# uga-ssrl/SSRLCV

Measured on AMD Instinct MI355X. Metric: Mpix/s SIFT extract (+ Mmatches/s 128-D brute-force, see `matcher`), higher is better.
Workload: dtype f32; 1 GPU; 2-view 4096x4096 pair per GPU (tools/scene.py pinhole views (PCG32 terrain + texture through Image::Camera)): SIFT_FeatureFactory::generateFeatures (sparse DoG path) on each image, pixels resident in HBM; images_per_gpu=2, parallelism=image-pair shard, library=release build (libssrlcv_hip_release.so)

## Files before the change

ssrlcv_amd/csrc/dev_switch.h:

```cpp
#pragma once
#include <stdlib.h>

#if (defined(SSRLCV_STAMPS) || defined(SSRLCV_MATCH_STATS) || defined(SSRLCV_TIMING_VARIANT)) && !defined(SSRLCV_INSTRUMENTED_BUILD)
#error "SSRLCV_STAMPS / SSRLCV_MATCH_STATS only build through `make instrumented` or the tools/ lab programs (-DSSRLCV_INSTRUMENTED_BUILD)"
#endif
#if defined(SSRLCV_LAB) || defined(SSRLCV_MATCH_LAB) || defined(SSRLCV_LAB_LOCAL_GATHER) || defined(SSRLCV_LAB_UPS_LOADS)
#error "the timing-lab variants (results invalid) were removed in round 6; see git history before 2026-10-05"
#endif

namespace svdev {
inline const char* env(const char* name) {
#ifdef SSRLCV_RELEASE
  (void)name;
  return nullptr;
#else
  return getenv(name);
#endif
}
}
```

ssrlcv_amd/csrc/keypoints.hip:

```cpp
#include <hip/hip_runtime.h>
#include <float.h>
#include <math.h>
#include <stdlib.h>
#include "compact.h"
#include "dev_switch.h"
#include "scan_lookback.h"
#include "device_math.h"
#include "sift_plan.h"
#include "ssrlcv_hip.h"

using svp::OctaveState;

namespace {

struct LevelSet {
  const float* lvl[svp::kGauss];
  const float* lvlMinMax;
  const float* minmax;
  const float2* polar;
  int w, h;
};

struct DogView {
  const float* lo;
// ... 104 lines not shown
  st->n = total;
  if (total == 0) st->hasExtrema = 0;
}
__global__ void k_book_featbase(OctaveState* st, uint32_t* featBase, uint32_t* numFeatures, uint32_t maxFeatures) {
  uint32_t tot = 0;
  for (int o = 0; o < svp::kOctaves; ++o) {
    featBase[o] = tot;
    tot += st[o].hasExtrema ? (uint32_t)st[o].n : 0u;
  }
  if (tot > maxFeatures) tot = maxFeatures;
  *numFeatures = tot;
}

__device__ __forceinline__ int segment_of(const OctaveState* st, int i) {
  int s = 0;
#pragma unroll
  for (int k = 1; k < svp::kDog; ++k)
    if (st->idx[k] <= i) s = k;
  return s;
}

__global__ __launch_bounds__(256) void k_flag_noise(const OctaveState* st, ssrlcv_sskeypoint* kps, float thr) {
  int n = st->hasExtrema ? st->n : 0;
  for (int i = blockIdx.x * 256 + threadIdx.x; i < n; i += gridDim.x * 256)
    kps[i].discard = (uint8_t)(fabsf(kps[i].intensity) < thr);
}

__global__ __launch_bounds__(256) void k_flag_edges(const OctaveState* st, ssrlcv_sskeypoint* kps, LevelSet L, float thr) {
  int n = st->hasExtrema ? st->n : 0;
  for (int i = blockIdx.x * 256 + threadIdx.x; i < n; i += gridDim.x * 256) {
    const DogView D = dog_view(L, segment_of(st, i));
    kps[i].discard = (uint8_t)edge_response_above(D, kps[i], L.w, thr);
  }
}

__global__ __launch_bounds__(256) void k_flag_noise_edges_window(const OctaveState* st, ssrlcv_sskeypoint* kps, LevelSet L,
                                                                 float noiseThr, float edgeThr, float pixelWidth,
                                                                 float lambda) {
  int n = st->hasExtrema ? st->n : 0;
  for (int i = blockIdx.x * 256 + threadIdx.x; i < n; i += gridDim.x * 256) {
    ssrlcv_sskeypoint kp = kps[i];
    bool drop = fabsf(kp.intensity) < noiseThr;
    drop = drop || edge_response_above(dog_view(L, segment_of(st, i)), kp, L.w, edgeThr);
    float ww = kp.sigma * lambda / pixelWidth;
    drop = drop || (kp.loc.x - ww) < 0.0f || (kp.loc.y - ww) < 0.0f || (kp.loc.x + ww) >= (unsigned)(L.w - 1) ||
           (kp.loc.y + ww) >= (unsigned)(L.h - 1);
    kps[i].discard = (uint8_t)drop;
  }
}

__global__ __launch_bounds__(256) void k_flag_window(const OctaveState* st, ssrlcv_sskeypoint* kps, int w, int h, float pixelWidth,
                                                     float lambda) {
  int n = st->hasExtrema ? st->n : 0;
  for (int i = blockIdx.x * 256 + threadIdx.x; i < n; i += gridDim.x * 256) {
    const ssrlcv_sskeypoint kp = kps[i];
    const float ww = kp.sigma * lambda / pixelWidth;
    kps[i].discard = (uint8_t)((kp.loc.x - ww) < 0.0f || (kp.loc.y - ww) < 0.0f || (kp.loc.x + ww) >= (unsigned)(w - 1) ||
                               (kp.loc.y + ww) >= (unsigned)(h - 1));
  }
}

template <typename Src>
__device__ __forceinline__ void refine_one(ssrlcv_sskeypoint& kp, int W, int H, int numBlurs, float sigmaMin, float mult, const Src& src) {
  int lx = (int)roundf(kp.loc.x), ly = (int)roundf(kp.loc.y);
  float hess[3][3], hinv[3][3] = {{0.0f, 0.0f, 0.0f}, {0.0f, 0.0f, 0.0f}, {0.0f, 0.0f, 0.0f}};
  float grad[3], temp[3], offset[3] = {0.0f, 0.0f, 0.0f};
  int bl = kp.blur;
  for (int attempt = 0; attempt < 5; ++attempt) {
    const auto Dl = src.view(bl - 1), Dm = src.view(bl), Du = src.view(bl + 1);
#define PM(yy, xx) Dm.norm((size_t)(yy) * W + (xx))
#define PL(yy, xx) Dl.norm((size_t)(yy) * W + (xx))
#define PU(yy, xx) Du.norm((size_t)(yy) * W + (xx))
    grad[0] = PM(ly, lx + 1) - PM(ly, lx - 1);
    grad[1] = PM(ly + 1, lx) - PM(ly - 1, lx);
    grad[2] = PU(ly, lx) - PL(ly, lx);
    float centre = PM(ly, lx);
    hess[0][0] = grad[0] - 2 * centre;
    hess[0][1] = (PM(ly + 1, lx + 1) - PM(ly - 1, lx + 1) - PM(ly + 1, lx - 1) + PM(ly - 1, lx - 1)) / 4.0f;
    hess[0][2] = (PU(ly, lx + 1) - PL(ly, lx + 1) - PU(ly, lx - 1) + PL(ly, lx - 1)) / 4.0f;
    hess[1][0] = hess[0][1];
    hess[1][1] = grad[1] - 2 * centre;
    hess[1][2] = (PU(ly + 1, lx) - PL(ly + 1, lx) - PU(ly - 1, lx) + PL(ly - 1, lx)) / 4.0f;
    hess[2][0] = hess[0][2];
    hess[2][1] = hess[1][2];
    hess[2][2] = grad[2] - 2 * centre;
#pragma unroll
    for (int r = 0; r < 3; ++r)
#pragma unroll
      for (int c = 0; c < 3; ++c) hess[r][c] *= -1.0f;
    sv::inverse3(hess, hinv);
#pragma unroll
    for (int r = 0; r < 3; ++r) {
      float val = 0;
#pragma unroll
      for (int c = 0; c < 3; ++c) val = __builtin_fmaf(hinv[r][c], grad[c], val);
      offset[r] = val;
    }
#pragma unroll
    for (int c = 0; c < 3; ++c) {
      float val = 0;
#pragma unroll
      for (int r = 0; r < 3; ++r) val = __builtin_fmaf(hess[r][c], grad[r], val);
      temp[c] = val;
    }
    if (fabsf(offset[0]) <= 0.5f && fabsf(offset[1]) <= 0.5f && fabsf(offset[2]) <= 0.5f) {
      kp.loc.x = (float)lx + offset[0];
      kp.loc.y = (float)ly + offset[1];
      lx = (int)roundf(kp.loc.x);
      ly = (int)roundf(kp.loc.y);
      kp.discard = (uint8_t)(lx <= 0 || ly <= 0 || lx >= W - 1 || ly >= H - 1);
      if (kp.discard) break;
      kp.intensity = PM(ly, lx) - (0.5f * ((temp[0] * grad[0]) + (temp[1] * grad[1]) + (temp[2] * grad[2])));
      kp.sigma = sigmaMin * sv_powf(mult, ((float)bl + offset[2]));
      if (fabsf(offset[2]) > 0.5) bl += (offset[2] > 0) ? 1 : -1;
      break;
    } else if (attempt == 4) {
      kp.discard = 1;
      break;
    } else {
      if (fabsf(offset[0]) > 0.5) lx += (offset[0] > 0) ? 1 : -1;
      if (fabsf(offset[1]) > 0.5) ly += (offset[1] > 0) ? 1 : -1;
      kp.loc.x = (float)lx;
      kp.loc.y = (float)ly;
      if (fabsf(offset[2]) > 0.5) bl += (offset[2] > 0) ? 1 : -1;
      if (bl >= numBlurs - 1 || bl <= 0 || lx <= 0 || ly <= 0 || lx >= W - 1 || ly >= H - 1) {
        kp.discard = 1;
        break;
      }
    }
#undef PM
#undef PL
#undef PU
  }
  kp.blur = bl;
}

__global__ __launch_bounds__(256) void k_refine(const OctaveState* st, ssrlcv_sskeypoint* kps, LevelSet L, float sigmaMin,
                                                float mult) {
  int n = st->hasExtrema ? st->n : 0;
  const PlanSource src{L};
  for (int gi = blockIdx.x * 256 + threadIdx.x; gi < n; gi += gridDim.x * 256) {
    ssrlcv_sskeypoint kp = kps[gi];
    refine_one(kp, L.w, L.h, svp::kDog, sigmaMin, mult, src);
    kps[gi] = kp;
  }
}

constexpr int kPolRows = 16;
struct PolarJobs {
  LevelSet L[svp::kOctaves];
  float2* out[svp::kOctaves];
  uint32_t start[svp::kOctaves + 1];
  uint32_t tilesX[svp::kOctaves];
};
#ifndef SSRLCV_NT_STORES
#define SSRLCV_NT_STORES 1
#endif
typedef float f32x2p __attribute__((ext_vector_type(2)));
__device__ __forceinline__ float polar_ld(const float* p) {
#if SSRLCV_NT_STORES
  return __builtin_nontemporal_load(p);
#else
  return *p;
#endif
}
__global__ __launch_bounds__(256) void k_polar(PolarJobs jobs) {
  __shared__ float s_n[kPolRows][256 + 2];
  int o = 0;
#pragma unroll
  for (int k = 1; k < svp::kOctaves; ++k)
    if (blockIdx.x >= jobs.start[k]) o = k;
  const LevelSet& L = jobs.L[o];
  float2* __restrict__ out = jobs.out[o];
  const uint32_t tile = blockIdx.x - jobs.start[o];
  const int tileX = (int)(tile % jobs.tilesX[o]), tileY = (int)(tile / jobs.tilesX[o]);
  const int W = L.w, H = L.h;
  const int x0 = tileX * 256, y0 = tileY * kPolRows;
  const int t = threadIdx.x, x = x0 + t;
  const int xc = x < W ? x : W - 1;
  const bool haloRole = t < 2 * kPolRows;
  const int hside = t & 1;
  int hx = hside ? x0 + 256 : x0 - 1;
  hx = hx < 0 ? 0 : (hx > W - 1 ? W - 1 : hx);
  int hy = y0 + (t >> 1);
  hy = hy > H - 1 ? H - 1 : hy;
  size_t rowOff[kPolRows + 2];
#pragma unroll
  for (int j = 0; j < kPolRows + 2; ++j) {
    int yy = y0 - 1 + j;
    yy = yy < 0 ? 0 : (yy > H - 1 ? H - 1 : yy);
    rowOff[j] = (size_t)yy * W + xc;
  }
  const size_t haloOff = (size_t)hy * W + hx;
  float nlo[kPolRows + 2], nloH = 0.0f;
  {
    const float mn = L.lvlMinMax[2];
    const sv::Divisor rg = sv::make_divisor(L.lvlMinMax[3] - mn);
    const float* __restrict__ g = L.lvl[1];
#pragma unroll
    for (int j = 0; j < kPolRows + 2; ++j) nlo[j] = sv::div_by(polar_ld(g + rowOff[j]) - mn, rg);
    if (haloRole) nloH = sv::div_by(g[haloOff] - mn, rg);
  }
  const int cl = x == 0 ? 1 : (x == W - 1 ? t - 1 : t);
  const int cr = x == 0 ? 3 : (x == W - 1 ? t + 1 : t + 2);
#pragma unroll 1
  for (int lvl = 1; lvl <= 3; ++lvl) {
    const float mn = L.lvlMinMax[2 * (lvl + 1)];
    const sv::Divisor rg = sv::make_divisor(L.lvlMinMax[2 * (lvl + 1) + 1] - mn);
    const float dmn = L.minmax[2 * lvl];
    const sv::Divisor drg = sv::make_divisor(L.minmax[2 * lvl + 1] - dmn);
    const float* __restrict__ g = L.lvl[lvl + 1];
    float v[kPolRows + 2];
#pragma unroll
    for (int j = 0; j < kPolRows + 2; ++j) {
      const float nhi = sv::div_by(polar_ld(g + rowOff[j]) - mn, rg);
      v[j] = sv::div_by((nhi - nlo[j]) - dmn, drg);
      nlo[j] = nhi;
    }
    if (lvl > 1) __syncthreads();
#pragma unroll
    for (int i = 0; i < kPolRows; ++i) s_n[i][t + 1] = v[i + 1];
    if (haloRole) {
      const float nhi = sv::div_by(g[haloOff] - mn, rg);
      s_n[t >> 1][hside ? 257 : 0] = sv::div_by((nhi - nloH) - dmn, drg);
      nloH = nhi;
    }
    __syncthreads();
    float2* __restrict__ lvlOut = out + (size_t)(lvl - 1) * svp::polar_level_stride(W, H);
    if (tile == 0) {
      if (t == 0) lvlOut[0] = make_float2(0.0f, 0.0f);
      for (int i = t; i < W + 1; i += 256) lvlOut[1 + (size_t)W * H + i] = make_float2(0.0f, 0.0f);
    }
    if (x < W) {
      float2* __restrict__ o = lvlOut + 1 + (size_t)y0 * W + x;
#pragma unroll
      for (int i = 0; i < kPolRows; ++i) {
        const int y = y0 + i;
        if (y >= H) break;
        float2 g2;
        g2.x = s_n[i][cr] - s_n[i][cl];
        const float up = y == 0 ? v[i + 3 < kPolRows + 2 ? i + 3 : kPolRows + 1] : (y == H - 1 ? v[i + 1] : v[i + 2]);
        const float dn = y == 0 ? v[i + 1] : (y == H - 1 ? v[i > 0 ? i - 1 : 0] : v[i]);
        g2.y = up - dn;
        float2 r;
        r.x = sqrtf((g2.x * g2.x) + (g2.y * g2.y));
        r.y = sv_atan2f(g2.y, g2.x);
#if SSRLCV_NT_STORES
        __builtin_nontemporal_store(f32x2p{r.x, r.y}, reinterpret_cast<f32x2p*>(o + (size_t)i * W));
#else
        o[(size_t)i * W] = r;
#endif
      }
    }
  }
}
typedef float f32x2 __attribute__((ext_vector_type(2)));
__device__ __forceinline__ int round_pos(float v) {
  int r;
  asm("v_cvt_rpi_i32_f32 %0, %1" : "=v"(r) : "v"(v));
  return r;
}

__device__ __forceinline__ float fmod_2pi_above(float v, float p) { return v >= p ? v - p : v; }
__device__ __forceinline__ float2 polar_px(const float2* __restrict__ pl, int W, int x, int y) {
  return pl[y * W + x];
}
__device__ __forceinline__ int round_coord(float v) {
  int r;
  asm("v_cvt_rpi_i32_f32 %0, %1" : "=v"(r) : "v"(v));
  return v == -0.5f ? -1 : r;
}

constexpr int kThetaChunk = 8;

struct RangeTable {
  uint32_t first[20], count[20], start[20];
  uint32_t total;
  uint32_t pad[3];
};
static_assert(sizeof(RangeTable) == 256, "tables sit at 256-byte strides in the plan's group block");
__device__ __constant__ const int kSegOrder[5] = {3, 2, 1, 4, 0};
__device__ __forceinline__ void build_ranges(const OctaveState* st, RangeTable* tab, int unitShift, uint32_t sel) {
  uint32_t pos = 0;
  for (int k = 0; k < 5; ++k) {
    const int seg = kSegOrder[k];
    for (int o = 0; o < svp::kOctaves; ++o) {
      const int r = k * 4 + o;
      uint32_t first = 0, count = 0;
      if (st[o].hasExtrema && ((sel >> (o * 5 + seg)) & 1u)) {
        const int lo = st[o].idx[seg], hi = seg < svp::kDog - 1 ? st[o].idx[seg + 1] : st[o].n;
        if (hi > lo) { first = (uint32_t)lo; count = (uint32_t)(hi - lo); }
      }
      tab->first[r] = first;
      tab->count[r] = count;
      tab->start[r] = pos;
      pos += (count + (1u << unitShift) - 1) >> unitShift;
    }
  }
  tab->total = pos;
}
__global__ void k_build_ranges(const OctaveState* st, RangeTable* tab, int unitShift, uint32_t sel) { build_ranges(st, tab, unitShift, sel); }
__global__ void k_book_and_desc_ranges(OctaveState* st, uint32_t* featBase, uint32_t* numFeatures, uint32_t maxFeatures, RangeTable* tab) {
  uint32_t tot = 0;
  for (int o = 0; o < svp::kOctaves; ++o) {
    featBase[o] = tot;
    tot += st[o].hasExtrema ? (uint32_t)st[o].n : 0u;
  }
  if (tot > maxFeatures) tot = maxFeatures;
  *numFeatures = tot;
  build_ranges(st, tab, 0, 0xFFFFFu);
}

constexpr int kOct0Groups = svp::kSampleGroups - 1;
struct GroupCtl {
  uint32_t segStart[svp::kDog];
  uint32_t totals[svp::kSampleGroups + 1];
  uint32_t groupSum[svp::kSampleGroups];
  uint32_t done[svp::kSampleGroups];
  uint32_t regular;
  uint32_t cut[2];
  uint32_t pad[32 - svp::kDog - 3 * svp::kSampleGroups - 4];
};
static_assert(sizeof(GroupCtl) == 128, "four of them + eight range tables fit the plan's 4 KB group block");
__device__ __forceinline__ bool blur_indices_regular(const OctaveState* st) {
  if (!st->hasExtrema) return true;
  bool ok = st->idx[0] == 0;
  for (int k = 1; k < svp::kDog; ++k) ok = ok && st->idx[k - 1] <= st->idx[k];
  return ok && st->idx[svp::kDog - 1] <= st->n;
}
__global__ void k_build_group_ranges(const OctaveState* st, RangeTable* tabs, GroupCtl* ctl, int unitShift, bool forceIrregular) {
  const bool reg = blur_indices_regular(st) && !forceIrregular;
  const uint32_t n0 = st[0].hasExtrema && st[0].n > 0 ? (uint32_t)st[0].n : 0u;
  ctl[0].regular = reg ? 1u : 0u;
  ctl[0].cut[0] = reg && n0 ? (uint32_t)st[0].idx[2] : n0;
  ctl[0].cut[1] = reg && n0 ? (uint32_t)st[0].idx[3] : n0;
  const uint32_t oct0 = 0x1Fu, rest = 0xFFFFFu & ~oct0;
  build_ranges(st, tabs + 0, unitShift, reg ? 0x03u : oct0);
  build_ranges(st, tabs + 1, unitShift, reg ? 0x04u : 0u);
  build_ranges(st, tabs + 2, unitShift, reg ? 0x18u : 0u);
  build_ranges(st, tabs + 3, unitShift, rest);
}
__global__ void k_build_desc_ranges_oct0(const OctaveState* st, RangeTable* tab, const GroupCtl* ctl, int g, uint32_t cap) {
  if (!ctl->regular) {
    build_ranges(st, tab, 0, g == kOct0Groups - 1 ? 0x1Fu : 0u);
    return;
  }
  const int segLo = g == 0 ? 0 : g + 1, segHi = g == 0 ? 2 : (g == 1 ? 3 : svp::kDog);
  const uint32_t end = ctl->totals[g + 1] < cap ? ctl->totals[g + 1] : cap;
  auto start_of = [&](int seg) {
    if (seg >= segHi) return end;
    const uint32_t enc = ctl->segStart[seg];
    const uint32_t v = enc ? enc - 1u : end;
    return v < end ? v : end;
  };
  uint32_t pos = 0;
  for (int k = 0; k < 5; ++k) {
    const int seg = kSegOrder[k];
    for (int o = 0; o < svp::kOctaves; ++o) {
      const int r = k * 4 + o;
      uint32_t first = 0, count = 0;
      if (o == 0 && seg >= segLo && seg < segHi) {
        const uint32_t lo = start_of(seg), hi = start_of(seg + 1);
        if (hi > lo) { first = lo; count = hi - lo; }
      }
      tab->first[r] = first;
      tab->count[r] = count;
      tab->start[r] = pos;
      pos += count;
    }
  }
  tab->total = pos;
}
__device__ __forceinline__ int range_of(const RangeTable* tab, uint32_t u) {
  int r = 0;
#pragma unroll
  for (int k = 1; k < 20; ++k)
    if (tab->start[k] <= u) r = k;
  return r;
}

struct OctaveSet {
  LevelSet L[svp::kOctaves];
  const ssrlcv_sskeypoint* kps[svp::kOctaves];
  float pixelWidth[svp::kOctaves];
  float* thetas[svp::kOctaves];
  uint32_t* thetaCnt[svp::kOctaves];
  const void* consts[svp::kOctaves];
};

template <int MAXO, int LPKS>
__global__ __launch_bounds__(64) void k_thetas(const OctaveState* states, const RangeTable* tab, OctaveSet set, float lambda,
                                               float orientationThreshold) {
  constexpr int LANES = 1 << LPKS, PER_BLOCK = 64 >> LPKS, CW = kThetaChunk * LANES;
  __shared__ float s_hist[36][PER_BLOCK];
  if (blockIdx.x >= tab->total) return;
  const int range = __builtin_amdgcn_readfirstlane(range_of(tab, blockIdx.x));
  const int octave = range & 3, useg = kSegOrder[range >> 2];
  const LevelSet& L = set.L[octave];
  const float pixelWidth = set.pixelWidth[octave];
  const int t = threadIdx.x, sub = t & (LANES - 1), col = t >> LPKS;
  const float fsub2 = (float)(2 * sub);
  const uint32_t local = (blockIdx.x - tab->start[range]) * PER_BLOCK + (uint32_t)(t >> LPKS);
  const bool have = local < tab->count[range];
  const int gi = (int)(tab->first[range] + local);
  const float pi = SSRLCV_PI_F;
  const float rad10 = pi / 18.0f;
  const float inv10 = 1.0f / rad10;
  ssrlcv_sskeypoint kp;
  kp.loc.x = kp.loc.y = 0.0f;
  kp.sigma = 1.0f;
  if (have) kp = set.kps[octave][gi];
  const float kx = kp.loc.x, ky = kp.loc.y;
  const float windowWidth = ceilf(kp.sigma * 3.0f * lambda / pixelWidth);
  const float minx = kx - windowWidth, miny = ky - windowWidth, maxx = kx + windowWidth, maxy = ky + windowWidth;
  const bool inside = have && useg >= 1 && useg <= 3 &&
                      !(minx < 0.0f || miny < 0.0f || maxx >= (unsigned)(L.w - 1) || maxy >= (unsigned)(L.h - 1));
#pragma unroll
  for (int i = 0; i < 36 * PER_BLOCK / 64; ++i) (&s_hist[0][0])[i * 64 + t] = 0.0f;
  const float weight = 2.0f * lambda * lambda * kp.sigma * kp.sigma;
  const float rweight = 1.0f / weight;
  const int W = L.w;
  const size_t levelStride = svp::polar_level_stride(L.w, L.h);
  {
    const float2* base = L.polar + (size_t)(useg - 1) * levelStride;
    const __amdgpu_buffer_rsrc_t rsrc = __builtin_amdgcn_make_buffer_rsrc((void*)base, 0, (int)(uint32_t)(levelStride * 8), 0x00020000);
    typedef unsigned u32x4 __attribute__((ext_vector_type(4)));
    typedef unsigned u32x2 __attribute__((ext_vector_type(2)));
    struct Cursor { float x, y, ty2; unsigned rowoff; bool act; };
    Cursor cf;
    cf.x = minx;
    cf.y = miny;
    cf.ty2 = (miny - ky) * (miny - ky);
    cf.rowoff = (unsigned)round_pos(miny) * (unsigned)W + 1u;
    cf.act = inside;
    auto advance = [&](Cursor& c) {
      float xn = c.x + (float)CW;
      if (__any(c.act && !(c.x >= (float)CW))) {
        float ch = c.x;
#pragma unroll 8
        for (int i = 0; i < CW; ++i) ch += 1.0f;
        xn = c.x >= (float)CW ? xn : ch;
      }
      if (c.act) {
        if (xn <= maxx) {
          c.x = xn;
        } else {
          c.x = minx;
          c.y += 1.0f;
          if (!(c.y <= maxy)) c.act = false;
          const float ty = c.y - ky;
          c.ty2 = ty * ty;
          c.rowoff = (unsigned)round_pos(c.y) * (unsigned)W + 1u;
        }
      }
    };
    typedef u32x4 Chunk[kThetaChunk / 2];
    auto fetch = [&](const Cursor& c, Chunk& into) {
      if (!c.act) return;
      const unsigned off = (c.rowoff + (unsigned)round_pos(c.x)) * 8u + 16u * (unsigned)sub;
#pragma unroll
      for (int j = 0; j < kThetaChunk / 4; ++j) into[j] = __builtin_amdgcn_raw_buffer_load_b128(rsrc, (int)(off + 16u * LANES * j), 0, 0);
    };
    auto fetch_upper = [&](const Cursor& c, Chunk& into) {
      if (!c.act) return;
      const unsigned off = (c.rowoff + (unsigned)round_pos(c.x)) * 8u + 16u * (unsigned)sub;
#pragma unroll
      for (int j = kThetaChunk / 4; j < kThetaChunk / 2; ++j) into[j] = __builtin_amdgcn_raw_buffer_load_b128(rsrc, (int)(off + 16u * LANES * j), 0, 0);
    };
    auto wants_upper = [&](const Cursor& c) { return __any(c.act && c.x + (float)(CW / 2 - 1) <= maxx); };
    Chunk qa, qb;
    Cursor ca, cb;
#pragma unroll
    for (int j = 0; j < kThetaChunk / 2; ++j) qa[j] = qb[j] = u32x4{0u, 0u, 0u, 0u};
    ca = cf;
    fetch(cf, qa);
    if (wants_upper(cf)) fetch_upper(cf, qa);
    advance(cf);
    cb = cf;
    auto step = [&](Chunk& cur, const Cursor& cc, Chunk& nxt, Cursor& cn) __attribute__((always_inline)) {
      cn = cf;
      fetch(cf, nxt);
      if (wants_upper(cf)) fetch_upper(cf, nxt);
      advance(cf);
      float xs[kThetaChunk];
      float xlast = cc.x + (float)(CW - 1);
#pragma unroll
      for (int i = 0; i < kThetaChunk; ++i) xs[i] = cc.x + (fsub2 + (float)(((i >> 1) << (1 + LPKS)) | (i & 1)));
      if (__any(cc.act && !(cc.x >= (float)CW))) {
        float ch = cc.x;
        float xc[kThetaChunk];
#pragma unroll
        for (int sIdx = 0; sIdx < CW; ++sIdx) {
          const int q = (sIdx >> 1) & (LANES - 1), i = ((sIdx >> (1 + LPKS)) << 1) | (sIdx & 1);
          if (LANES == 1 || q == 0) xc[i] = ch;
          else xc[i] = sub == q ? ch : xc[i];
          if (sIdx + 1 < CW) ch += 1.0f;
        }
        const bool direct = cc.x >= (float)CW;
#pragma unroll
        for (int i = 0; i < kThetaChunk; ++i) xs[i] = direct ? xs[i] : xc[i];
        xlast = direct ? xlast : ch;
      }
      const float cty2 = cc.ty2;
      const unsigned crow = cc.rowoff;
      const bool cact = cc.act;
      const bool aligned = cc.x >= 4.0f && round_pos(xlast) == round_pos(cc.x) + (CW - 1);
      if (__any(cact && !aligned)) {
        if (cact && !aligned) {
#pragma unroll
          for (int i = 0; i < kThetaChunk; ++i) {
            u32x2 e = u32x2{0u, 0u};
            if (xs[i] <= maxx) e = __builtin_amdgcn_raw_buffer_load_b64(rsrc, (int)((crow + (unsigned)round_pos(xs[i])) * 8u), 0, 0);
            cur[i >> 1][(i & 1) * 2] = e[0];
            cur[i >> 1][(i & 1) * 2 + 1] = e[1];
          }
        }
      }
      auto weigh = [&](float ang, float xi, float& wgt, int& bin) {
        const float angle = fmod_2pi_above(ang + (2.0f * pi), 2.0f * pi);
        bin = (int)floorf(sv::exact_div3(angle, rad10, inv10));
        const float tx = xi - kx;
        wgt = sv::expf_nonpos(sv::exact_div5(-((tx * tx) + cty2), weight, rweight));
      };
      const bool upperHalf = __any(cact && xs[kThetaChunk / 2] <= maxx);
      float wg[kThetaChunk], mg[kThetaChunk];
      float* slot[kThetaChunk];
      auto weigh_half = [&](auto hc) __attribute__((always_inline)) {
        constexpr int i0 = decltype(hc)::value * (kThetaChunk / 2);
#pragma unroll
        for (int i = i0; i < i0 + kThetaChunk / 2; ++i) {
          const unsigned um = cur[i >> 1][(i & 1) * 2], ua = cur[i >> 1][(i & 1) * 2 + 1];
          int bin;
          weigh(__builtin_bit_cast(float, ua), xs[i], wg[i], bin);
          const bool counts = cact && xs[i] <= maxx && (unsigned)bin < 36u;
          slot[i] = &s_hist[counts ? bin : 0][col];
          mg[i] = counts ? __builtin_bit_cast(float, um) : 0.0f;
        }
      };
      auto vote_half = [&](auto hc) __attribute__((always_inline)) {
        constexpr int j0 = decltype(hc)::value * (kThetaChunk / 4);
#pragma unroll
        for (int j = j0; j < j0 + kThetaChunk / 4; ++j) {
#pragma unroll
          for (int q = 0; q < LANES; ++q) {
            if (LANES == 1 || sub == q) {
              const float h0 = *slot[2 * j], h1 = *slot[2 * j + 1];
              const float n0 = fmaf(mg[2 * j], wg[2 * j], h0);
              const float n1 = fmaf(mg[2 * j + 1], wg[2 * j + 1], slot[2 * j + 1] == slot[2 * j] ? n0 : h1);
              *slot[2 * j] = n0;
              *slot[2 * j + 1] = n1;
            }
            if (LANES > 1) __builtin_amdgcn_wave_barrier();
          }
        }
      };
      weigh_half(std::integral_constant<int, 0>{});
      if (upperHalf) weigh_half(std::integral_constant<int, 1>{});
      vote_half(std::integral_constant<int, 0>{});
      if (upperHalf) vote_half(std::integral_constant<int, 1>{});
    };
    while (__any(ca.act)) {
      step(qa, ca, qb, cb);
      if (!__any(cb.act)) break;
      step(qb, cb, qa, ca);
    }
  }
  uint32_t cnt = 0;
  float outTheta[MAXO];
#pragma unroll
  for (int i = 0; i < MAXO; ++i) outTheta[i] = -FLT_MAX;
  if (inside && sub == 0) {
    float maxHist = 0.0f;
    for (int i = 0; i < 36; ++i) {
      const float h = s_hist[i][col];
      if (h > maxHist) maxHist = h;
    }
    maxHist *= orientationThreshold;
    float bestMag[MAXO], bestTh[MAXO];
#pragma unroll
    for (int i = 0; i < MAXO; ++i) { bestMag[i] = 0.0f; bestTh[i] = 0.0f; }
    float hprev = s_hist[35][col], hb = s_hist[0][col];
    for (int b = 0; b < 36; ++b) {
      const float hnext = s_hist[b == 35 ? 0 : b + 1][col];
      if (!(hb < maxHist || hb < hprev || hb < hnext || hb < bestMag[MAXO - 1])) {
        float tmag = hb;
        float tt = (hprev - hnext) / (hprev - (2.0f * hb) + hnext);
        tt *= (pi / 36.0f);
        tt += (b * rad10);
        tt = fmodf(tt + (2.0f * pi), 2.0f * pi);
#pragma unroll
        for (int i = 0; i < MAXO; ++i) {
          if (tmag > bestMag[i]) {
#pragma unroll
            for (int ii = i; ii < MAXO; ++ii) {
              float m2 = bestMag[ii], t2 = bestTh[ii];
              bestMag[ii] = tmag;
              bestTh[ii] = tt;
              tmag = m2;
              tt = t2;
            }
          }
        }
      }
      hprev = hb;
      hb = hnext;
    }
#pragma unroll
    for (int i = 0; i < MAXO; ++i) {
      if (bestMag[i] != 0.0f) { outTheta[i] = bestTh[i]; cnt = i + 1; }
    }
  }
  if (have && sub == 0) {
#pragma unroll
    for (int i = 0; i < MAXO; ++i) set.thetas[octave][(size_t)gi * svp::kMaxOrient + i] = outTheta[i];
    set.thetaCnt[octave][gi] = cnt;
  }
}

__device__ __forceinline__ float uniform_f(float v) {
  return __builtin_bit_cast(float, __builtin_amdgcn_readfirstlane(__builtin_bit_cast(int, v)));
}
struct DescConst {
  float c, s;
  float windowWidth;
  float invExpDen;
  float voteScale;
  float invBin;
  uint32_t magic;
  int32_t segment;
};
static_assert(sizeof(DescConst) == 32, "one s_load_dwordx8");
__global__ __launch_bounds__(256) void k_desc_consts(const RangeTable* tab, OctaveSet set, float lambda, const OctaveState* states,
                                                     const GroupCtl* regularCtl) {
  const uint32_t total = tab->total;
  const bool fromTable = regularCtl != nullptr && regularCtl->regular != 0u;
  for (uint32_t u = blockIdx.x * 256 + threadIdx.x; u < total; u += gridDim.x * 256) {
    const int range = range_of(tab, u);
    const int octave = range & 3;
    const int i = (int)(tab->first[range] + (u - tab->start[range]));
    const ssrlcv_sskeypoint* kps = set.kps[octave];
    const float pixelWidth = set.pixelWidth[octave];
    DescConst* __restrict__ out = (DescConst*)const_cast<void*>(set.consts[octave]);
    DescConst d;
    const float theta = kps[i].theta;
    d.c = sv_cosf(-theta);
    d.s = sv_sinf(-theta);
    d.windowWidth = ceilf(kps[i].sigma * lambda / pixelWidth);
    d.invExpDen = 1.0f / (2.0f * d.windowWidth * d.windowWidth);
    int boundExp;
    (void)frexpf(1.4143f * ((d.windowWidth + 2.0f) * (d.windowWidth + 2.0f)), &boundExp);
    d.voteScale = ldexpf(1.0f, 31 - boundExp);
    d.invBin = 1.0f / (d.windowWidth / 2.0f);
    const unsigned wi = (unsigned)(int)d.windowWidth;
    d.magic = wi > 1u ? 0xFFFFFFFFu / wi + 1u : 0u;
    d.segment = fromTable ? kSegOrder[range >> 2] : segment_of(states + octave, i);
    out[i] = d;
  }
}

__device__ __forceinline__ unsigned vote_u32(float v) {
  int r;
  asm("v_cvt_rpi_i32_f32 %0, %1" : "=v"(r) : "v"(v));
  return (unsigned)r;
}

#ifndef SSRLCV_DESC_COPIES
#define SSRLCV_DESC_COPIES 8
#endif
constexpr int kDescCopies = SSRLCV_DESC_COPIES;
#ifndef SSRLCV_DESC_VGPRS
#define SSRLCV_DESC_VGPRS 64
#endif
__global__ __launch_bounds__(256) __attribute__((amdgpu_waves_per_eu(4, 8), amdgpu_num_vgpr(SSRLCV_DESC_VGPRS), amdgpu_num_sgpr(102))) void k_descriptors(const RangeTable* tab, OctaveSet set, const uint32_t* featBase,
                                                     ssrlcv_sift_feature* __restrict__ features, uint32_t maxFeatures) {
  __shared__ unsigned s_bins[4][(1 + 128 + 2) * kDescCopies];
  __shared__ __attribute__((aligned(8))) uint8_t s_bytes[4][128];
  const int lane = threadIdx.x & 63, wave = __builtin_amdgcn_readfirstlane(threadIdx.x >> 6);
  unsigned* bins = s_bins[wave] + kDescCopies;
  const int copy = lane & (kDescCopies - 1);
  const float pi = SSRLCV_PI_F;
  const float rad45 = pi / 4.0f;
  const float inv45 = 1.0f / rad45;
  const uint32_t totalUnits = tab->total;
  for (uint32_t unit = blockIdx.x * 4 + wave; unit < totalUnits; unit += gridDim.x * 4) {
    const int range = range_of(tab, unit);
    const int octave = range & 3;
    const int gi = (int)(tab->first[range] + (unit - tab->start[range]));
    const LevelSet& L = set.L[octave];
    const float pixelWidth = set.pixelWidth[octave];
    const float2* __restrict__ polar = L.polar;
    const DescConst dc = reinterpret_cast<const DescConst*>(set.consts[octave])[gi];
    const ssrlcv_sskeypoint kp = set.kps[octave][gi];
    const int seg = dc.segment;
    const float kx = kp.loc.x, ky = kp.loc.y;
    const float theta = kp.theta;
    const float windowWidth = dc.windowWidth;
    const float binWidth = windowWidth / 2.0f;
    const float c = dc.c, s = dc.s;
    const float2* __restrict__ pl = polar + (size_t)(seg - 1) * svp::polar_level_stride(L.w, L.h) + 1;
#pragma unroll
    for (int i = 0; i < 2 * kDescCopies; ++i) bins[i * 64 + lane] = 0u;
    f32x2 rc[16];
    {
      const int ci = lane & 15;
      const float hx = ((float)(ci >> 2) * 0.5f - 0.75f) * windowWidth, hy = ((float)(ci & 3) * 0.5f - 0.75f) * windowWidth;
      const float rx = (hx * c) + (hy * s), ry = (-hx * s) + (hy * c);
#pragma unroll
      for (int cell = 0; cell < 16; ++cell) {
        if ((cell >> 2) == 0 || (cell & 3) == 0) continue;
        rc[cell].x = __builtin_bit_cast(float, __builtin_amdgcn_readlane(__builtin_bit_cast(int, rx), cell));
        rc[cell].y = __builtin_bit_cast(float, __builtin_amdgcn_readlane(__builtin_bit_cast(int, ry), cell));
      }
    }
    const float expDen = 2.0f * windowWidth * windowWidth, invExpDen = dc.invExpDen, invBin = dc.invBin;
    const float voteScale = dc.voteScale;
    const int Wi = (int)windowWidth;
    const unsigned centreIdx = (unsigned)(Wi * (Wi + 1));
    const unsigned magic = dc.magic;
    auto sample = [&](unsigned idx, float& cx, float& cy, bool& ok) {
      const unsigned yq = Wi == 1 ? idx : __umulhi(idx, magic);
      const unsigned xq = idx - yq * (unsigned)Wi + 1u;
      const bool centre = idx >= centreIdx;
      const float x = centre ? 0.0f : (float)(int)xq;
      const float y = centre ? 0.0f : (float)(int)yq;
      cx = (x * c) + (y * s);
      cy = (-x * s) + (y * c);
      ok = idx <= centreIdx && fmaxf(fabsf(cx), fabsf(cy)) <= windowWidth;
    };
    auto gather = [&](float px, float py) { return polar_px(pl, L.w, round_coord(px), round_coord(py)); };
    auto split = [&](float2 pg, bool live, float& w0, float& w1, unsigned*& pa, float& ang, bool& odd) {
      ang = fmod_2pi_above(pg.y - theta + (2.0f * pi), 2.0f * pi);
      const float t45 = ang * inv45;
      const float fk = floorf(t45);
      const float u = t45 - fk;
      odd = live && !(u > 1.0e-4f && u < 0.9999f);
      int k0 = (int)fk;
      const float a0 = fabsf(ang - (fk * rad45)), a1 = fabsf(ang - ((fk + 1.0f) * rad45));
      w0 = (live && !odd && (unsigned)k0 < 8u) ? 1.0f - sv::exact_div3(a0, rad45, inv45) : 0.0f;
      w1 = (live && !odd && (unsigned)(k0 + 1) < 8u) ? 1.0f - sv::exact_div3(a1, rad45, inv45) : 0.0f;
      k0 = k0 < -1 ? -1 : k0;
      pa = bins + k0 * kDescCopies + copy;
    };
    float ncx, ncy;
    bool nok;
    sample((unsigned)lane, ncx, ncy, nok);
    float2 npg[4] = {make_float2(0.0f, 0.0f), make_float2(0.0f, 0.0f), make_float2(0.0f, 0.0f), make_float2(0.0f, 0.0f)};
    auto gather4 = [&]() {
      npg[0] = gather(ncx + kx, ncy + ky);
      npg[1] = gather(kx - ncy, ncx + ky);
      npg[2] = gather(kx - ncx, ky - ncy);
      npg[3] = gather(ncy + kx, ky - ncx);
    };
    if (nok) gather4();
    for (unsigned base = 0; base <= centreIdx; base += 64) {
      const float cx = ncx, cy = ncy;
      const bool ok = nok;
      const float2 pg0 = npg[0], pg1 = npg[1], pg2 = npg[2], pg3 = npg[3];
      const bool turned = ok && base + (unsigned)lane < centreIdx;
      sample(base + 64 + (unsigned)lane, ncx, ncy, nok);
      if (nok) gather4();
      const float r2n = -((cx * cx) + (cy * cy));
      const float g = sv::expf_nonpos(sv::exact_div3(r2n, expDen, invExpDen)) * voteScale;
      float a0, a1, b0, b1, c0, c1, d0, d1, angA, angB, angC, angD;
      bool oddA, oddB, oddC, oddD;
      unsigned *pa, *pb, *pc, *pd;
      split(pg0, ok, a0, a1, pa, angA, oddA);
      split(pg1, turned, b0, b1, pb, angB, oddB);
      split(pg2, turned, c0, c1, pc, angC, oddC);
      split(pg3, turned, d0, d1, pd, angD, oddD);
      const float magA = pg0.x * g, magB = pg1.x * g, magC = pg2.x * g, magD = pg3.x * g;
      const float bwl = ok ? binWidth : -1.0f;
#pragma unroll
      for (int cell = 0; cell < 16; ++cell) {
        const int nx = cell >> 2, ny = cell & 3;
        if (nx == 0 || ny == 0) continue;
        const int cellB = (3 - ny) * 4 + nx, cellC = 15 - cell, cellD = ny * 4 + (3 - nx);
        const float tx = fabsf(rc[cell].x - cx), ty = fabsf(rc[cell].y - cy);
        if (fmaxf(tx, ty) <= bwl) {
          const float wxy = (1.0f - sv::exact_div3(tx, binWidth, invBin)) * (1.0f - sv::exact_div3(ty, binWidth, invBin));
          atomicAdd(pa + cell * 8 * kDescCopies, vote_u32((wxy * a0) * magA));
          atomicAdd(pa + cell * 8 * kDescCopies + kDescCopies, vote_u32((wxy * a1) * magA));
          atomicAdd(pb + cellB * 8 * kDescCopies, vote_u32((wxy * b0) * magB));
          atomicAdd(pb + cellB * 8 * kDescCopies + kDescCopies, vote_u32((wxy * b1) * magB));
          atomicAdd(pc + cellC * 8 * kDescCopies, vote_u32((wxy * c0) * magC));
          atomicAdd(pc + cellC * 8 * kDescCopies + kDescCopies, vote_u32((wxy * c1) * magC));
          atomicAdd(pd + cellD * 8 * kDescCopies, vote_u32((wxy * d0) * magD));
          atomicAdd(pd + cellD * 8 * kDescCopies + kDescCopies, vote_u32((wxy * d1) * magD));
        }
      }
      if (__ballot(oddA || oddB || oddC || oddD) != 0ull) {
#pragma unroll 1
        for (int m = 0; m < 4; ++m) {
          const bool odd = m == 0 ? oddA : m == 1 ? oddB : m == 2 ? oddC : oddD;
          if (!odd) continue;
          const float mcx = m == 0 ? cx : m == 1 ? -cy : m == 2 ? -cx : cy;
          const float mcy = m == 0 ? cy : m == 1 ? cx : m == 2 ? -cy : -cx;
          const float mang = m == 0 ? angA : m == 1 ? angB : m == 2 ? angC : angD;
          const float mmag = m == 0 ? magA : m == 1 ? magB : m == 2 ? magC : magD;
#pragma unroll 1
          for (int cell = 0; cell < 16; ++cell) {
            const int ci = lane & 15;
            (void)ci;
            const float hx0 = ((float)(cell >> 2) * 0.5f - 0.75f) * windowWidth, hy0 = ((float)(cell & 3) * 0.5f - 0.75f) * windowWidth;
            const float rx = (hx0 * c) + (hy0 * s), ry = (-hx0 * s) + (hy0 * c);
            float hx = fabsf(rx - mcx), hy = fabsf(ry - mcy);
            if (hx <= binWidth && hy <= binWidth) {
              hx = hx / binWidth;
              hy = hy / binWidth;
              for (int k = 0; k < 8; ++k) {
                float angle = fabsf(mang - ((float)k * rad45));
                if (angle < rad45) {
                  angle /= rad45;
                  const float temp = (1.0f - hx) * (1.0f - hy) * (1.0f - angle) * mmag;
                  atomicAdd(bins + (cell * 8 + k) * kDescCopies + copy, vote_u32(temp));
                }
              }
            }
          }
        }
      }
    }
    __builtin_amdgcn_wave_barrier();
    unsigned t0 = 0u, t1 = 0u;
#pragma unroll
    for (int cpy = 0; cpy < kDescCopies; ++cpy) {
      t0 += bins[lane * kDescCopies + cpy];
      t1 += bins[(lane + 64) * kDescCopies + cpy];
    }
    float v0 = (float)t0, v1 = (float)t1;
    float sq = sqrtf(sv::wave_sum((v0 * v0) + (v1 * v1)));
    v0 = v0 / sq;
    v1 = v1 / sq;
    if (v0 > 0.2f) v0 = 0.2f;
    if (v1 > 0.2f) v1 = 0.2f;
    sq = sqrtf(sv::wave_sum((v0 * v0) + (v1 * v1)));
    {
      int b0 = lane, b1 = lane + 64;
      int o0 = (((b0 >> 3) & 3) * 4 + (b0 >> 5)) * 8 + (b0 & 7);
      int o1 = (((b1 >> 3) & 3) * 4 + (b1 >> 5)) * 8 + (b1 & 7);
      s_bytes[wave][o0] = (uint8_t)roundf(255.0f * v0 / sq);
      s_bytes[wave][o1] = (uint8_t)roundf(255.0f * v1 / sq);
    }
    __builtin_amdgcn_wave_barrier();
    const uint32_t fi = featBase[octave] + (uint32_t)gi;
    if (fi < maxFeatures) {
      ssrlcv_sift_feature* f = features + fi;
      if (lane < 16) *reinterpret_cast<uint2*>(&f->values[lane * 8]) = *reinterpret_cast<const uint2*>(&s_bytes[wave][lane * 8]);
      if (lane == 16) {
        f->parent = -1;
        reinterpret_cast<int*>(f)[1] = 0;
        f->theta = kp.theta;
        f->sigma = kp.sigma;
        f->loc.x = kp.loc.x * pixelWidth;
        f->loc.y = kp.loc.y * pixelWidth;
      }
    }
    __builtin_amdgcn_wave_barrier();
  }
}

LevelSet make_levels(const ssrlcv_sift_plan* plan, char* ws, int o) {
  LevelSet L;
  const svp::OctavePlan& oc = plan->oct[o];
  for (int b = 0; b < svp::kGauss; ++b) L.lvl[b] = (const float*)(ws + plan->off_gauss[o][b]);
  L.lvlMinMax = (const float*)(ws + plan->off_minmax) + (size_t)o * 2 * (svp::kGauss + svp::kDog);
  L.minmax = L.lvlMinMax + 2 * svp::kGauss;
  L.polar = (const float2*)(ws + oc.off_polar);
  L.w = (int)oc.w;
  L.h = (int)oc.h;
  return L;
}

void launch_polar(const ssrlcv_sift_plan* plan, char* ws, hipStream_t st, int oFirst = 0, int oLast = svp::kOctaves - 1) {
  PolarJobs jobs;
  uint32_t pos = 0;
  for (int o = 0; o < svp::kOctaves; ++o) {
    const svp::OctavePlan& oc = plan->oct[o];
    jobs.L[o] = make_levels(plan, ws, o);
    jobs.out[o] = (float2*)(ws + oc.off_polar);
    jobs.start[o] = pos;
    jobs.tilesX[o] = (oc.w + 255) / 256;
    if (o >= oFirst && o <= oLast) pos += jobs.tilesX[o] * ((oc.h + kPolRows - 1) / kPolRows);
  }
  jobs.start[svp::kOctaves] = pos;
  hipLaunchKernelGGL(k_polar, dim3(pos), dim3(256), 0, st, jobs);
}

}
namespace svp {
void launch_polar_octave(const ssrlcv_sift_plan* plan, char* ws, int octave, hipStream_t st) {
  PolarJobs jobs;
  const svp::OctavePlan& oc = plan->oct[octave];
  const uint32_t tilesX = (oc.w + 255) / 256, tiles = tilesX * ((oc.h + kPolRows - 1) / kPolRows);
  for (int o = 0; o < svp::kOctaves; ++o) {
    jobs.L[o] = make_levels(plan, ws, octave);
    jobs.out[o] = (float2*)(ws + oc.off_polar);
    jobs.tilesX[o] = tilesX;
    jobs.start[o] = o <= octave ? 0u : tiles;
  }
  jobs.start[svp::kOctaves] = tiles;
  hipLaunchKernelGGL(k_polar, dim3(tiles), dim3(256), 0, st, jobs);
}
}
namespace {
hipError_t run_discard(OctaveState* st, const ssrlcv_sskeypoint* src, ssrlcv_sskeypoint* dst, uint32_t cap,
                       uint32_t* words, hipStream_t stream) {
  const OctaveState* cst = st;
  auto keyfn = [=] __device__(uint32_t i) -> uint32_t {
    if (!cst->hasExtrema || (int)i >= cst->n) return 0u;
    if (src[i].discard) return 0u;
    return 1u << segment_of(cst, (int)i);
  };
  auto emit = [=] __device__(uint32_t i, int, uint32_t d) { dst[d] = src[i]; };
  uint32_t* totals = nullptr;
  auto post = [=] __device__(const uint32_t* tot) { book_discard(st, tot); };
  return svc::partition<svp::kDog, 8>(cap, keyfn, emit, words, &totals, stream, &st->n, 1u, post);
}

constexpr unsigned kWaveKernelOversubscription = 16;
inline unsigned list_blocks(uint32_t cap) {
  unsigned b = (cap + 255) / 256;
  return b > 1024 ? 1024 : b;
}

}

extern "C" {

int ssrlcv_sift_plan_keypoints(const ssrlcv_sift_plan* plan, void* workspace, int octave, ssrlcv_sskeypoint** list,
                               int** blurIndices_dev) {
  if (!plan || !workspace || octave < 0 || octave >= svp::kOctaves) return SSRLCV_ERR_INVALID_ARG;
  char* ws = (char*)workspace;
  if (list) *list = (ssrlcv_sskeypoint*)(ws + (plan->listInB[octave] ? plan->oct[octave].off_kpB : plan->oct[octave].off_kpA));
  if (blurIndices_dev) *blurIndices_dev = (int*)(ws + plan->off_state + sizeof(OctaveState) * octave);
  return SSRLCV_OK;
}

int ssrlcv_sift_plan_overflow(const ssrlcv_sift_plan* plan, const void* workspace, uint32_t* octaveMask,
                              ssrlcv_stream_t stream) {
  if (!plan || !workspace || !octaveMask) return SSRLCV_ERR_INVALID_ARG;
  OctaveState st[svp::kOctaves];
  SSRLCV_HIP_TRY(hipMemcpyAsync(st, (const char*)workspace + plan->off_state, sizeof st, hipMemcpyDeviceToHost,
                                (hipStream_t)stream));
  SSRLCV_HIP_TRY(hipStreamSynchronize((hipStream_t)stream));
  uint32_t m = 0;
  for (int o = 0; o < svp::kOctaves; ++o)
    if (st[o].overflow) m |= 1u << o;
  *octaveMask = m;
  return m ? SSRLCV_ERR_CAPACITY : SSRLCV_OK;
}

}
namespace {

struct ListCtx {
  const ssrlcv_sift_plan* plan;
  const svp::OctavePlan* oc;
  int o;
  hipStream_t s;
  OctaveState* st;
  LevelSet L;
  ssrlcv_sskeypoint *A, *B;
  uint8_t* flags;
  uint32_t* words;
  uint32_t cap;
  ssrlcv_sskeypoint* cur() const { return plan->listInB[o] ? B : A; }
  ssrlcv_sskeypoint* oth() const { return plan->listInB[o] ? A : B; }
  void flip() const { plan->listInB[o] ^= 1; }
};
ListCtx make_ctx(const ssrlcv_sift_plan* plan, char* ws, int o, hipStream_t s) {
  ListCtx c;
  c.plan = plan;
  c.oc = &plan->oct[o];
  c.o = o;
  c.s = s;
  c.st = (OctaveState*)(ws + plan->off_state) + o;
  c.L = make_levels(plan, ws, o);
  c.A = (ssrlcv_sskeypoint*)(ws + c.oc->off_kpA);
  c.B = (ssrlcv_sskeypoint*)(ws + c.oc->off_kpB);
  c.flags = (uint8_t*)(ws + c.oc->off_flags);
  c.words = (uint32_t*)(ws + c.oc->off_part);
  c.cap = c.oc->cap;
  return c;
}

int stage_extrema(const ListCtx& c, bool afterFirstNoise) {
  hipLaunchKernelGGL(k_state_reset, dim3(1), dim3(1), 0, c.s, c.st);
  c.plan->listInB[c.o] = 0;
  const uint32_t P = c.oc->w * c.oc->h, cap = c.cap;
  const int W = (int)c.oc->w;
  const int octaveId = c.o;
  const float s1 = c.oc->sigma[1], s2 = c.oc->sigma[2], s3 = c.oc->sigma[3];
  const LevelSet Lc = c.L;
  ssrlcv_sskeypoint* first = c.A;
  auto emit = [=] __device__(uint32_t p, int b, uint32_t d) {
    if (d >= cap) return;
    ssrlcv_sskeypoint kp;
    kp.octave = octaveId;
    kp.blur = (int)b + 1;
    kp.loc.x = (float)(p % W);
    kp.loc.y = (float)(p / W);
    kp.intensity = dog_view(Lc, b + 1).raw(p);
    kp.sigma = b == 0 ? s1 : b == 1 ? s2 : s3;
    kp.theta = -1.0f;
    kp.discard = 0;
    first[d] = kp;
  };
  uint32_t* totals = nullptr;
  hipError_t e = svc::partition_flags<3>(P, c.flags, afterFirstNoise ? svp::kNoiseFlagShift : 0, emit, c.words, &totals, c.s);
  if (e != hipSuccess) return (int)e;
  hipLaunchKernelGGL(k_book_extrema, dim3(1), dim3(1), 0, c.s, c.st, totals, cap);
  return SSRLCV_OK;
}
int discard_flagged(const ListCtx& c) {
  hipError_t e = run_discard(c.st, c.cur(), c.oth(), c.cap, c.words, c.s);
  if (e != hipSuccess) return (int)e;
  c.flip();
  return SSRLCV_OK;
}
int stage_noise(const ListCtx& c, float threshold) {
  hipLaunchKernelGGL(k_flag_noise, dim3(list_blocks(c.cap)), dim3(256), 0, c.s, c.st, c.cur(), threshold);
  return discard_flagged(c);
}
int stage_refine(const ListCtx& c) {
  hipLaunchKernelGGL(k_refine, dim3(list_blocks(c.cap)), dim3(256), 0, c.s, c.st, c.cur(), c.L, c.oc->sigma[0],
                     c.oc->sigma[1] / c.oc->sigma[0]);
  int rc = discard_flagged(c);
  if (rc) return rc;
  OctaveState* st = c.st;
  const OctaveState* cst = c.st;
  const ssrlcv_sskeypoint* src = c.cur();
  ssrlcv_sskeypoint* dst = c.oth();
  auto keyfn = [=] __device__(uint32_t i) -> uint32_t {
    if (!cst->hasExtrema || (int)i >= cst->n) return 0u;
    int b = src[i].blur;
    return (b < 0 || b >= svp::kDog) ? 0u : (1u << b);
  };
  auto emit = [=] __device__(uint32_t i, int, uint32_t d) { dst[d] = src[i]; };
  uint32_t* totals = nullptr;
  auto post = [=] __device__(const uint32_t* tot) { book_rescan(st, tot); };
  hipError_t e = svc::partition<svp::kDog, 8>(c.cap, keyfn, emit, c.words, &totals, c.s, &st->n, 1u, post);
  if (e != hipSuccess) return (int)e;
  c.flip();
  return SSRLCV_OK;
}
int stage_edges(const ListCtx& c) {
  hipLaunchKernelGGL(k_flag_edges, dim3(list_blocks(c.cap)), dim3(256), 0, c.s, c.st, c.cur(), c.L, svp::kEdgeThreshold);
  return discard_flagged(c);
}
int stage_window(const ListCtx& c) {
  hipLaunchKernelGGL(k_flag_window, dim3(list_blocks(c.cap)), dim3(256), 0, c.s, c.st, c.cur(), c.L.w, c.L.h, c.oc->pixelWidth,
                     c.plan->params.descriptorContribWidth);
  return discard_flagged(c);
}
int stage_noise_edges_window(const ListCtx& c) {
  hipLaunchKernelGGL(k_flag_noise_edges_window, dim3(list_blocks(c.cap)), dim3(256), 0, c.s, c.st, c.cur(), c.L, svp::kNoiseThreshold,
                     svp::kEdgeThreshold, c.oc->pixelWidth, c.plan->params.descriptorContribWidth);
  return discard_flagged(c);
}

OctaveSet make_set(const ssrlcv_sift_plan* plan, char* ws) {
  OctaveSet set;
  for (int o = 0; o < svp::kOctaves; ++o) {
    const svp::OctavePlan& oc = plan->oct[o];
    set.L[o] = make_levels(plan, ws, o);
    set.kps[o] = (const ssrlcv_sskeypoint*)(ws + (plan->listInB[o] ? oc.off_kpB : oc.off_kpA));
    set.pixelWidth[o] = oc.pixelWidth;
    set.thetas[o] = (float*)(ws + oc.off_theta);
    set.thetaCnt[o] = (uint32_t*)(ws + oc.off_thetaCnt);
    set.consts[o] = ws + oc.off_descConst;
  }
  return set;
}

constexpr int kExpandItems = 16;
__global__ __launch_bounds__(svs::kThreads) void k_expand_orient(OctaveState* st, const ssrlcv_sskeypoint* __restrict__ src,
                                                                 ssrlcv_sskeypoint* __restrict__ dst, const float* __restrict__ thetas,
                                                                 const uint32_t* __restrict__ thetaCnt, uint32_t maxO, uint32_t cap,
                                                                 svs::TileScan<1> ts, GroupCtl* ctl, int g, int pieces) {
  constexpr int ITEMS = kExpandItems;
  constexpr uint32_t kTile = svs::kThreads * ITEMS;
  const uint32_t n = st->hasExtrema && st->n > 0 ? (uint32_t)st->n : 0u;
  uint32_t lo = 0, hi = n;
  if (pieces > 1) {
    if (g > 0) lo = ctl->cut[g - 1] < n ? ctl->cut[g - 1] : n;
    if (g + 1 < pieces) hi = ctl->cut[g] < n ? ctl->cut[g] : n;
    if (hi < lo) hi = lo;
  }
  const uint32_t e0 = lo * maxO, e1 = hi * maxO;
  const uint32_t tiles = (e1 - e0 + kTile - 1) / kTile;
  const uint32_t before = ctl->totals[g];
  uint32_t segFirst[svp::kDog];
#pragma unroll
  for (int k = 0; k < svp::kDog; ++k) segFirst[k] = (uint32_t)st->idx[k] * maxO;
  for (uint32_t tile = svs::next_tile(ts.counter); tile < tiles; tile = svs::next_tile(ts.counter)) {
    const uint32_t base = e0 + tile * kTile + threadIdx.x * ITEMS;
    bool keep[ITEMS];
    uint32_t mine[1] = {0};
#pragma unroll
    for (int j = 0; j < ITEMS; ++j) {
      const uint32_t e = base + j, i = e / maxO;
      keep[j] = e < e1 && (e - i * maxO) < thetaCnt[i];
      mine[0] += keep[j] ? 1u : 0u;
    }
    uint32_t excl[1], total[1], prefix[1];
    svs::block_exclusive<1>(mine, excl, total);
    svs::tile_prefix<1>(ts, tile, total, prefix);
    uint32_t at = before + prefix[0] + excl[0];
#pragma unroll
    for (int j = 0; j < ITEMS; ++j) {
      const uint32_t e = base + j;
      if (e < e1) {
#pragma unroll
        for (int k = 0; k < svp::kDog; ++k)
          if (segFirst[k] == e) ctl->segStart[k] = at + 1u;
      }
      if (keep[j]) {
        if (at < cap) {
          const uint32_t i = e / maxO;
          ssrlcv_sskeypoint kp = src[i];
          kp.theta = thetas[(size_t)i * svp::kMaxOrient + (e - i * maxO)];
          dst[at] = kp;
        }
        ++at;
      }
    }
    if (tile == tiles - 1 && threadIdx.x == 0) ctl->groupSum[g] = prefix[0] + total[0];
  }
  __shared__ bool s_last;
  __syncthreads();
  if (threadIdx.x == 0) {
    __threadfence();
    s_last = atomicAdd(&ctl->done[g], 1u) == gridDim.x - 1;
  }
  __syncthreads();
  if (s_last && threadIdx.x == 0) {
    __threadfence();
    const uint32_t total = before + __hip_atomic_load(&ctl->groupSum[g], __ATOMIC_RELAXED, __HIP_MEMORY_SCOPE_AGENT);
    ctl->totals[g + 1] = total;
    if (g + 1 == pieces && st->hasExtrema) {
      for (int b = 0; b < svp::kDog; ++b) {
        const uint32_t enc = __hip_atomic_load(&ctl->segStart[b], __ATOMIC_RELAXED, __HIP_MEMORY_SCOPE_AGENT);
        const uint32_t start = enc ? enc - 1u : total;
        st->idx[b] = (int)(start < cap ? start : cap);
      }
      uint32_t kept = total;
      if (kept > cap) { st->overflow = 1; kept = cap; }
      st->n = (int)kept;
      if (kept == 0) st->hasExtrema = 0;
    }
  }
}

struct GroupBlock {
  RangeTable thetaTab[svp::kSampleGroups];
  RangeTable descTab[svp::kSampleGroups];
  GroupCtl ctl[svp::kOctaves];
};
static_assert(sizeof(RangeTable) <= 256 && 8 * 256 + svp::kOctaves * sizeof(GroupCtl) <= 4096, "fits the plan's group block");
inline RangeTable* theta_tab(const ssrlcv_sift_plan* plan, char* ws, int g) { return (RangeTable*)(ws + plan->off_groups + 256 * g); }
inline RangeTable* desc_tab(const ssrlcv_sift_plan* plan, char* ws, int g) { return (RangeTable*)(ws + plan->off_groups + 256 * (svp::kSampleGroups + g)); }
inline GroupCtl* group_ctl(const ssrlcv_sift_plan* plan, char* ws, int o) { return (GroupCtl*)(ws + plan->off_groups + 2048) + o; }

#ifndef SSRLCV_THETAS_LANES_SHIFT
#define SSRLCV_THETAS_LANES_SHIFT 2
#endif
inline int thetas_lanes_shift() {
  static const int shift = [] {
    const char* e = svdev::env("SSRLCV_THETAS_LANES");
    if (!e) return SSRLCV_THETAS_LANES_SHIFT;
    const int lanes = atoi(e);
    return lanes >= 4 ? 2 : (lanes >= 2 ? 1 : 0);
  }();
  return shift;
}
inline unsigned thetas_grid(const ssrlcv_sift_plan* plan, int oFirst, int oLast, int shift) {
  unsigned blocks = 20;
  const uint32_t per = 64u >> shift;
  for (int o = oFirst; o <= oLast; ++o) blocks += (plan->oct[o].cap + per - 1) / per;
  return blocks;
}
template <int LPKS, typename... Args>
void launch_thetas_l(uint32_t maxO, unsigned blocks, hipStream_t st, Args... args) {
  switch (maxO) {
    case 1: hipLaunchKernelGGL((k_thetas<1, LPKS>), dim3(blocks), dim3(64), 0, st, args...); break;
    case 2: hipLaunchKernelGGL((k_thetas<2, LPKS>), dim3(blocks), dim3(64), 0, st, args...); break;
    case 3: hipLaunchKernelGGL((k_thetas<3, LPKS>), dim3(blocks), dim3(64), 0, st, args...); break;
    default: hipLaunchKernelGGL((k_thetas<4, LPKS>), dim3(blocks), dim3(64), 0, st, args...); break;
  }
}
template <typename... Args>
void launch_thetas(uint32_t maxO, int shift, unsigned blocks, hipStream_t st, Args... args) {
  switch (shift) {
    case 0: launch_thetas_l<0>(maxO, blocks, st, args...); break;
    case 1: launch_thetas_l<1>(maxO, blocks, st, args...); break;
    default: launch_thetas_l<2>(maxO, blocks, st, args...); break;
  }
}

int expand_prepare(const ssrlcv_sift_plan* plan, char* ws, int o, int g, hipStream_t st) {
  const svp::OctavePlan& oc = plan->oct[o];
  const uint32_t capTiles = (oc.cap * plan->params.maxOrientations + svs::kThreads * kExpandItems - 1) / (svs::kThreads * kExpandItems);
  const size_t scanBytes = svs::workspace_bytes<1>(capTiles);
  SSRLCV_HIP_TRY(hipMemsetAsync(ws + oc.off_part + (size_t)g * scanBytes, 0, scanBytes, st));
  return SSRLCV_OK;
}
int launch_expand(const ssrlcv_sift_plan* plan, char* ws, int o, int g, int pieces, hipStream_t es, bool scratchZeroed = false) {
  const svp::OctavePlan& oc = plan->oct[o];
  const uint32_t maxO = plan->params.maxOrientations, cap = oc.cap;
  OctaveState* states = (OctaveState*)(ws + plan->off_state);
  const ssrlcv_sskeypoint* src = (const ssrlcv_sskeypoint*)(ws + (plan->listInB[o] ? oc.off_kpB : oc.off_kpA));
  ssrlcv_sskeypoint* dst = (ssrlcv_sskeypoint*)(ws + (plan->listInB[o] ? oc.off_kpA : oc.off_kpB));
  const uint32_t capTiles = (cap * maxO + svs::kThreads * kExpandItems - 1) / (svs::kThreads * kExpandItems);
  const size_t scanBytes = svs::workspace_bytes<1>(capTiles);
  char* part = ws + oc.off_part + (size_t)g * scanBytes;
  if (!scratchZeroed) SSRLCV_HIP_TRY(hipMemsetAsync(part, 0, scanBytes, es));
  unsigned blocks = capTiles / 8 + 1;
  blocks = blocks > 1024u ? 1024u : blocks;
  hipLaunchKernelGGL(k_expand_orient, dim3(blocks), dim3(svs::kThreads), 0, es, states + o, src, dst, (const float*)(ws + oc.off_theta),
                     (const uint32_t*)(ws + oc.off_thetaCnt), maxO, cap, svs::make_tile_scan<1>(part, capTiles), group_ctl(plan, ws, o), g, pieces);
  return SSRLCV_OK;
}
bool expand_scratch_fits(const ssrlcv_sift_plan* plan, int o, int pieces) {
  const svp::OctavePlan& oc = plan->oct[o];
  const uint32_t capTiles = (oc.cap * plan->params.maxOrientations + svs::kThreads * kExpandItems - 1) / (svs::kThreads * kExpandItems);
  const size_t P = (size_t)oc.w * oc.h;
  const size_t words = (size_t)3 * 4 * ((P + 8191) / 8192) + 16 + (size_t)svp::kDog * 4 * (((size_t)oc.cap * svp::kMaxOrient + 2047) / 2048) + 16;
  return (size_t)pieces * svs::workspace_bytes<1>(capTiles) <= words * 4;
}

int queue_rest_orientations(const ssrlcv_sift_plan* plan, char* ws, hipStream_t st, svp::PlanAsync* as) {
  OctaveState* states = (OctaveState*)(ws + plan->off_state);
  const uint32_t maxO = plan->params.maxOrientations;
  OctaveSet set = make_set(plan, ws);
  uint32_t thetaSel = 0xFFFFFu;
#ifdef SSRLCV_INSTRUMENTED_BUILD
  if (const char* e = svdev::env("SSRLCV_TIMING_THETAS_SEL")) thetaSel = (uint32_t)strtoul(e, nullptr, 16);
#endif
  const int lanesShift = thetas_lanes_shift();
  RangeTable* restRanges = theta_tab(plan, ws, 1);
  hipLaunchKernelGGL(k_build_ranges, dim3(1), dim3(1), 0, st, states, restRanges, 6 - lanesShift, 0xFFFFFu & ~0x1Fu & thetaSel);
  launch_thetas(maxO, lanesShift, thetas_grid(plan, 1, svp::kOctaves - 1, lanesShift), st, (const OctaveState*)states, (const RangeTable*)restRanges,
                set, plan->params.orientationContribWidth, plan->params.orientationThreshold);
  for (int o = 1; o < svp::kOctaves; ++o) {
    int rc = launch_expand(plan, ws, o, 0, 1, st);
    if (rc) return rc;
    plan->listInB[o] ^= 1;
  }
  SSRLCV_HIP_TRY(hipEventRecord(as->expandJoin[1], st));
  return SSRLCV_OK;
}

inline hipStream_t expand_stream(svp::PlanAsync* as, hipStream_t caller, int o) {
  return !as || o == 0 ? caller : (o == 1 ? as->chain : (o == 2 ? as->table : as->chain2));
}
int orientations_prologue(const ssrlcv_sift_plan* plan, char* ws, hipStream_t caller, svp::PlanAsync* as) {
  OctaveState* states = (OctaveState*)(ws + plan->off_state);
  uint32_t thetaSel = 0xFFFFFu;
#ifdef SSRLCV_INSTRUMENTED_BUILD
  if (const char* e = svdev::env("SSRLCV_TIMING_THETAS_SEL")) thetaSel = (uint32_t)strtoul(e, nullptr, 16);
#endif
  SSRLCV_HIP_TRY(hipMemsetAsync(group_ctl(plan, ws, 0), 0, sizeof(GroupCtl) * svp::kOctaves, caller));
  hipLaunchKernelGGL(k_build_ranges, dim3(1), dim3(1), 0, caller, states, theta_tab(plan, ws, 0), 6 - thetas_lanes_shift(), thetaSel);
  if (as) {
    SSRLCV_HIP_TRY(hipEventRecord(as->expandFork, caller));
    for (int o = 1; o < svp::kOctaves; ++o) SSRLCV_HIP_TRY(hipStreamWaitEvent(expand_stream(as, caller, o), as->expandFork, 0));
  }
  for (int o = 0; o < svp::kOctaves; ++o) {
    const int rc = expand_prepare(plan, ws, o, 0, expand_stream(as, caller, o));
    if (rc) return rc;
  }
  return SSRLCV_OK;
}

int stage_orientations(const ssrlcv_sift_plan* plan, char* ws, hipStream_t caller, svp::PlanAsync* as, bool polarDone, bool restInFlight = false,
                       bool prologueDone = false) {
  OctaveState* states = (OctaveState*)(ws + plan->off_state);
  const uint32_t maxO = plan->params.maxOrientations;
  OctaveSet set = make_set(plan, ws);
  RangeTable* thetaRanges = theta_tab(plan, ws, 0);
  uint32_t thetaSel = 0xFFFFFu;
#ifdef SSRLCV_INSTRUMENTED_BUILD
  if (const char* e = svdev::env("SSRLCV_TIMING_THETAS_SEL")) thetaSel = (uint32_t)strtoul(e, nullptr, 16);
#endif
  const int lanesShift = thetas_lanes_shift();
  const float lambdaO = plan->params.orientationContribWidth, othr = plan->params.orientationThreshold;
  if (restInFlight) {
    hipLaunchKernelGGL(k_build_ranges, dim3(1), dim3(1), 0, caller, states, thetaRanges, 6 - lanesShift, 0x1Fu & thetaSel);
    launch_thetas(maxO, lanesShift, thetas_grid(plan, 0, 0, lanesShift), caller, (const OctaveState*)states, (const RangeTable*)thetaRanges, set,
                  lambdaO, othr);
    int rc = launch_expand(plan, ws, 0, 0, 1, caller);
    if (rc) return rc;
    plan->listInB[0] ^= 1;
    SSRLCV_HIP_TRY(hipStreamWaitEvent(caller, as->expandJoin[1], 0));
    return SSRLCV_OK;
  }
  if (!prologueDone) orientations_prologue(plan, ws, caller, as);
  if (!polarDone) launch_polar(plan, ws, caller);
  launch_thetas(maxO, lanesShift, thetas_grid(plan, 0, svp::kOctaves - 1, lanesShift), caller, (const OctaveState*)states, (const RangeTable*)thetaRanges, set, lambdaO, othr);
  if (as) {
    SSRLCV_HIP_TRY(hipEventRecord(as->groupFork, caller));
    for (int o = 1; o < svp::kOctaves; ++o) SSRLCV_HIP_TRY(hipStreamWaitEvent(expand_stream(as, caller, o), as->groupFork, 0));
  }
  for (int o = 0; o < svp::kOctaves; ++o) {
    int rc = launch_expand(plan, ws, o, 0, 1, expand_stream(as, caller, o), true);
    if (rc) return rc;
    plan->listInB[o] ^= 1;
  }
  if (as) {
    for (int o = 1; o < svp::kOctaves; ++o) {
      SSRLCV_HIP_TRY(hipEventRecord(as->groupExpanded[o - 1], expand_stream(as, caller, o)));
      SSRLCV_HIP_TRY(hipStreamWaitEvent(caller, as->groupExpanded[o - 1], 0));
    }
  }
  return SSRLCV_OK;
}

void book_features(const ssrlcv_sift_plan* plan, char* ws, uint32_t* numFeatures, hipStream_t caller, bool withDescRanges = false) {
  if (withDescRanges)
    hipLaunchKernelGGL(k_book_and_desc_ranges, dim3(1), dim3(1), 0, caller, (OctaveState*)(ws + plan->off_state),
                       (uint32_t*)(ws + plan->oct[0].off_featBase), numFeatures, plan->maxFeatures, desc_tab(plan, ws, 0));
  else
    hipLaunchKernelGGL(k_book_featbase, dim3(1), dim3(1), 0, caller, (OctaveState*)(ws + plan->off_state),
                       (uint32_t*)(ws + plan->oct[0].off_featBase), numFeatures, plan->maxFeatures);
}

unsigned desc_blocks(const ssrlcv_sift_plan* plan, int oFirst, int oLast, unsigned* maxBlocks) {
  unsigned blocks = 0, mx = 1;
  for (int o = oFirst; o <= oLast; ++o) {
    blocks += list_blocks(plan->oct[o].cap);
    mx = list_blocks(plan->oct[o].cap) > mx ? list_blocks(plan->oct[o].cap) : mx;
  }
  if (maxBlocks) *maxBlocks = mx;
  return blocks;
}

int stage_descriptors(const ssrlcv_sift_plan* plan, char* ws, ssrlcv_sift_feature* features, hipStream_t caller, bool rangesBuilt = false) {
  OctaveState* states = (OctaveState*)(ws + plan->off_state);
  OctaveSet set = make_set(plan, ws);
  RangeTable* descRanges = desc_tab(plan, ws, 0);
  uint32_t* featBase = (uint32_t*)(ws + plan->oct[0].off_featBase);
  unsigned maxBlocks = 1;
  const unsigned descBlocks = desc_blocks(plan, 0, svp::kOctaves - 1, &maxBlocks);
  if (!rangesBuilt) hipLaunchKernelGGL(k_build_ranges, dim3(1), dim3(1), 0, caller, states, descRanges, 0, 0xFFFFFu);
  hipLaunchKernelGGL(k_desc_consts, dim3(maxBlocks * svp::kOctaves), dim3(256), 0, caller, (const RangeTable*)descRanges, set,
                     plan->params.descriptorContribWidth, (const OctaveState*)states, (const GroupCtl*)nullptr);
  hipLaunchKernelGGL(k_descriptors, dim3(descBlocks * kWaveKernelOversubscription), dim3(256), 0, caller, (const RangeTable*)descRanges, set,
                     (const uint32_t*)featBase, features, plan->maxFeatures);
  return SSRLCV_OK;
}

int stage_sampling_pipelined(const ssrlcv_sift_plan* plan, char* ws, ssrlcv_sift_feature* features, uint32_t* numFeatures,
                             hipStream_t caller, svp::PlanAsync* as) {
  OctaveState* states = (OctaveState*)(ws + plan->off_state);
  const uint32_t maxO = plan->params.maxOrientations;
  const float lambdaO = plan->params.orientationContribWidth, othr = plan->params.orientationThreshold;
  const float lambdaD = plan->params.descriptorContribWidth;
  uint32_t* featBase = (uint32_t*)(ws + plan->oct[0].off_featBase);
  OctaveSet setT = make_set(plan, ws);
  for (int o = 0; o < svp::kOctaves; ++o) plan->listInB[o] ^= 1;
  OctaveSet setD = make_set(plan, ws);
  for (int o = 0; o < svp::kOctaves; ++o) plan->listInB[o] ^= 1;
  const hipStream_t gs[svp::kSampleGroups] = {caller, as->chain, as->chain2, as->table};
  const int lanesShift = thetas_lanes_shift();
  unsigned thetaBlocks[svp::kSampleGroups], descBlocks[svp::kSampleGroups], constBlocks[svp::kSampleGroups];
  for (int g = 0; g < svp::kSampleGroups; ++g) {
    const int oFirst = g < kOct0Groups ? 0 : 1, oLast = g < kOct0Groups ? 0 : svp::kOctaves - 1;
    thetaBlocks[g] = thetas_grid(plan, oFirst, oLast, lanesShift);
    unsigned mx = 1;
    descBlocks[g] = desc_blocks(plan, oFirst, oLast, &mx) * kWaveKernelOversubscription;
    constBlocks[g] = mx * (unsigned)(oLast - oFirst + 1);
  }
  SSRLCV_HIP_TRY(hipMemsetAsync(group_ctl(plan, ws, 0), 0, sizeof(GroupCtl) * svp::kOctaves, caller));
  SSRLCV_HIP_TRY(hipMemsetAsync(featBase, 0, 4 * svp::kOctaves, caller));
  static const bool forceIrregular = svdev::env("SSRLCV_SAMPLING_IRREGULAR") != nullptr;
  hipLaunchKernelGGL(k_build_group_ranges, dim3(1), dim3(1), 0, caller, (const OctaveState*)states, theta_tab(plan, ws, 0), group_ctl(plan, ws, 0), 6 - lanesShift,
                     forceIrregular);
  SSRLCV_HIP_TRY(hipEventRecord(as->groupFork, caller));
  for (int g = 1; g < svp::kSampleGroups; ++g) SSRLCV_HIP_TRY(hipStreamWaitEvent(gs[g], as->groupFork, 0));
  for (int g = 0; g < svp::kSampleGroups; ++g)
    launch_thetas(maxO, lanesShift, thetaBlocks[g], gs[g], (const OctaveState*)states, (const RangeTable*)theta_tab(plan, ws, g), setT, lambdaO, othr);
  for (int g = 0; g < kOct0Groups; ++g) {
    if (g > 0) SSRLCV_HIP_TRY(hipStreamWaitEvent(gs[g], as->groupExpanded[g - 1], 0));
    int rc = launch_expand(plan, ws, 0, g, kOct0Groups, gs[g]);
    if (rc) return rc;
    SSRLCV_HIP_TRY(hipEventRecord(as->groupExpanded[g], gs[g]));
    hipLaunchKernelGGL(k_build_desc_ranges_oct0, dim3(1), dim3(1), 0, gs[g], (const OctaveState*)states, desc_tab(plan, ws, g),
                       (const GroupCtl*)group_ctl(plan, ws, 0), g, plan->oct[0].cap);
    hipLaunchKernelGGL(k_desc_consts, dim3(constBlocks[g]), dim3(256), 0, gs[g], (const RangeTable*)desc_tab(plan, ws, g), setD, lambdaD,
                       (const OctaveState*)states, (const GroupCtl*)group_ctl(plan, ws, 0));
    if (g > 0) SSRLCV_HIP_TRY(hipEventRecord(as->groupReady[g], gs[g]));
  }
  {
    const int g = svp::kSampleGroups - 1;
    for (int o = 1; o < svp::kOctaves; ++o) {
      int rc = launch_expand(plan, ws, o, 0, 1, gs[g]);
      if (rc) return rc;
    }
    SSRLCV_HIP_TRY(hipStreamWaitEvent(gs[g], as->groupExpanded[kOct0Groups - 1], 0));
    book_features(plan, ws, numFeatures, gs[g]);
    hipLaunchKernelGGL(k_build_ranges, dim3(1), dim3(1), 0, gs[g], (const OctaveState*)states, desc_tab(plan, ws, g), 0, 0xFFFFFu & ~0x1Fu);
    hipLaunchKernelGGL(k_desc_consts, dim3(constBlocks[g]), dim3(256), 0, gs[g], (const RangeTable*)desc_tab(plan, ws, g), setD, lambdaD,
                       (const OctaveState*)states, (const GroupCtl*)nullptr);
    SSRLCV_HIP_TRY(hipEventRecord(as->groupReady[g], gs[g]));
  }
  for (int o = 0; o < svp::kOctaves; ++o) plan->listInB[o] ^= 1;
  for (int g = 0; g < svp::kSampleGroups; ++g) {
    if (g > 0) SSRLCV_HIP_TRY(hipStreamWaitEvent(caller, as->groupReady[g], 0));
    hipLaunchKernelGGL(k_descriptors, dim3(descBlocks[g]), dim3(256), 0, caller, (const RangeTable*)desc_tab(plan, ws, g), setD,
                       (const uint32_t*)featBase, features, plan->maxFeatures);
  }
  return SSRLCV_OK;
}

int run_list_chain(const ssrlcv_sift_plan* plan, char* ws, int o, hipStream_t s) {
  const int stop = plan->stopStage;
  const ListCtx c = make_ctx(plan, ws, o, s);
  int rc = stage_extrema(c, stop >= 1);
  if (!rc && stop >= 2) rc = stage_refine(c);
  if (!rc && stop >= 5) rc = stage_noise_edges_window(c);
  else {
    if (!rc && stop >= 3) rc = stage_noise(c, svp::kNoiseThreshold);
    if (!rc && stop >= 4) rc = stage_edges(c);
  }
  return rc;
}

}
namespace svp {
int launch_chain_octave(const ssrlcv_sift_plan* plan, char* ws, int octave, hipStream_t st) { return run_list_chain(plan, ws, octave, st); }
}
extern "C" {

static void drain_side_streams(const ssrlcv_sift_plan* plan, hipStream_t st) {
  svp::PlanAsync* as = plan->asyncState == 1 ? plan->async : nullptr;
  if (as) {
    for (hipStream_t side : {as->chain, as->table, as->chain2, as->polar}) {
      if (hipEventRecord(as->fork, side) == hipSuccess) (void)hipStreamWaitEvent(st, as->fork, 0);
    }
    (void)hipGetLastError();
  }
  plan->chain0InFlight = 0;
  plan->polarInFlight = 0;
}
static int describe_impl(const ssrlcv_sift_plan* plan, void* workspace, ssrlcv_sift_feature* features, uint32_t* numFeatures, ssrlcv_stream_t stream);
int ssrlcv_hip_sift_describe(const ssrlcv_sift_plan* plan, void* workspace, ssrlcv_sift_feature* features, uint32_t* numFeatures,
                             ssrlcv_stream_t stream) {
  const int rc = describe_impl(plan, workspace, features, numFeatures, stream);
  if (rc && plan) drain_side_streams(plan, (hipStream_t)stream);
  return rc;
}
static int describe_impl(const ssrlcv_sift_plan* plan, void* workspace, ssrlcv_sift_feature* features,
                             uint32_t* numFeatures, ssrlcv_stream_t stream) {
  if (!plan || !workspace || !numFeatures) return SSRLCV_ERR_INVALID_ARG;
  char* ws = (char*)workspace;
  const int stop = plan->stopStage;
  if (stop >= 7 && !features) return SSRLCV_ERR_INVALID_ARG;
  svp::PlanAsync* as = svp::plan_async(plan);
  const hipStream_t caller = (hipStream_t)stream;
  static const bool splitWanted = svdev::env("SSRLCV_THETAS_SPLIT") != nullptr;
  static const bool pipelinedSampling = svdev::env("SSRLCV_SAMPLING_PIPELINED") != nullptr;
  const bool splitRest = as && stop >= 6 && !plan->polarInFlight && splitWanted && !pipelinedSampling;
  if (splitRest) SSRLCV_HIP_TRY(hipMemsetAsync(group_ctl(plan, ws, 0), 0, sizeof(GroupCtl) * svp::kOctaves, caller));
  if (as) {
    SSRLCV_HIP_TRY(hipEventRecord(as->fork, caller));
    SSRLCV_HIP_TRY(hipStreamWaitEvent(as->chain, as->fork, 0));
    SSRLCV_HIP_TRY(hipStreamWaitEvent(as->chain2, as->fork, 0));
    SSRLCV_HIP_TRY(hipStreamWaitEvent(as->table, as->fork, 0));
    if ((svp::stream_priority_mode() & 1)) SSRLCV_HIP_TRY(hipStreamWaitEvent(as->polar, as->fork, 0));
    if (stop >= 6 && !plan->polarInFlight) {
      const hipStream_t ps = (svp::stream_priority_mode() & 1) ? as->polar : as->table;
      if (splitRest) {
        launch_polar(plan, ws, ps, 1, svp::kOctaves - 1);
        SSRLCV_HIP_TRY(hipEventRecord(as->polarDone[1], ps));
        launch_polar(plan, ws, ps, 0, 0);
      } else {
        launch_polar(plan, ws, ps);
      }
    }
  }
  for (int o = 0; o < svp::kOctaves; ++o) {
    const hipStream_t cs = !as || o == 0 ? caller : (o == 1 ? as->chain : as->chain2);
    if (!((plan->chain0InFlight >> o) & 1)) {
      const int rc = run_list_chain(plan, ws, o, cs);
      if (rc) return rc;
    }
    if (as && (o == 1 || o == svp::kOctaves - 1)) {
      SSRLCV_HIP_TRY(hipEventRecord(as->join[o], cs));
      SSRLCV_HIP_TRY(hipStreamWaitEvent(caller, as->join[o], 0));
    }
  }
  plan->chain0InFlight = 0;
  if (splitRest) {
    SSRLCV_HIP_TRY(hipStreamWaitEvent(as->chain2, as->join[1], 0));
    SSRLCV_HIP_TRY(hipStreamWaitEvent(as->chain2, as->polarDone[1], 0));
    const int rc = queue_rest_orientations(plan, ws, as->chain2, as);
    if (rc) return rc;
  }
  const bool earlyPrologue = as && stop >= 6 && !splitRest && !(stop >= 7 && pipelinedSampling && expand_scratch_fits(plan, 0, kOct0Groups));
  if (earlyPrologue) {
    const int rc = orientations_prologue(plan, ws, caller, as);
    if (rc) return rc;
  }
  if (as) {
    SSRLCV_HIP_TRY(hipEventRecord(as->join[svp::kOctaves], (svp::stream_priority_mode() & 1) ? as->polar : as->table));
    SSRLCV_HIP_TRY(hipStreamWaitEvent(caller, as->join[svp::kOctaves], 0));
    if (plan->polarInFlight) {
      for (int o = 0; o < svp::kOctaves; ++o) SSRLCV_HIP_TRY(hipStreamWaitEvent(caller, as->polarDone[o], 0));
      plan->polarInFlight = 0;
    }
  }
  if (stop >= 7 && as && pipelinedSampling && expand_scratch_fits(plan, 0, kOct0Groups)) {
    int rc = stage_sampling_pipelined(plan, ws, features, numFeatures, caller, as);
    if (rc) return rc;
    SSRLCV_LAUNCH_CHECK();
    return SSRLCV_OK;
  }
  if (stop >= 6) {
    int rc = stage_orientations(plan, ws, caller, as, as != nullptr, splitRest, earlyPrologue);
    if (rc) return rc;
  }
  book_features(plan, ws, numFeatures, caller, stop >= 7);
  if (stop >= 7) {
    int rc = stage_descriptors(plan, ws, features, caller, true);
    if (rc) return rc;
  }
  SSRLCV_LAUNCH_CHECK();
  return SSRLCV_OK;
}

int ssrlcv_hip_sift_stage(const ssrlcv_sift_plan* plan, void* workspace, int stage, ssrlcv_sift_feature* features,
                          uint32_t* numFeatures, ssrlcv_stream_t stream) {
  if (!plan || !workspace || !numFeatures || stage < 0 || stage > 7) return SSRLCV_ERR_INVALID_ARG;
  if (stage == 7 && !features) return SSRLCV_ERR_INVALID_ARG;
  char* ws = (char*)workspace;
  const hipStream_t caller = (hipStream_t)stream;
  int rc = SSRLCV_OK;
  if (stage <= 5) {
    for (int o = 0; o < svp::kOctaves && !rc; ++o) {
      const ListCtx c = make_ctx(plan, ws, o, caller);
      switch (stage) {
        case 0: rc = stage_extrema(c, false); break;
        case 1: rc = stage_noise(c, (float)(svp::kNoiseThreshold * 0.8)); break;
        case 2: rc = stage_refine(c); break;
        case 3: rc = stage_noise(c, svp::kNoiseThreshold); break;
        case 4: rc = stage_edges(c); break;
        default: rc = stage_window(c); break;
      }
    }
  } else if (stage == 6) {
    rc = stage_orientations(plan, ws, caller, nullptr, false);
  }
  if (rc) return rc;
  book_features(plan, ws, numFeatures, caller);
  if (stage == 7) rc = stage_descriptors(plan, ws, features, caller);
  if (rc) return rc;
  SSRLCV_LAUNCH_CHECK();
  return SSRLCV_OK;
}

}
namespace {
__global__ __launch_bounds__(256) void k_x_find_extrema(int W, int H, const float* __restrict__ up, const float* __restrict__ mid,
                                                        const float* __restrict__ low, int* __restrict__ extrema) {
  const size_t id = (size_t)blockIdx.x * 256 + threadIdx.x;
  if (id >= (size_t)W * H) return;
  const int x = (int)(id % W), y = (int)(id / W);
  if (!(x > 0 && y > 0 && x < W - 1 && y < H - 1)) return;
  const float v = mid[id];
  float mx = -FLT_MAX, mn = FLT_MAX;
#pragma unroll
  for (int dy = -1; dy <= 1; ++dy)
#pragma unroll
    for (int dx = -1; dx <= 1; ++dx) {
      const size_t a = (size_t)(y + dy) * W + (x + dx);
      mx = fmaxf(mx, fmaxf(low[a], fmaxf(mid[a], up[a])));
      mn = fminf(mn, fminf(low[a], fminf(mid[a], up[a])));
    }
  extrema[id] = (mx == v || mn == v) ? (int)id : -1;
}
__global__ __launch_bounds__(256) void k_x_fill_extrema(int n, int W, int octave, int blur, float sigma, const int* __restrict__ addr,
                                                        const float* __restrict__ pixels, ssrlcv_sskeypoint* __restrict__ out) {
  const int i = blockIdx.x * 256 + threadIdx.x;
  if (i >= n) return;
  const int index = addr[i];
  ssrlcv_sskeypoint kp;
  kp.octave = octave;
  kp.blur = blur;
  kp.loc.x = (float)(index % W);
  kp.loc.y = (float)(index / W);
  kp.intensity = pixels[index];
  kp.sigma = sigma;
  kp.theta = -1.0f;
  kp.discard = 0;
  out[i] = kp;
}
__global__ __launch_bounds__(256) void k_x_flag_noise(uint32_t n, ssrlcv_sskeypoint* kps, float thr) {
  const uint32_t i = blockIdx.x * 256 + threadIdx.x;
  if (i < n) kps[i].discard = (uint8_t)(fabsf(kps[i].intensity) < thr);
}
__global__ __launch_bounds__(256) void k_x_flag_edges(uint32_t n, uint32_t start, int W, ssrlcv_sskeypoint* kps, const float* pixels,
                                                      float thr) {
  const uint32_t i = blockIdx.x * 256 + threadIdx.x;
  if (i < n) kps[start + i].discard = (uint8_t)edge_response_above(MatView{pixels}, kps[start + i], W, thr);
}
__global__ __launch_bounds__(256) void k_x_check(uint32_t n, uint32_t start, int W, int H, float pixelWidth, float lambda,
                                                 ssrlcv_sskeypoint* kps) {
  const uint32_t i = blockIdx.x * 256 + threadIdx.x;
  if (i >= n) return;
  const ssrlcv_sskeypoint kp = kps[start + i];
  const float ww = kp.sigma * lambda / pixelWidth;
  if ((kp.loc.x - ww) < 0.0f || (kp.loc.y - ww) < 0.0f || (kp.loc.x + ww) >= (unsigned)(W - 1) || (kp.loc.y + ww) >= (unsigned)(H - 1))
    kps[start + i].discard = 1;
}
__global__ __launch_bounds__(256) void k_x_refine(uint32_t n, int W, int H, float sigmaMin, float mult, int numBlurs, MatSource src,
                                                  ssrlcv_sskeypoint* kps) {
  const uint32_t i = blockIdx.x * 256 + threadIdx.x;
  if (i >= n) return;
  ssrlcv_sskeypoint kp = kps[i];
  refine_one(kp, W, H, numBlurs, sigmaMin, mult, src);
  kps[i] = kp;
}
__device__ __forceinline__ float2 x_gradient(const float* __restrict__ px, int W, int H, int x, int y) {
  int xc0 = x + 1, xc1 = x - 1, yc0 = y + 1, yc1 = y - 1;
  if (xc1 == -1) { xc0 += 1; xc1 += 1; }
  else if (xc0 == W) { xc0 -= 1; xc1 -= 1; }
  if (yc1 == -1) { yc0 += 1; yc1 += 1; }
  else if (yc0 == H) { yc0 -= 1; yc1 -= 1; }
  float2 g;
  g.x = px[(size_t)y * W + xc0] - px[(size_t)y * W + xc1];
  g.y = px[(size_t)yc0 * W + x] - px[(size_t)yc1 * W + x];
  return g;
}
__global__ __launch_bounds__(256) void k_x_gradients(int W, int H, const float* __restrict__ px, float2* __restrict__ grad) {
  const size_t id = (size_t)blockIdx.x * 256 + threadIdx.x;
  if (id < (size_t)W * H) grad[id] = x_gradient(px, W, H, (int)(id % W), (int)(id / W));
}
__global__ __launch_bounds__(64) void k_x_thetas(uint32_t n, uint32_t start, int W, int H, float pixelWidth, float lambda,
                                                 const ssrlcv_sskeypoint* __restrict__ kps, const float2* __restrict__ grad,
                                                 int* __restrict__ thetaNumbers, uint32_t maxO, float orientationThreshold,
                                                 float* __restrict__ thetas) {
  const uint32_t gi = blockIdx.x * 64 + threadIdx.x;
  if (gi >= n) return;
  const float pi = 3.1415927f;
  const ssrlcv_sskeypoint kp = kps[start + gi];
  const int regNumOrient = (int)(maxO > 8u ? 8u : maxO);
  for (int i = 0; i < regNumOrient; ++i) { thetas[(size_t)gi * maxO + i] = -FLT_MAX; thetaNumbers[(size_t)gi * maxO + i] = -1; }
  const float kx = kp.loc.x, ky = kp.loc.y;
  const float windowWidth = ceilf(kp.sigma * 3.0f * lambda / pixelWidth);
  const float minx = kx - windowWidth, miny = ky - windowWidth, maxx = kx + windowWidth, maxy = ky + windowWidth;
  if (minx < 0.0f || miny < 0.0f || maxx >= (unsigned)(W - 1) || maxy >= (unsigned)(H - 1)) return;
  float hist[36];
  for (int i = 0; i < 36; ++i) hist[i] = 0.0f;
  const float weight = 2.0f * lambda * lambda * kp.sigma * kp.sigma;
  const float rad10 = pi / 18.0f;
  for (float y = miny; y <= maxy; y += 1.0f) {
    for (float x = minx; x <= maxx; x += 1.0f) {
      const float2 g = grad[(size_t)llroundf(y) * W + (size_t)llroundf(x)];
      const float tx = x - kx, ty = y - ky;
      const float angle = fmodf(sv_atan2f(g.y, g.x) + (2.0f * pi), 2.0f * pi);
      const int bin = (int)floorf(angle / rad10);
      const float mag = sqrtf((g.x * g.x) + (g.y * g.y));
      const float wgt = sv_expf(-((tx * tx) + (ty * ty)) / weight);
#pragma unroll
      for (int b = 0; b < 36; ++b)
        if (b == bin) hist[b] = __builtin_fmaf(mag, wgt, hist[b]);
    }
  }
  float maxHist = 0.0f;
  for (int i = 0; i < 36; ++i)
    if (hist[i] > maxHist) maxHist = hist[i];
  maxHist *= orientationThreshold;
  float bx[8], by[8];
  for (int i = 0; i < 8; ++i) { bx[i] = 0.0f; by[i] = 0.0f; }
  for (int b = 0; b < 36; ++b) {
// ... 273 lines not shown
```

ssrlcv_amd/csrc/pyramid.hip:

```cpp
#include <hip/hip_runtime.h>
#include <map>
#include <mutex>
#include <float.h>
#include <math.h>
#include <new>
#include <stdlib.h>
#include <string.h>
#include "dev_switch.h"
#include "device_math.h"
#include "sift_plan.h"
#include "ssrlcv_hip.h"

namespace {

__device__ __forceinline__ int sym_coord(int i, int l) {
  int ll = 2 * l;
  if (__builtin_expect(i < -ll || i >= ll, 0)) i = (i + ll) % ll;
  if (i < 0) i += ll;
  return (i > l - 1) ? ll - 1 - i : i;
}

__device__ __forceinline__ int mirror_into(int i, int l, int R) {
  if (l < 64) return sym_coord(i, l);
  i = i > l - 1 + R ? l - 1 + R : i;
// ... 876 lines not shown
        bin2x_from_tile(pend[t2], pairOk, a.binOut, (size_t)(gy >> 1) * (size_t)(W >> 1) + (size_t)(gxo >> 1));
      }
    }
#pragma unroll
    for (int t2 = 0; t2 < 2; ++t2) {
      const int gxo = x0 + (ct0 + t2) * 16 + lk * 4;
      float* o = a.out + ((size_t)gy * W + gxo);
      const f32x4 v = pend[t2];
      if (gy < H && vec4 && gxo + 3 < W) {
        *reinterpret_cast<f32x4*>(o) = v;
        mn = fminf(fminf(mn, v[0]), fminf(v[1], fminf(v[2], v[3])));
        mx = fmaxf(fmaxf(mx, v[0]), fmaxf(v[1], fmaxf(v[2], v[3])));
      } else if (gy < H) {
#pragma unroll
        for (int r = 0; r < 4; ++r)
          if (gxo + r < W) { o[r] = v[r]; mn = fminf(mn, v[r]); mx = fmaxf(mx, v[r]); }
      }
    }
  }
  if (a.minmax) block_minmax_commit(mn, mx, a.minmax, s_mem);
}

__global__ __launch_bounds__(256) void k_conv1d(const float* __restrict__ in, float* __restrict__ out, uint32_t w,
                                                uint32_t h, int taps, const float* __restrict__ wgt, int vertical,
                                                float* __restrict__ minmax) {
  uint32_t x = blockIdx.x * 256 + threadIdx.x;
  uint32_t y = blockIdx.y;
  float mn = FLT_MAX, mx = -FLT_MAX;
  if (x < w && y < h) {
    int r = taps / 2;
    float sum = 0.0f;
    for (int k = -r; k <= r; ++k) {
      int sx = vertical ? (int)x : sym_coord((int)x + k, (int)w);
      int sy = vertical ? sym_coord((int)y + k, (int)h) : (int)y;
      sum = __builtin_fmaf(in[(size_t)sy * w + sx], wgt[k + r], sum);
    }
    out[(size_t)y * w + x] = sum;
    mn = sum;
    mx = sum;
  }
  if (minmax) wave_minmax_commit(mn, mx, minmax);
}

__global__ __launch_bounds__(256) void k_minmax(const float* __restrict__ in, size_t n, float* __restrict__ minmax) {
  float mn = FLT_MAX, mx = -FLT_MAX;
  size_t stride = (size_t)gridDim.x * 256 * 4;
  for (size_t i = ((size_t)blockIdx.x * 256 + threadIdx.x) * 4; i < n; i += stride) {
    if (i + 3 < n) {
      float4 v = *reinterpret_cast<const float4*>(in + i);
      mn = fminf(fminf(mn, v.x), fminf(v.y, fminf(v.z, v.w)));
      mx = fmaxf(fmaxf(mx, v.x), fmaxf(v.y, fmaxf(v.z, v.w)));
    } else {
      for (size_t k = i; k < n; ++k) { mn = fminf(mn, in[k]); mx = fmaxf(mx, in[k]); }
    }
  }
  __shared__ float s_red[8];
  block_minmax_commit(mn, mx, minmax, s_red);
}
__global__ __launch_bounds__(256) void k_normalize(float* __restrict__ data, size_t n, const float* __restrict__ minmax) {
  const float mn = minmax[0], mx = minmax[1];
  const sv::Divisor range = sv::make_divisor(mx - mn);
  size_t i = (size_t)blockIdx.x * 256 + threadIdx.x;
  if (i < n) data[i] = sv::div_by(data[i] - mn, range);
}

struct DogArgs {
  const float* lvl[svp::kGauss];
  float* dog[svp::kDog];
  const float* lvlMinMax;
  float* dogMinMax;
  float* partial;
  size_t n;
};
template <bool PARTIAL>
__global__ __launch_bounds__(256) void k_dog(DogArgs a, int first, int last) {
  float lmn[svp::kGauss];
  sv::Divisor range[svp::kGauss];
#pragma unroll
  for (int b = 0; b < svp::kGauss; ++b) {
    lmn[b] = 0.0f;
    range[b] = sv::Divisor{1.0f, 1.0f};
    if (b >= first && b <= last) {
      lmn[b] = a.lvlMinMax[2 * b];
      range[b] = sv::make_divisor(a.lvlMinMax[2 * b + 1] - lmn[b]);
    }
  }
  float dmn[svp::kDog], dmx[svp::kDog];
#pragma unroll
  for (int b = 0; b < svp::kDog; ++b) { dmn[b] = FLT_MAX; dmx[b] = -FLT_MAX; }
  typedef float f32x4nt __attribute__((ext_vector_type(4)));
  auto normalised = [&](const float* lvl, size_t i, float mn, const sv::Divisor& rg) {
    const f32x4nt c0 = __builtin_nontemporal_load(reinterpret_cast<const f32x4nt*>(lvl + i));
    return make_float4(sv::div_by(c0.x - mn, rg), sv::div_by(c0.y - mn, rg), sv::div_by(c0.z - mn, rg), sv::div_by(c0.w - mn, rg));
  };
  size_t stride = (size_t)gridDim.x * 256 * 4;
  for (size_t i = ((size_t)blockIdx.x * 256 + threadIdx.x) * 4; i < a.n; i += stride) {
    float4 prev = make_float4(0.0f, 0.0f, 0.0f, 0.0f);
#pragma unroll
    for (int b = 0; b < svp::kDog; ++b) {
      if (b < first || b >= last) continue;
      if (b == first) prev = normalised(a.lvl[b], i, lmn[b], range[b]);
      const float4 cur = normalised(a.lvl[b + 1], i, lmn[b + 1], range[b + 1]);
      float4 d = make_float4(cur.x - prev.x, cur.y - prev.y, cur.z - prev.z, cur.w - prev.w);
      __builtin_nontemporal_store(f32x4nt{d.x, d.y, d.z, d.w}, reinterpret_cast<f32x4nt*>(a.dog[b] + i));
      dmn[b] = fminf(fminf(dmn[b], d.x), fminf(d.y, fminf(d.z, d.w)));
      dmx[b] = fmaxf(fmaxf(dmx[b], d.x), fmaxf(d.y, fmaxf(d.z, d.w)));
      prev = cur;
    }
  }
  if (PARTIAL) {
    const int lane = threadIdx.x & 63;
    const size_t slot = (size_t)blockIdx.x * 4 + (threadIdx.x >> 6);
#pragma unroll
    for (int b = 0; b < svp::kDog; ++b) {
      if (b < first || b >= last) continue;
#pragma unroll
      for (int o = 32; o > 0; o >>= 1) {
        dmn[b] = fminf(dmn[b], __shfl_xor(dmn[b], o, 64));
        dmx[b] = fmaxf(dmx[b], __shfl_xor(dmx[b], o, 64));
      }
      if (lane == 0) {
        a.partial[(size_t)(2 * b) * svp::kDogMaxWaves + slot] = dmn[b];
        a.partial[(size_t)(2 * b + 1) * svp::kDogMaxWaves + slot] = dmx[b];
      }
    }
    return;
  }
  if (a.dogMinMax) {
    __shared__ float s_red[4][2 * svp::kDog];
    const int lane = threadIdx.x & 63, wave = threadIdx.x >> 6;
#pragma unroll
    for (int b = 0; b < svp::kDog; ++b) {
      if (b < first || b >= last) continue;
#pragma unroll
      for (int o = 32; o > 0; o >>= 1) {
        dmn[b] = fminf(dmn[b], __shfl_xor(dmn[b], o, 64));
        dmx[b] = fmaxf(dmx[b], __shfl_xor(dmx[b], o, 64));
      }
      if (lane == 0) { s_red[wave][2 * b] = dmn[b]; s_red[wave][2 * b + 1] = dmx[b]; }
    }
    __syncthreads();
    const int t = threadIdx.x;
    if (t < 2 * svp::kDog && (t >> 1) >= first && (t >> 1) < last) {
      float v = s_red[0][t];
      for (int w = 1; w < 4; ++w) v = (t & 1) ? fmaxf(v, s_red[w][t]) : fminf(v, s_red[w][t]);
      if (t & 1) atomic_max_f(a.dogMinMax + t, v);
      else atomic_min_f(a.dogMinMax + t, v);
    }
  }
}

constexpr int kFinalizeThreads = 1024;
__global__ __launch_bounds__(kFinalizeThreads) void k_dog_finalize(const float* __restrict__ partial, unsigned waves, int first,
                                                                   float* __restrict__ dogMinMax) {
  const int b = first + (int)blockIdx.x;
  const float* pmn = partial + (size_t)(2 * b) * svp::kDogMaxWaves;
  const float* pmx = partial + (size_t)(2 * b + 1) * svp::kDogMaxWaves;
  float mn = FLT_MAX, mx = -FLT_MAX;
  for (unsigned i = threadIdx.x; i < waves; i += kFinalizeThreads) {
    mn = fminf(mn, pmn[i]);
    mx = fmaxf(mx, pmx[i]);
  }
#pragma unroll
  for (int o = 32; o > 0; o >>= 1) {
    mn = fminf(mn, __shfl_xor(mn, o, 64));
    mx = fmaxf(mx, __shfl_xor(mx, o, 64));
  }
  __shared__ float s_red[2 * kFinalizeThreads / 64];
  const int wave = threadIdx.x >> 6;
  if ((threadIdx.x & 63) == 0) { s_red[2 * wave] = mn; s_red[2 * wave + 1] = mx; }
  __syncthreads();
  if (threadIdx.x == 0) {
    for (int w = 1; w < kFinalizeThreads / 64; ++w) { mn = fminf(mn, s_red[2 * w]); mx = fmaxf(mx, s_red[2 * w + 1]); }
    dogMinMax[2 * b] = mn;
    dogMinMax[2 * b + 1] = mx;
  }
}

struct DogxArgs {
  const float* lvl[svp::kGauss];
  const float* lvlMinMax;
  uint8_t* flags;
  float* partial;
  int w, h;
  int strips;
  int rowsPerWave;
  float minAbs;
};

__device__ __forceinline__ float dpp_from_lane_below(float v) {
  return __builtin_bit_cast(float, __builtin_amdgcn_update_dpp(__builtin_bit_cast(int, v), __builtin_bit_cast(int, v), 0x138, 0xF, 0xF, false));
}
__device__ __forceinline__ float dpp_from_lane_above(float v) {
  return __builtin_bit_cast(float, __builtin_amdgcn_update_dpp(__builtin_bit_cast(int, v), __builtin_bit_cast(int, v), 0x130, 0xF, 0xF, false));
}
__device__ __forceinline__ float dmax3(float a, float b, float c) { return __builtin_fmaxf(__builtin_fmaxf(a, b), c); }
__device__ __forceinline__ float dmin3(float a, float b, float c) { return __builtin_fminf(__builtin_fminf(a, b), c); }

template <int NPX, int first, int last, int mmFirst, bool orFlags>
#ifndef SSRLCV_DOGX_MINWAVES
#define SSRLCV_DOGX_MINWAVES 1
#endif
#ifndef SSRLCV_DOGX_VGPR_MIN
#define SSRLCV_DOGX_VGPR_MIN 0
#endif
#ifndef SSRLCV_EARLY_CHAIN0
#define SSRLCV_EARLY_CHAIN0 1
#endif
#ifndef SSRLCV_DOGX_RING
#define SSRLCV_DOGX_RING 1
#endif
#ifndef SSRLCV_PAIR_F32_MINPX
#define SSRLCV_PAIR_F32_MINPX (~(size_t)0)
#endif
__global__ __launch_bounds__(256, SSRLCV_DOGX_MINWAVES) void k_dogx(DogxArgs a) {
  typedef float vec __attribute__((ext_vector_type(NPX)));
  const int lane = threadIdx.x & 63;
  const int gwave = blockIdx.x * 4 + (threadIdx.x >> 6);
  const int strip = gwave % a.strips, seg = gwave / a.strips;
  const int W = a.w, H = a.h;
  const int r0 = seg * a.rowsPerWave;
  if (r0 >= H) return;
  const int r1 = r0 + a.rowsPerWave < H ? r0 + a.rowsPerWave : H;
  const int x = (strip * 62 + lane - 1) * NPX;
  const bool mine = lane >= 1 && lane <= 62 && x < W;
  const int xl = x < 0 ? 0 : (x < W ? x : W - NPX);
  float lmn[svp::kGauss];
  sv::Divisor rg[svp::kGauss];
#pragma unroll
  for (int b = 0; b < svp::kGauss; ++b) {
    lmn[b] = 0.0f;
    rg[b] = sv::Divisor{1.0f, 1.0f};
    if (b >= first && b <= last) {
      lmn[b] = a.lvlMinMax[2 * b];
      rg[b] = sv::make_divisor(a.lvlMinMax[2 * b + 1] - lmn[b]);
#if SSRLCV_DOGX_VGPR_MIN
      asm volatile("" : "+v"(lmn[b]));
#endif
    }
  }
  float dmn[svp::kDog], dmx[svp::kDog];
#pragma unroll
  for (int b = 0; b < svp::kDog; ++b) { dmn[b] = FLT_MAX; dmx[b] = -FLT_MAX; }
  float gmxA[3][NPX], gmnA[3][NPX], gmxB[3][NPX], gmnB[3][NPX], gmxC[3][NPX], gmnC[3][NPX];
  float ctrX[3][NPX], ctrY[3][NPX], ctrZ[3][NPX];
#pragma unroll
  for (int k = 0; k < 3; ++k)
#pragma unroll
    for (int i = 0; i < NPX; ++i) {
      gmxA[k][i] = gmnA[k][i] = gmxB[k][i] = gmnB[k][i] = gmxC[k][i] = gmnC[k][i] = 0.0f;
      ctrX[k][i] = ctrY[k][i] = ctrZ[k][i] = 0.0f;
    }
  constexpr bool RING = SSRLCV_DOGX_RING && NPX == 4;
  constexpr int NL = last - first + 1;
  static_assert(!RING || (NL >= 4 && NL <= 6), "ring_take's wait counts are written out for 4..6 levels");
  __shared__ float4 s_ring[RING ? 4 * 2 * NL * 64 : 1];
  const int wave = __builtin_amdgcn_readfirstlane((int)(threadIdx.x >> 6));
  float4* const ring = s_ring + (RING ? wave * 2 * NL * 64 : 0);
  vec cur[svp::kGauss];
  auto fetch = [&](int y) {
    y = y < 0 ? 0 : (y > H - 1 ? H - 1 : y);
    const size_t row = (size_t)y * W + xl;
#pragma unroll
    for (int b = first; b <= last; ++b) cur[b] = __builtin_nontemporal_load(reinterpret_cast<const vec*>(a.lvl[b] + row));
  };
  auto ring_issue = [&](int y, int slot) {
    y = y < 0 ? 0 : (y > H - 1 ? H - 1 : y);
    const size_t row = (size_t)y * W + xl;
#pragma unroll
    for (int b = first; b <= last; ++b)
      __builtin_amdgcn_global_load_lds((const void __attribute__((address_space(1)))*)(a.lvl[b] + row),
                                       (void __attribute__((address_space(3)))*)(ring + (slot * NL + (b - first)) * 64), 16, 0, 2 );
  };
  auto ring_take = [&](int slot, bool followed) {
    if (followed) {
      if (NL == 6) asm volatile("s_waitcnt vmcnt(6)" ::: "memory");
      else if (NL == 5) asm volatile("s_waitcnt vmcnt(5)" ::: "memory");
      else asm volatile("s_waitcnt vmcnt(4)" ::: "memory");
    } else {
      asm volatile("s_waitcnt vmcnt(0)" ::: "memory");
    }
    const uint32_t addr = (uint32_t)(uintptr_t)(void __attribute__((address_space(3)))*)(ring + slot * NL * 64) + 16u * (uint32_t)lane;
#pragma unroll
    for (int b = first; b <= last; ++b)
      asm volatile("ds_read_b128 %0, %1 offset:%2" : "=v"(cur[b]) : "v"(addr), "n"((b - first) * 1024) : "memory");
    if (NL == 6) asm volatile("s_waitcnt lgkmcnt(0)" : "+v"(cur[first]), "+v"(cur[first + 1]), "+v"(cur[first + 2]), "+v"(cur[first + 3]), "+v"(cur[first + 4]), "+v"(cur[last]) : : "memory");
    else if (NL == 5) asm volatile("s_waitcnt lgkmcnt(0)" : "+v"(cur[first]), "+v"(cur[first + 1]), "+v"(cur[first + 2]), "+v"(cur[first + 3]), "+v"(cur[last]) : : "memory");
    else asm volatile("s_waitcnt lgkmcnt(0)" : "+v"(cur[first]), "+v"(cur[first + 1]), "+v"(cur[first + 2]), "+v"(cur[last]) : : "memory");
  };
  const int yEnd = r0 - 1 + (r1 - r0 + 2 + 2) / 3 * 3 - 1;
  unsigned pendPacked = 0;
  unsigned* pendPtr = nullptr;
  auto flush_flags = [&]() {
    if (pendPtr) *pendPtr = orFlags ? (*pendPtr | pendPacked) : pendPacked;
    pendPtr = nullptr;
  };
  auto row = [&](int y, const float (&oMx)[3][NPX], const float (&oMn)[3][NPX], const float (&pMx)[3][NPX],
                 const float (&pMn)[3][NPX], float (&nMx)[3][NPX], float (&nMn)[3][NPX], const float (&cPrev)[3][NPX],
                 float (&cNew)[3][NPX]) __attribute__((always_inline)) {
    float d[svp::kDog][NPX];
    {
      float prev[NPX];
#pragma unroll
      for (int b = first; b <= last; ++b) {
        float n[NPX];
#pragma unroll
        for (int i = 0; i < NPX; ++i) n[i] = sv::div_by(cur[b][i] - lmn[b], rg[b]);
        if (b > first) {
#pragma unroll
          for (int i = 0; i < NPX; ++i) d[b - 1][i] = n[i] - prev[i];
        }
#pragma unroll
        for (int i = 0; i < NPX; ++i) prev[i] = n[i];
      }
    }
#pragma unroll
    for (int b = first; b < last; ++b) {
#pragma unroll
      for (int i = 0; i < NPX; ++i) asm volatile("" : "+v"(d[b][i]) : : "memory");
    }
    if (RING) {
      if (y < yEnd) {
        const int slot = (y + 1 - (r0 - 1)) & 1;
        ring_take(slot, y + 2 <= yEnd);
        flush_flags();
        if (y + 3 <= yEnd) ring_issue(y + 3, slot);
      } else {
        flush_flags();
      }
    } else {
      fetch(y + 1);
    }
    float hmx[svp::kDog][NPX], hmn[svp::kDog][NPX];
#pragma unroll
    for (int b = first; b < last; ++b) {
      const float left = dpp_from_lane_below(d[b][NPX - 1]);
      const float right = dpp_from_lane_above(d[b][0]);
#pragma unroll
      for (int i = 0; i < NPX; ++i) {
        const float l = i == 0 ? left : d[b][i - 1], r = i == NPX - 1 ? right : d[b][i + 1];
        hmx[b][i] = dmax3(l, d[b][i], r);
        hmn[b][i] = dmin3(l, d[b][i], r);
      }
      if (b >= mmFirst) {
        if (NPX == 4) {
          dmx[b] = dmax3(dmx[b], hmx[b][1], d[b][3]);
          dmn[b] = dmin3(dmn[b], hmn[b][1], d[b][3]);
        } else if (NPX == 2) {
          dmx[b] = dmax3(dmx[b], d[b][0], d[b][1]);
          dmn[b] = dmin3(dmn[b], d[b][0], d[b][1]);
        } else {
          dmx[b] = __builtin_fmaxf(dmx[b], d[b][0]);
          dmn[b] = __builtin_fminf(dmn[b], d[b][0]);
        }
      }
    }
#pragma unroll
    for (int k = 0; k < 3; ++k) {
#pragma unroll
      for (int i = 0; i < NPX; ++i) nMx[k][i] = nMn[k][i] = 0.0f;
      if (k < first || k + 2 >= last) continue;
#pragma unroll
      for (int i = 0; i < NPX; ++i) {
        nMx[k][i] = dmax3(hmx[k][i], hmx[k + 1][i], hmx[k + 2][i]);
        nMn[k][i] = dmin3(hmn[k][i], hmn[k + 1][i], hmn[k + 2][i]);
      }
    }
    const int yo = y - 1;
    if (yo >= r0 && yo < r1 && mine) {
      const bool rowIn = yo > 0 && yo < H - 1;
      unsigned packed = 0;
#pragma unroll
      for (int i = 0; i < NPX; ++i) {
        const bool in = rowIn && (x + i) > 0 && (x + i) < W - 1;
#pragma unroll
        for (int k = 0; k < 3; ++k) {
          if (k < first || k + 2 >= last) continue;
          const float hi = dmax3(oMx[k][i], pMx[k][i], nMx[k][i]);
          const float lo = dmin3(oMn[k][i], pMn[k][i], nMn[k][i]);
          const float c = cPrev[k][i];
          const bool ext = in && (hi == c || lo == c);
          const bool loud = ext && !(__builtin_fabsf(c) < a.minAbs);
          packed |= (ext ? 1u << (8 * i + k) : 0u) | (loud ? 1u << (8 * i + svp::kNoiseFlagShift + k) : 0u);
        }
      }
      uint8_t* fp = a.flags + (size_t)yo * W + x;
      if (RING) {
        pendPacked = packed;
        pendPtr = reinterpret_cast<unsigned*>(fp);
      } else if (NPX == 4) {
        unsigned* p4 = reinterpret_cast<unsigned*>(fp);
        *p4 = orFlags ? (*p4 | packed) : packed;
      } else if (NPX == 2) {
        unsigned short* p2 = reinterpret_cast<unsigned short*>(fp);
        *p2 = (unsigned short)(orFlags ? (*p2 | packed) : packed);
      } else {
        *fp = (uint8_t)(orFlags ? (*fp | packed) : packed);
      }
    }
#pragma unroll
    for (int k = 0; k < 3; ++k) {
#pragma unroll
      for (int i = 0; i < NPX; ++i) cNew[k][i] = (k < first || k + 2 >= last) ? 0.0f : d[k + 1][i];
    }
  };
  if (RING) {
    ring_issue(r0 - 1, 0);
    ring_issue(r0, 1);
    ring_take(0, true);
    ring_issue(r0 + 1, 0);
  } else {
    fetch(r0 - 1);
  }
  for (int y = r0 - 1; y <= r1; y += 3) {
    row(y, gmxA, gmnA, gmxB, gmnB, gmxC, gmnC, ctrX, ctrY);
    row(y + 1, gmxB, gmnB, gmxC, gmnC, gmxA, gmnA, ctrY, ctrZ);
    row(y + 2, gmxC, gmnC, gmxA, gmnA, gmxB, gmnB, ctrZ, ctrX);
  }
  if (RING) flush_flags();
  if (RING) asm volatile("s_waitcnt vmcnt(0)" ::: "memory");
#pragma unroll
  for (int b = mmFirst; b < last; ++b) {
#pragma unroll
    for (int o = 32; o > 0; o >>= 1) {
      dmn[b] = fminf(dmn[b], __shfl_xor(dmn[b], o, 64));
      dmx[b] = fmaxf(dmx[b], __shfl_xor(dmx[b], o, 64));
    }
    if (lane == 0) {
      a.partial[(size_t)(2 * b) * svp::kDogMaxWaves + gwave] = dmn[b];
      a.partial[(size_t)(2 * b + 1) * svp::kDogMaxWaves + gwave] = dmx[b];
    }
  }
}

int launch_dogx(const float* const levels[svp::kGauss], const float* levelMinMax, uint32_t w, uint32_t h, uint8_t* flags,
                float* dogMinMax, float* partial, int first, int last, int mmFirst, bool orFlags, float minAbs,
                unsigned targetWaves, hipStream_t st) {
  if (first < 0 || last > svp::kDog || last - first < 1 || mmFirst < first || mmFirst >= last) return SSRLCV_ERR_INVALID_ARG;
  DogxArgs a;
  for (int b = 0; b < svp::kGauss; ++b) a.lvl[b] = levels[b];
  a.lvlMinMax = levelMinMax;
  a.flags = flags;
  a.partial = partial;
  a.w = (int)w;
  a.h = (int)h;
  a.minAbs = minAbs;
  static const int forceNpx = svdev::env("SSRLCV_DOGX_NPX") ? atoi(svdev::env("SSRLCV_DOGX_NPX")) : 0;
  bool aligned16 = (w & 3) == 0, aligned8 = (w & 1) == 0;
  for (int b = first; b <= last; ++b) {
    aligned16 = aligned16 && (reinterpret_cast<size_t>(levels[b]) & 15) == 0;
    aligned8 = aligned8 && (reinterpret_cast<size_t>(levels[b]) & 7) == 0;
  }
  aligned16 = aligned16 && (reinterpret_cast<size_t>(flags) & 3) == 0;
  aligned8 = aligned8 && (reinterpret_cast<size_t>(flags) & 1) == 0;
  int npx = aligned16 ? 4 : aligned8 ? 2 : 1;
  if (forceNpx == 2 && aligned8) npx = 2;
  if (forceNpx == 1) npx = 1;
  a.strips = (int)((w + 62 * npx - 1) / (62 * npx));
  if (targetWaves > svp::kDogMaxWaves) targetWaves = svp::kDogMaxWaves;
  unsigned segs = targetWaves / (unsigned)a.strips;
  if (segs < 1) segs = 1;
  unsigned rows = (h + segs - 1) / segs;
  if (rows < 16) rows = 16;
  rows += (3 - (rows + 2) % 3) % 3;
  a.rowsPerWave = (int)rows;
  segs = (h + rows - 1) / rows;
  const unsigned waves = segs * (unsigned)a.strips;
  if (waves > svp::kDogMaxWaves) return SSRLCV_ERR_UNSUPPORTED;
  const dim3 grid((waves + 3) / 4);
#define SSRLCV_LAUNCH_DOGX(F, L, M, O)                                                               \
  do {                                                                                              \
    if (npx == 4) hipLaunchKernelGGL((k_dogx<4, F, L, M, O>), grid, dim3(256), 0, st, a);           \
    else if (npx == 2) hipLaunchKernelGGL((k_dogx<2, F, L, M, O>), grid, dim3(256), 0, st, a);      \
    else hipLaunchKernelGGL((k_dogx<1, F, L, M, O>), grid, dim3(256), 0, st, a);                    \
  } while (0)
  if (first == 0 && last == 5 && mmFirst == 0 && !orFlags) SSRLCV_LAUNCH_DOGX(0, 5, 0, false);
  else if (first == 0 && last == 3 && mmFirst == 0 && !orFlags) SSRLCV_LAUNCH_DOGX(0, 3, 0, false);
  else if (first == 1 && last == 5 && mmFirst == 3 && orFlags) SSRLCV_LAUNCH_DOGX(1, 5, 3, true);
  else return SSRLCV_ERR_INVALID_ARG;
#undef SSRLCV_LAUNCH_DOGX
  hipLaunchKernelGGL(k_dog_finalize, dim3((unsigned)(last - mmFirst)), dim3(kFinalizeThreads), 0, st, partial, waves, mmFirst, dogMinMax);
  SSRLCV_LAUNCH_CHECK();
  return SSRLCV_OK;
}

bool upsample_fusable(uint32_t w, uint32_t h, int taps) {
  static const bool off = svdev::env("SSRLCV_NO_UPSAMPLE_FUSION") != nullptr || svdev::env("SSRLCV_GAUSS_MFMA") != nullptr;
  return !off && taps / 2 <= 8 && w % kTX == 0 && (w & 3) == 0 && (h & 1) == 0;
}

void launch_valu(ConvArgs a, int RT, uint32_t firstColumn, hipStream_t st) {
  const uint32_t w = a.w, h = a.h;
  const uint32_t bx = (w - firstColumn + kTX - 1) / kTX;
  uint32_t rows = h;
  while (rows > 64 && ((w + kTX - 1) / kTX) * ((h + rows - 1) / rows) < 1024) rows = (rows + 1) / 2;
  rows = (rows + kNR - 1) / kNR * kNR;
  a.rowsPerBlock = rows;
  const uint32_t by = (h + rows - 1) / rows;
  const bool aligned = firstColumn == 0 && (w & 3) == 0 && (a.u8 || (reinterpret_cast<size_t>(a.in) & 15) == 0);
  const uint32_t nFull = aligned ? w / kTX : 0;
#define SSRLCV_LAUNCH_VALU(RR)                                                                                 \
  do {                                                                                                          \
    if (nFull && a.u8) hipLaunchKernelGGL((k_gauss_strip<RR, true>), dim3(nFull, by), dim3(kTX), 0, st, a);     \
    else if (nFull) hipLaunchKernelGGL((k_gauss_strip<RR, false>), dim3(nFull, by), dim3(kTX), 0, st, a);       \
    if (nFull < bx) {                                                                                           \
      a.x0base = firstColumn + nFull * kTX;                                                                     \
      hipLaunchKernelGGL(k_gauss_fused<RR>, dim3(bx - nFull, by), dim3(kTX), 0, st, a);                         \
    }                                                                                                           \
  } while (0)
  switch (RT) {
    case 6: SSRLCV_LAUNCH_VALU(6); break;
    case 8: SSRLCV_LAUNCH_VALU(8); break;
    case 11: SSRLCV_LAUNCH_VALU(11); break;
    case 16: SSRLCV_LAUNCH_VALU(16); break;
    case 23: SSRLCV_LAUNCH_VALU(23); break;
    default: SSRLCV_LAUNCH_VALU(32); break;
  }
#undef SSRLCV_LAUNCH_VALU
}

int& rm_mask() {
  static int m = svdev::env("SSRLCV_GAUSS_RM") ? atoi(svdev::env("SSRLCV_GAUSS_RM")) : (4 | 8 | 16);
  return m;
}
size_t& rm_min_px() {
  static size_t v = svdev::env("SSRLCV_GAUSS_RM_MINPX") ? (size_t)atoll(svdev::env("SSRLCV_GAUSS_RM_MINPX")) : ((size_t)1 << 24);
  return v;
}
int& rm_oneb_mask() {
  static int m = svdev::env("SSRLCV_GAUSS_RM_ONEB") ? atoi(svdev::env("SSRLCV_GAUSS_RM_ONEB")) : 0;
  return m;
}
int& rm_rows() {
  static int r = svdev::env("SSRLCV_GAUSS_RM_ROWS") ? atoi(svdev::env("SSRLCV_GAUSS_RM_ROWS")) : 0;
  return r;
}

int launch_conv(const float* in, float* out, float* tmp, uint32_t w, uint32_t h, int taps, const float* weights_host,
                float* minmax, hipStream_t st, const uint8_t* u8src = nullptr, float* binOut = nullptr,
                bool* binned = nullptr) {
  if (taps < 1 || (taps & 1) == 0 || taps > svp::kMaxTaps) return SSRLCV_ERR_INVALID_ARG;
  int R = taps / 2;
  if (R > 32) return SSRLCV_ERR_UNSUPPORTED;
  ConvArgs a;
  a.in = in;
  a.out = out;
  a.minmax = minmax;
  a.w = w;
  a.h = h;
  a.x0base = 0;
  a.rowsPerBlock = h;
  a.binOut = nullptr;
  static const bool noXcdStrips = svdev::env("SSRLCV_NO_XCD_STRIPS") != nullptr;
  a.xcdStrips = noXcdStrips ? 0u : 1u;
  if (binned) *binned = false;
  static const bool noBinFold = svdev::env("SSRLCV_NO_BIN_FUSION") != nullptr;
  const bool canBin = binOut && !noBinFold && (w & 3) == 0 && (h & 1) == 0 && (reinterpret_cast<size_t>(binOut) & 7) == 0;
#ifdef SSRLCV_STAMPS
  a.stamps = g_lab_stamps;
#endif
  a.u8 = u8src;
  if (u8src && !upsample_fusable(w, h, taps)) return SSRLCV_ERR_INVALID_ARG;
  memset(a.wgt, 0, sizeof a.wgt);
  int RT = R <= 6 ? 6 : R <= 8 ? 8 : R <= 11 ? 11 : R <= 16 ? 16 : R <= 23 ? 23 : 32;
  for (int k = 0; k <= R; ++k) {
    if (weights_host[k] != weights_host[taps - 1 - k]) return SSRLCV_ERR_UNSUPPORTED;
    a.wgt[(RT - R) + k] = weights_host[k];
  }
  static const bool forceValu = svdev::env("SSRLCV_GAUSS_VALU") != nullptr, forceMfma = svdev::env("SSRLCV_GAUSS_MFMA") != nullptr;
  static const int mfmaMinR = svdev::env("SSRLCV_GAUSS_MFMA_MINR") ? atoi(svdev::env("SSRLCV_GAUSS_MFMA_MINR")) : 11;
  const bool useMfma = forceMfma || (!forceValu && !u8src && RT >= mfmaMinR);
  static const size_t tileMaxPx = svdev::env("SSRLCV_GAUSS_TILE_MAXPX") ? (size_t)atoll(svdev::env("SSRLCV_GAUSS_TILE_MAXPX")) : ((size_t)1 << 20);
  const bool tiny = w < 64 || h < 64;
  if (tiny || (!u8src && !forceValu && (size_t)w * h <= tileMaxPx)) {
    if (u8src) return SSRLCV_ERR_INVALID_ARG;
    if (canBin) { a.binOut = binOut; if (binned) *binned = true; }
#define SSRLCV_LAUNCH_TILE(RR)                                                                                     \
  do {                                                                                                              \
    static bool attr = false;                                                                                       \
    if (!attr) {                                                                                                    \
      SSRLCV_HIP_TRY(hipFuncSetAttribute((const void*)k_gauss_tile<RR>, hipFuncAttributeMaxDynamicSharedMemorySize, \
                                         (int)TileCfg<RR>::ldsBytes));                                              \
      attr = true;                                                                                                  \
    }                                                                                                               \
    hipLaunchKernelGGL(k_gauss_tile<RR>, dim3((w + 63) / 64, (h + 63) / 64), dim3(kTileThreads), TileCfg<RR>::ldsBytes, st, a); \
  } while (0)
    switch (RT) {
      case 6: SSRLCV_LAUNCH_TILE(6); break;
      case 8: SSRLCV_LAUNCH_TILE(8); break;
      case 11: SSRLCV_LAUNCH_TILE(11); break;
      case 16: SSRLCV_LAUNCH_TILE(16); break;
      case 23: SSRLCV_LAUNCH_TILE(23); break;
      default: SSRLCV_LAUNCH_TILE(32); break;
    }
#undef SSRLCV_LAUNCH_TILE
    SSRLCV_LAUNCH_CHECK();
    return SSRLCV_OK;
  }
  const int rmMask = rm_mask(), rmRows = rm_rows();
  const int R2 = R <= 6 ? 6 : R <= 8 ? 8 : R <= 12 ? 12 : R <= 16 ? 16 : R <= 24 ? 24 : 32;
  const int r2bit = R2 == 6 ? 1 : R2 == 8 ? 2 : R2 == 12 ? 4 : R2 == 16 ? 8 : R2 == 24 ? 16 : 32;
  if ((rmMask & r2bit) && !forceValu && !forceMfma && (size_t)w * h >= rm_min_px() && !u8src && w >= 256 && h >= 64 && (w & 3) == 0 && (h & 3) == 0 && (reinterpret_cast<size_t>(in) & 15) == 0 &&
      (reinterpret_cast<size_t>(out) & 15) == 0 && (uint64_t)w * h * 4 < ((uint64_t)1 << 32)) {
    const uint32_t nS = w / 256, cov = nS * 256;
    ConvArgs r = a;
    if (canBin && cov == w) { r.binOut = binOut; if (binned) *binned = true; }
    memset(r.wgt, 0, sizeof r.wgt);
    for (int k = 0; k <= R; ++k) r.wgt[(R2 - R) + k] = weights_host[k];
#define SSRLCV_LAUNCH_RM_V(RR, OB)                                                                                  \
  do {                                                                                                              \
    constexpr size_t ldsB = OB ? RmCfg<RR>::ldsBytesOneB : RmCfg<RR>::ldsBytes;                                    \
    static int blocksPerCu = 0, cus = 0;                                                                            \
    if (!blocksPerCu) {                                                                                             \
      SSRLCV_HIP_TRY(hipFuncSetAttribute((const void*)k_gauss_rm<RR, OB>, hipFuncAttributeMaxDynamicSharedMemorySize, \
                                         (int)ldsB));                                                               \
      int dev = 0, occ = 0;                                                                                         \
      SSRLCV_HIP_TRY(hipGetDevice(&dev));                                                                           \
      SSRLCV_HIP_TRY(hipDeviceGetAttribute(&cus, hipDeviceAttributeMultiprocessorCount, dev));                      \
      if (hipOccupancyMaxActiveBlocksPerMultiprocessor(&occ, (const void*)k_gauss_rm<RR, OB>, 256, ldsB) != hipSuccess || occ < 1) \
        occ = 1;                                                                                                    \
      blocksPerCu = occ;                                                                                            \
    }                                                                                                               \
    uint32_t by = ((uint32_t)(blocksPerCu * cus) + nS - 1) / nS;                                                    \
    uint32_t rows = (h + by - 1) / by;                                                                              \
    rows = rows < 128 ? 128 : rows;                                                                                 \
    if (rmRows > 0) rows = (uint32_t)rmRows;                                                                        \
    rows = (rows + 15) / 16 * 16;                                                                                   \
    r.rowsPerBlock = rows;                                                                                          \
    hipLaunchKernelGGL((k_gauss_rm<RR, OB>), dim3(nS, (h + rows - 1) / rows), dim3(256), ldsB, st, r);              \
  } while (0)
#define SSRLCV_LAUNCH_RM(RR)                                  \
  do {                                                        \
    if (rm_oneb_mask() & r2bit) SSRLCV_LAUNCH_RM_V(RR, true); \
    else SSRLCV_LAUNCH_RM_V(RR, false);                       \
// ... 83 lines not shown
      auto mk = [&](hipEvent_t& e) { ok = ok && hipEventCreateWithFlags(&e, hipEventDisableTiming) == hipSuccess; };
      if (ok) {
        struct Side { hipStream_t chain, table, chain2, polar; };
        static std::map<int, Side> pool;
        int dev = 0;
        ok = hipGetDevice(&dev) == hipSuccess;
        auto it = pool.find(dev);
        if (ok && it == pool.end()) {
          Side pr{nullptr, nullptr, nullptr, nullptr};
          int least = 0, greatest = 0;
          (void)hipDeviceGetStreamPriorityRange(&least, &greatest);
          const int tablePrio = svdev::env("SSRLCV_SIDE_LOW_PRIORITY") ? least : 0;
          const int prioMode = svp::stream_priority_mode();
          ok = hipStreamCreateWithPriority(&pr.chain, hipStreamNonBlocking, (prioMode & 2) ? greatest : 0) == hipSuccess &&
               hipStreamCreateWithPriority(&pr.table, hipStreamNonBlocking, tablePrio) == hipSuccess &&
               hipStreamCreateWithPriority(&pr.chain2, hipStreamNonBlocking, (prioMode & 2) ? greatest : 0) == hipSuccess &&
               hipStreamCreateWithPriority(&pr.polar, hipStreamNonBlocking, (prioMode & 1) ? least : 0) == hipSuccess;
          if (ok) it = pool.emplace(dev, pr).first;
        }
        if (ok) {
          a->chain = it->second.chain;
          a->table = it->second.table;
          a->chain2 = it->second.chain2;
          a->polar = it->second.polar;
        }
        mk(a->fork);
        for (hipEvent_t& e : a->join) mk(e);
        for (hipEvent_t& e : a->convDone) mk(e);
        for (hipEvent_t& e : a->dogDone) mk(e);
        for (hipEvent_t& e : a->polarDone) mk(e);
        for (hipEvent_t& e : a->binDone) mk(e);
        mk(a->groupFork);
        for (hipEvent_t& e : a->groupExpanded) mk(e);
        for (hipEvent_t& e : a->groupReady) mk(e);
        mk(a->expandFork);
        for (hipEvent_t& e : a->expandJoin) mk(e);
        for (auto& lv : a->levelDone)
          for (hipEvent_t& e : lv) mk(e);
      }
      if (ok) {
        plan->async = a;
        plan->asyncState = 1;
      } else {
        delete a;
        (void)hipGetLastError();
      }
    }
  }
  return plan->asyncState == 1 ? plan->async : nullptr;
}
}

extern "C" {

int ssrlcv_gauss_kernel_host(float sigma, float pixelWidth, float* weights) {
  int ksize = (int)ceilf((float)8 * sigma / pixelWidth);
  if (ksize % 2 == 0) ksize++;
  if (ksize > svp::kMaxTaps) return -ksize;
  int i = 0;
  for (int x = -ksize / 2; x <= ksize / 2; ++x, ++i) {
    weights[i] = expf(-((x * x) / 2.0f / sigma / sigma)) / sqrtf((float)(2.0f * SSRLCV_PI_D)) / sigma;
  }
  return ksize;
}

int ssrlcv_hip_convert_to_bw(const uint8_t* colorPixels, uint32_t colorDepth, uint8_t* bw, size_t numPixels,
                             ssrlcv_stream_t stream) {
  if (!colorPixels || !bw || colorDepth < 2 || colorDepth > 4) return SSRLCV_ERR_INVALID_ARG;
  if (numPixels == 0) return SSRLCV_OK;
  hipLaunchKernelGGL(k_to_bw, dim3((unsigned)((numPixels + 255) / 256)), dim3(256), 0, (hipStream_t)stream, colorPixels,
                     (int)colorDepth, bw, numPixels);
  SSRLCV_LAUNCH_CHECK();
  return SSRLCV_OK;
}

int ssrlcv_hip_u8_to_f32(const uint8_t* pixels, float* out, size_t n, ssrlcv_stream_t stream) {
  if (!pixels || !out) return SSRLCV_ERR_INVALID_ARG;
  if (n == 0) return SSRLCV_OK;
  hipLaunchKernelGGL(k_u8_to_f32, dim3((unsigned)((n + 1023) / 1024)), dim3(256), 0, (hipStream_t)stream, pixels, out, n);
  SSRLCV_LAUNCH_CHECK();
  return SSRLCV_OK;
}

int ssrlcv_hip_upsample2x(const float* in, uint32_t w, uint32_t h, float* out, ssrlcv_stream_t stream) {
  if (!in || !out || !w || !h) return SSRLCV_ERR_INVALID_ARG;
  hipLaunchKernelGGL(k_upsample2x<float>, dim3((2 * w + 255) / 256, 2 * h), dim3(256), 0, (hipStream_t)stream, in, w, h, out);
  SSRLCV_LAUNCH_CHECK();
  return SSRLCV_OK;
}

int ssrlcv_hip_upsample2x_u8(const uint8_t* in, uint32_t w, uint32_t h, float* out, ssrlcv_stream_t stream) {
  if (!in || !out || !w || !h) return SSRLCV_ERR_INVALID_ARG;
  if ((w & 1) == 0 && (reinterpret_cast<size_t>(out) & 15) == 0)
    hipLaunchKernelGGL(k_upsample2x_u8x4, dim3((2 * w / 4 + 255) / 256, 2 * h), dim3(256), 0, (hipStream_t)stream, in, w,
                       h, out);
  else
    hipLaunchKernelGGL(k_upsample2x<uint8_t>, dim3((2 * w + 255) / 256, 2 * h), dim3(256), 0, (hipStream_t)stream, in, w,
                       h, out);
  SSRLCV_LAUNCH_CHECK();
  return SSRLCV_OK;
}

int ssrlcv_hip_bin2x(const float* in, uint32_t w, uint32_t h, float* out, ssrlcv_stream_t stream) {
  if (!in || !out || w < 2 || h < 2 || (w & 1)) return SSRLCV_ERR_INVALID_ARG;
  hipLaunchKernelGGL(k_bin2x, dim3((w / 2 + 255) / 256, h / 2), dim3(256), 0, (hipStream_t)stream, in, w, h, out);
  SSRLCV_LAUNCH_CHECK();
  return SSRLCV_OK;
}

int ssrlcv_hip_gauss_sep_conv(const float* in, float* out, float* tmp, uint32_t w, uint32_t h, int taps,
                              const float* weights_host, float* minmax, ssrlcv_stream_t stream) {
  if (!in || !out || !weights_host || !w || !h || in == out) return SSRLCV_ERR_INVALID_ARG;
  return launch_conv(in, out, tmp, w, h, taps, weights_host, minmax, (hipStream_t)stream);
}

int ssrlcv_hip_minmax(const float* in, size_t n, float* minmax, ssrlcv_stream_t stream) {
  if (!in || !minmax || !n) return SSRLCV_ERR_INVALID_ARG;
  hipStream_t st = (hipStream_t)stream;
  hipLaunchKernelGGL(k_init_minmax, dim3(1), dim3(64), 0, st, minmax, 1);
  size_t blocks = (n + 1023) / 1024;
  if (blocks > 1024) blocks = 1024;
  hipLaunchKernelGGL(k_minmax, dim3((unsigned)blocks), dim3(256), 0, st, in, n, minmax);
  SSRLCV_LAUNCH_CHECK();
  return SSRLCV_OK;
}

int ssrlcv_hip_normalize(float* data, size_t n, const float* minmax, ssrlcv_stream_t stream) {
  if (!data || !minmax || !n) return SSRLCV_ERR_INVALID_ARG;
  hipLaunchKernelGGL(k_normalize, dim3((unsigned)((n + 255) / 256)), dim3(256), 0, (hipStream_t)stream, data, n, minmax);
  SSRLCV_LAUNCH_CHECK();
  return SSRLCV_OK;
}

static int launch_dog(const float* const levels_host[6], const float* levelMinMax, uint32_t w, uint32_t h,
                      float* const dog_host[5], float* dogMinMax, int firstDog, int lastDog, unsigned maxBlocks,
                      float* partial, ssrlcv_stream_t stream) {
  if (!levels_host || !levelMinMax || !dog_host || !w || !h) return SSRLCV_ERR_INVALID_ARG;
  if (firstDog < 0 || lastDog > svp::kDog || firstDog >= lastDog) return SSRLCV_ERR_INVALID_ARG;
  size_t n = (size_t)w * h;
  if (n % 4) return SSRLCV_ERR_INVALID_ARG;
  DogArgs a;
  for (int b = 0; b < svp::kGauss; ++b) a.lvl[b] = levels_host[b];
  for (int b = 0; b < svp::kDog; ++b) a.dog[b] = dog_host[b];
  a.lvlMinMax = levelMinMax;
  a.dogMinMax = dogMinMax;
  a.partial = partial;
  a.n = n;
  size_t blocks = (n / 4 + 255) / 256;
  if (partial && dogMinMax) {
    if (maxBlocks > svp::kDogMaxBlocks) maxBlocks = svp::kDogMaxBlocks;
    if (blocks > maxBlocks) blocks = maxBlocks;
    hipLaunchKernelGGL(k_dog<true>, dim3((unsigned)blocks), dim3(256), 0, (hipStream_t)stream, a, firstDog, lastDog);
    hipLaunchKernelGGL(k_dog_finalize, dim3((unsigned)(lastDog - firstDog)), dim3(kFinalizeThreads), 0, (hipStream_t)stream, partial,
                       (unsigned)blocks * 4, firstDog, dogMinMax);
  } else {
    if (blocks > 1024) blocks = 1024;
    hipLaunchKernelGGL(k_dog<false>, dim3((unsigned)blocks), dim3(256), 0, (hipStream_t)stream, a, firstDog, lastDog);
  }
  SSRLCV_LAUNCH_CHECK();
  return SSRLCV_OK;
}
int ssrlcv_hip_dog_normalised_sub(const float* const levels_host[6], const float* levelMinMax, uint32_t w, uint32_t h,
                                  float* const dog_host[5], float* dogMinMax, ssrlcv_stream_t stream) {
  return launch_dog(levels_host, levelMinMax, w, h, dog_host, dogMinMax, 0, svp::kDog, 1024, nullptr, stream);
}

int ssrlcv_sift_plan_create(uint32_t w, uint32_t h, const ssrlcv_sift_params* params, ssrlcv_sift_plan** out) {
  if (!out || !params || !w || !h) return SSRLCV_ERR_INVALID_ARG;
  if (params->maxOrientations == 0 || params->maxOrientations > (uint32_t)svp::kMaxOrient) return SSRLCV_ERR_UNSUPPORTED;
  if (!(params->descriptorContribWidth > 0.0f) || params->descriptorContribWidth > 30.0f ||
      !(params->orientationContribWidth > 0.0f) || params->orientationContribWidth > 5.0f)
    return SSRLCV_ERR_UNSUPPORTED;
  if (w / 8 == 0 || h / 8 == 0) return SSRLCV_ERR_INVALID_ARG;
  int padMode = 0;
  uint32_t padX = 0, padY = 0, ow = w * 2, oh = h * 2;
  if (w % 2 == 0 && h % 2 == 0) {
    if (w % 8 || h % 8) {
      padMode = 1;
      padX = w % 8 ? (8 - w % 8) / 2 : 0;
      padY = h % 8 ? (8 - h % 8) / 2 : 0;
      ow = (w + 2 * padX) * 2;
      oh = (h + 2 * padY) * 2;
    }
  } else if (ow % 32 || oh % 32) {
    padMode = 2;
    padX = ow % 32 ? (32 - ow % 32) / 2 : 0;
    padY = oh % 32 ? (32 - oh % 32) / 2 : 0;
    ow += 2 * padX;
    oh += 2 * padY;
  }
  if (ow < 128 || oh < 128) return SSRLCV_ERR_UNSUPPORTED;
  if (svp::polar_level_stride(ow, oh) * 8 >= ((size_t)1 << 32)) return SSRLCV_ERR_UNSUPPORTED;
  ssrlcv_sift_plan* p = new (std::nothrow) ssrlcv_sift_plan;
  if (!p) return SSRLCV_ERR_INVALID_ARG;
  memset(p, 0, sizeof *p);
  p->W = w;
  p->H = h;
  p->padMode = padMode;
  p->padX = padX;
  p->padY = padY;
  p->params = *params;
  p->stopStage = 7;
  p->fusedCall = 0;
  p->polarInFlight = 0;
  p->chain0InFlight = 0;
  p->stageEvent = nullptr;
  p->async = nullptr;
  p->asyncState = 0;
  float sigmas[svp::kGauss];
  float mulY = sqrtf(2.0f), mulX = 2;
  sigmas[0] = sqrtf(2.0f) / 2.0f;
  for (int i = 1; i < svp::kGauss; ++i) sigmas[i] = sigmas[i - 1] * mulY;
  float pixelWidth = 1.0f;
  pixelWidth /= 2.0f;
  size_t off = 0;
  auto take = [&](size_t bytes) { size_t r = off; off += align256(bytes); return r; };
  size_t P0 = (size_t)ow * oh;
  p->off_pad = take(padMode == 1 ? (size_t)(w + 2 * padX) * (h + 2 * padY) : padMode == 2 ? (size_t)w * h * 16 : 0);
  p->off_in0 = take(P0 * 4);
  p->off_in1 = take(P0 / 4 * 4);
  p->off_in2 = take(P0 / 16 * 4);
  for (int o = 0; o < svp::kOctaves; ++o)
    for (int b = 0; b < svp::kGauss; ++b) p->off_gauss[o][b] = take((P0 >> (2 * o)) * 4);
  p->off_minmax = take(sizeof(float) * 2 * (svp::kGauss + svp::kDog) * svp::kOctaves);
  p->off_state = take(sizeof(svp::OctaveState) * svp::kOctaves);
  uint32_t maxFeat = 0;
  for (int o = 0; o < svp::kOctaves; ++o) {
    svp::OctavePlan& oc = p->oct[o];
    oc.w = ow;
    oc.h = oh;
    oc.pixelWidth = pixelWidth;
    for (int b = 0; b < svp::kGauss; ++b) {
      oc.sigma[b] = sigmas[b];
      oc.taps[b] = ssrlcv_gauss_kernel_host(sigmas[b], pixelWidth, oc.weights[b]);
      if (oc.taps[b] <= 0 || oc.taps[b] > 65) { delete p; return SSRLCV_ERR_UNSUPPORTED; }
    }
    size_t P = (size_t)ow * oh;
    oc.off_flags = take(P);
    oc.off_polar = take(svp::polar_level_stride(oc.w, oc.h) * 3 * 8);
    uint32_t cap = params->maxKeyPointsPerOctave ? params->maxKeyPointsPerOctave : (uint32_t)(P / 16);
    if (cap < 4096) cap = 4096;
    oc.cap = cap;
    oc.off_kpA = take((size_t)cap * sizeof(ssrlcv_sskeypoint));
    oc.off_kpB = take((size_t)cap * sizeof(ssrlcv_sskeypoint));
    oc.off_theta = take((size_t)cap * svp::kMaxOrient * sizeof(float));
    oc.off_thetaCnt = take((size_t)cap * sizeof(uint32_t));
    size_t words = (size_t)3 * 4 * ((P + 8191) / 8192) + 16 +
                   (size_t)svp::kDog * 4 * (((size_t)cap * svp::kMaxOrient + 2047) / 2048) + 16;
    oc.off_part = take(words * 4);
    oc.off_featBase = take(256);
    oc.off_descConst = take((size_t)cap * 32);
    maxFeat += cap;
    if (o + 1 < svp::kOctaves) {
      ow /= 2;
      oh /= 2;
      pixelWidth *= 2.0f;
      for (int b = 0; b < svp::kGauss; ++b) sigmas[b] *= mulX;
    }
  }
  p->off_extremaCounts = take(256);
  p->off_dogPartial = take(sizeof(float) * 2 * svp::kDog * svp::kDogMaxWaves * svp::kOctaves);
  p->off_groups = take(4096);
  p->total = off;
  p->maxFeatures = maxFeat;
  *out = p;
  return SSRLCV_OK;
}

void ssrlcv_sift_plan_destroy(ssrlcv_sift_plan* plan) {
  if (!plan) return;
  if (plan->async) {
    svp::PlanAsync* a = plan->async;
    (void)hipEventDestroy(a->fork);
    for (hipEvent_t e : a->join) (void)hipEventDestroy(e);
    for (hipEvent_t e : a->convDone) (void)hipEventDestroy(e);
    for (hipEvent_t e : a->dogDone) (void)hipEventDestroy(e);
    for (hipEvent_t e : a->polarDone) (void)hipEventDestroy(e);
    for (hipEvent_t e : a->binDone) (void)hipEventDestroy(e);
    (void)hipEventDestroy(a->expandFork);
    (void)hipEventDestroy(a->groupFork);
    for (hipEvent_t e : a->groupExpanded) (void)hipEventDestroy(e);
    for (hipEvent_t e : a->groupReady) (void)hipEventDestroy(e);
    for (hipEvent_t e : a->expandJoin) (void)hipEventDestroy(e);
    for (auto& lv : a->levelDone)
      for (hipEvent_t e : lv) (void)hipEventDestroy(e);
    delete a;
  }
  delete plan;
}
size_t ssrlcv_sift_plan_workspace_bytes(const ssrlcv_sift_plan* plan) { return plan ? plan->total : 0; }
uint32_t ssrlcv_sift_plan_max_features(const ssrlcv_sift_plan* plan) { return plan ? plan->maxFeatures : 0; }
void ssrlcv_sift_plan_set_stop_stage(ssrlcv_sift_plan* plan, int stage) { if (plan) plan->stopStage = stage; }
int ssrlcv_sift_plan_set_stage_event(ssrlcv_sift_plan* plan, void* event) {
  if (!plan) return SSRLCV_ERR_INVALID_ARG;
  plan->stageEvent = (hipEvent_t)event;
  return SSRLCV_OK;
}

int ssrlcv_sift_plan_level(const ssrlcv_sift_plan* plan, void* workspace, int kind, int octave, int blur, float** data,
                           uint32_t* w, uint32_t* h, float** minmax_dev) {
  if (!plan || !workspace || octave < 0 || octave >= svp::kOctaves) return SSRLCV_ERR_INVALID_ARG;
  char* ws = (char*)workspace;
  const svp::OctavePlan& oc = plan->oct[octave];
  float* mm = (float*)(ws + plan->off_minmax) + (size_t)octave * 2 * (svp::kGauss + svp::kDog);
  if (kind == 0) {
    if (blur < 0 || blur >= svp::kDog) return SSRLCV_ERR_INVALID_ARG;
    if (((size_t)oc.w * oc.h) % 4) return SSRLCV_ERR_UNSUPPORTED;
    SSRLCV_HIP_TRY(hipDeviceSynchronize());
    const float* lv[svp::kGauss];
    float* dogs[svp::kDog];
    float* scratch = (float*)(ws + plan->off_in0);
    for (int b = 0; b < svp::kGauss; ++b) lv[b] = (const float*)(ws + plan->off_gauss[octave][b]);
    for (int b = 0; b < svp::kDog; ++b) dogs[b] = scratch;
    int rc = launch_dog(lv, mm, oc.w, oc.h, dogs, nullptr, blur, blur + 1, 1024, nullptr, nullptr);
    if (rc) return rc;
    SSRLCV_HIP_TRY(hipDeviceSynchronize());
    if (data) *data = scratch;
    if (minmax_dev) *minmax_dev = mm + 2 * (svp::kGauss + blur);
  } else if (kind == 1) {
    if (blur < 0 || blur >= svp::kGauss) return SSRLCV_ERR_INVALID_ARG;
    if (data) *data = (float*)(ws + plan->off_gauss[octave][blur]);
    if (minmax_dev) *minmax_dev = mm + 2 * blur;
  } else {
    return SSRLCV_ERR_INVALID_ARG;
  }
  if (w) *w = oc.w;
  if (h) *h = oc.h;
  return SSRLCV_OK;
}

namespace {
struct DogSchedule {
  int split;
  unsigned waves;
  DogSchedule() {
    split = 0;
    if (const char* e = svdev::env("SSRLCV_DOG_SPLIT")) split = atoi(e) != 0 ? 1 : 0;
    waves = 14336;
    if (const char* e = svdev::env("SSRLCV_DOGX_WAVES")) waves = (unsigned)atoi(e) > 0 ? (unsigned)atoi(e) : 14336;
  }
};
}

int ssrlcv_hip_sift_build_dog(const ssrlcv_sift_plan* plan, const uint8_t* pixels, void* workspace,
                              ssrlcv_stream_t stream) {
  if (!plan || !pixels || !workspace) return SSRLCV_ERR_INVALID_ARG;
  hipStream_t st = (hipStream_t)stream;
  char* ws = (char*)workspace;
  float* mmAll = (float*)(ws + plan->off_minmax);
  const int pairs = (svp::kGauss + svp::kDog) * svp::kOctaves;
  svp::PlanAsync* as = svp::plan_async(plan);
  hipStream_t sd = as ? as->table : st;
  static const DogSchedule sched;
  static const bool overlapOctaves = svdev::env("SSRLCV_NO_OCTAVE_OVERLAP") == nullptr;
  static const int overlapFrom = svdev::env("SSRLCV_OCTAVE_OVERLAP_FROM") ? atoi(svdev::env("SSRLCV_OCTAVE_OVERLAP_FROM")) : 1;
  static const int deferDog0 = [] {
    const int n = svdev::env("SSRLCV_DOGX0_AFTER") ? atoi(svdev::env("SSRLCV_DOGX0_AFTER")) : 0;
    return n == 1 || n == 2 ? n : 0;
  }();
  static const bool wantEarlyPolar = svdev::env("SSRLCV_EARLY_POLAR") != nullptr;
  const bool earlyPolar = as && plan->fusedCall && plan->stopStage >= 6 && wantEarlyPolar;
  plan->polarInFlight = 0;
  plan->chain0InFlight = 0;
  if (earlyPolar) {
    SSRLCV_HIP_TRY(hipEventRecord(as->fork, st));
    SSRLCV_HIP_TRY(hipStreamWaitEvent(as->polar, as->fork, 0));
  }
  hipLaunchKernelGGL(k_init_minmax, dim3(1), dim3(64), 0, st, mmAll, pairs);
  float* in = (float*)(ws + plan->off_in0);
  int rc;
  bool fuseUpsample = false;
  if (plan->padMode == 1) {
    const uint32_t pw = plan->W + 2 * plan->padX, ph = plan->H + 2 * plan->padY;
    uint8_t* padded = (uint8_t*)(ws + plan->off_pad);
    hipLaunchKernelGGL(k_add_border<uint8_t>, dim3((pw + 255) / 256, ph), dim3(256), 0, st, pixels, plan->W, plan->H, padded,
                       plan->padX, plan->padY);
    rc = ssrlcv_hip_upsample2x_u8(padded, pw, ph, in, stream);
  } else if (plan->padMode == 2) {
    float* up = (float*)(ws + plan->off_pad);
    rc = ssrlcv_hip_upsample2x_u8(pixels, plan->W, plan->H, up, stream);
    hipLaunchKernelGGL(k_add_border<float>, dim3((plan->oct[0].w + 255) / 256, plan->oct[0].h), dim3(256), 0, st, up,
                       2 * plan->W, 2 * plan->H, in, plan->padX, plan->padY);
  } else if (upsample_fusable(plan->oct[0].w, plan->oct[0].h, plan->oct[0].taps[0])) {
    rc = 0;
    fuseUpsample = true;
  } else {
    rc = ssrlcv_hip_upsample2x_u8(pixels, plan->W, plan->H, in, stream);
  }
  if (rc) return rc;
  float* nextIn[3] = {(float*)(ws + plan->off_in1), (float*)(ws + plan->off_in2), (float*)(ws + plan->off_in1)};
  const float firstNoise = (float)(svp::kNoiseThreshold * 0.8);
  static const int phased = svdev::env("SSRLCV_PHASED") ? atoi(svdev::env("SSRLCV_PHASED")) : 0;
  if (as && phased > 0) {
    const int ahead = phased - 1;
    const float* octIn = in;
    for (int o = 0; o < svp::kOctaves; ++o) {
      const svp::OctavePlan& oc = plan->oct[o];
      float* mm = mmAll + (size_t)o * 2 * (svp::kGauss + svp::kDog);
      const float* src = octIn;
      for (int b = 0; b < 4; ++b) {
        float* dst = (float*)(ws + plan->off_gauss[o][b]);
        bool binned = false;
        rc = launch_conv(src, dst, nullptr, oc.w, oc.h, oc.taps[b], oc.weights[b], mm + 2 * b, st,
                         (fuseUpsample && o == 0 && b == 0) ? pixels : nullptr, (b == 3 && o + 1 < svp::kOctaves) ? nextIn[o] : nullptr, &binned);
        if (rc) return rc;
        src = dst;
        if (b == 3 && o + 1 < svp::kOctaves) {
          if (!binned) {
            rc = ssrlcv_hip_bin2x(dst, oc.w, oc.h, nextIn[o], (ssrlcv_stream_t)st);
            if (rc) return rc;
          }
          octIn = nextIn[o];
        }
      }
      SSRLCV_HIP_TRY(hipEventRecord(as->binDone[o], st));
    }
    for (int o = 0; o < svp::kOctaves; ++o) {
      const svp::OctavePlan& oc = plan->oct[o];
      float* mm = mmAll + (size_t)o * 2 * (svp::kGauss + svp::kDog);
      const hipStream_t sb = o == 0 ? as->table : (o == 1 ? as->chain : st);
      const int gate = o + ahead < svp::kOctaves ? o + ahead : svp::kOctaves - 1;
      if (sb != st) SSRLCV_HIP_TRY(hipStreamWaitEvent(sb, as->binDone[gate], 0));
      const float* lv[svp::kGauss];
      for (int b = 0; b < svp::kGauss; ++b) lv[b] = (const float*)(ws + plan->off_gauss[o][b]);
      for (int b = 4; b < svp::kGauss; ++b) {
        rc = launch_conv(lv[b - 1], (float*)(ws + plan->off_gauss[o][b]), nullptr, oc.w, oc.h, oc.taps[b], oc.weights[b], mm + 2 * b, sb);
        if (rc) return rc;
      }
      float* dogPartial = (float*)(ws + plan->off_dogPartial) + (size_t)o * 2 * svp::kDog * svp::kDogMaxWaves;
      rc = launch_dogx(lv, mm, oc.w, oc.h, (uint8_t*)(ws + oc.off_flags), mm + 2 * svp::kGauss, dogPartial, 0, svp::kDog, 0, false, firstNoise,
                       sched.waves, sb);
      if (rc) return rc;
      SSRLCV_HIP_TRY(hipEventRecord(as->dogDone[o], sb));
      if (earlyPolar) {
        SSRLCV_HIP_TRY(hipStreamWaitEvent(as->polar, as->dogDone[o], 0));
        svp::launch_polar_octave(plan, ws, o, as->polar);
        SSRLCV_HIP_TRY(hipEventRecord(as->polarDone[o], as->polar));
      }
    }
    if (earlyPolar) plan->polarInFlight = 1;
    SSRLCV_HIP_TRY(hipStreamWaitEvent(st, as->dogDone[0], 0));
    SSRLCV_HIP_TRY(hipStreamWaitEvent(st, as->dogDone[1], 0));
    return SSRLCV_OK;
  }
  for (int o = 0; o < svp::kOctaves; ++o) {
    const svp::OctavePlan& oc = plan->oct[o];
    float* mm = mmAll + (size_t)o * 2 * (svp::kGauss + svp::kDog);
    const size_t* offGauss = plan->off_gauss[o];
    const hipStream_t so = (as && overlapOctaves && o >= overlapFrom && ((o - overlapFrom) & 1) == 0) ? as->chain : st;
    const hipStream_t sdo = (as && overlapOctaves && o >= 2) ? so : ((deferDog0 && as && o == 1) ? as->chain2 : sd);
    float* dogPartial = (float*)(ws + plan->off_dogPartial) + (size_t)o * 2 * svp::kDog * svp::kDogMaxWaves;
    uint8_t* flags = (uint8_t*)(ws + oc.off_flags);
    if (as && o >= 1) SSRLCV_HIP_TRY(hipStreamWaitEvent(so, as->binDone[o - 1], 0));
    const float* src = in;
    const float* lv[svp::kGauss] = {nullptr, nullptr, nullptr, nullptr, nullptr, nullptr};
    for (int b = 0; b < svp::kGauss; ++b) lv[b] = (const float*)(ws + offGauss[b]);
    const bool split = as && sched.split == 1;
    static const size_t pairMinPx = svdev::env("SSRLCV_GAUSS_PAIR_MINPX") ? (size_t)atoll(svdev::env("SSRLCV_GAUSS_PAIR_MINPX")) : ((size_t)1 << 26);
    static const size_t pairMinPxF32 = svdev::env("SSRLCV_GAUSS_PAIR_MINPX_F32") ? (size_t)atoll(svdev::env("SSRLCV_GAUSS_PAIR_MINPX_F32")) : SSRLCV_PAIR_F32_MINPX;
    int firstLevel = 0;
    const bool u8Pair = o == 0 && fuseUpsample && (size_t)oc.w * oc.h >= pairMinPx;
    const bool f32Pair = !(o == 0 && fuseUpsample) && (size_t)oc.w * oc.h >= pairMinPxF32;
    if ((u8Pair || f32Pair) && pair_rm_usable(oc.w, oc.h) &&
        pair_usable(oc.w, oc.h, oc.taps[0], oc.taps[1], f32Pair ? in : (const float*)(ws + offGauss[0]), (float*)(ws + offGauss[0]), (float*)(ws + offGauss[1]))) {
      static const bool valuForm = svdev::env("SSRLCV_GAUSS_PAIR_FORM") != nullptr && svdev::env("SSRLCV_GAUSS_PAIR_FORM")[0] == 'v';
      const float* pin = f32Pair ? in : nullptr;
      const uint8_t* pu8 = f32Pair ? nullptr : pixels;
      rc = valuForm ? launch_pair(pin, pu8, (float*)(ws + offGauss[0]), (float*)(ws + offGauss[1]), oc.w, oc.h, oc.weights[0], oc.weights[1], mm, mm + 2, so)
                    : launch_pair_rm(pin, pu8, (float*)(ws + offGauss[0]), (float*)(ws + offGauss[1]), oc.w, oc.h, oc.weights[0], oc.weights[1], mm, mm + 2, so);
      if (rc) return rc;
      src = (const float*)(ws + offGauss[1]);
      firstLevel = 2;
    }
    for (int b = firstLevel; b < svp::kGauss; ++b) {
      float* dst = (float*)(ws + offGauss[b]);
      bool binned = false;
      rc = launch_conv(src, dst, nullptr, oc.w, oc.h, oc.taps[b], oc.weights[b], mm + 2 * b, so,
                       (fuseUpsample && o == 0 && b == 0) ? pixels : nullptr,
                       (b == 3 && o + 1 < svp::kOctaves) ? nextIn[o] : nullptr, &binned);
      if (rc) return rc;
      src = dst;
      if (b == 3 && o + 1 < svp::kOctaves) {
        if (!binned) {
          rc = ssrlcv_hip_bin2x(lv[3], oc.w, oc.h, nextIn[o], (ssrlcv_stream_t)so);
          if (rc) return rc;
        }
        in = nextIn[o];
        if (as) SSRLCV_HIP_TRY(hipEventRecord(as->binDone[o], so));
        if (deferDog0 && as && o == deferDog0) {
          const svp::OctavePlan& o0 = plan->oct[0];
          const float* lv0[svp::kGauss];
          for (int q = 0; q < svp::kGauss; ++q) lv0[q] = (const float*)(ws + plan->off_gauss[0][q]);
          SSRLCV_HIP_TRY(hipStreamWaitEvent(sd, as->binDone[o], 0));
          rc = launch_dogx(lv0, mmAll, o0.w, o0.h, (uint8_t*)(ws + o0.off_flags), mmAll + 2 * svp::kGauss, (float*)(ws + plan->off_dogPartial), 0,
                           svp::kDog, 0, false, firstNoise, sched.waves, sd);
          if (rc) return rc;
          SSRLCV_HIP_TRY(hipEventRecord(as->dogDone[0], sd));
        }
      }
      if (split && b == 3) {
        SSRLCV_HIP_TRY(hipEventRecord(as->levelDone[o][b], so));
        SSRLCV_HIP_TRY(hipStreamWaitEvent(sdo, as->levelDone[o][b], 0));
        rc = launch_dogx(lv, mm, oc.w, oc.h, flags, mm + 2 * svp::kGauss, dogPartial, 0, 3, 0, false, firstNoise, sched.waves, sdo);
        if (rc) return rc;
      }
    }
    if (as) {
      SSRLCV_HIP_TRY(hipEventRecord(as->convDone[o], so));
      SSRLCV_HIP_TRY(hipStreamWaitEvent(sdo, as->convDone[o], 0));
    }
    if (deferDog0 && as && o == 0) continue;
    if (split) rc = launch_dogx(lv, mm, oc.w, oc.h, flags, mm + 2 * svp::kGauss, dogPartial, 1, svp::kDog, 3, true, firstNoise, sched.waves, sdo);
    else rc = launch_dogx(lv, mm, oc.w, oc.h, flags, mm + 2 * svp::kGauss, dogPartial, 0, svp::kDog, 0, false, firstNoise, sched.waves, sdo);
    if (rc) return rc;
    if (as) SSRLCV_HIP_TRY(hipEventRecord(as->dogDone[o], sdo));
#if SSRLCV_EARLY_CHAIN0
    static const bool noEarlyChain = svdev::env("SSRLCV_NO_EARLY_CHAIN") != nullptr;
    if (as && !noEarlyChain && ((SSRLCV_EARLY_CHAIN0 >> o) & 1) && plan->fusedCall && plan->stopStage >= 6) {
      SSRLCV_HIP_TRY(hipStreamWaitEvent(as->chain2, as->dogDone[o], 0));
      rc = svp::launch_chain_octave(plan, ws, o, as->chain2);
      if (rc) return rc;
      plan->chain0InFlight |= 1 << o;
    }
#endif
    if (earlyPolar) {
      SSRLCV_HIP_TRY(hipStreamWaitEvent(as->polar, as->dogDone[o], 0));
      svp::launch_polar_octave(plan, ws, o, as->polar);
      SSRLCV_HIP_TRY(hipEventRecord(as->polarDone[o], as->polar));
    }
  }
  if (earlyPolar) plan->polarInFlight = 1;
  if (as) {
    for (int o = 0; o < svp::kOctaves; ++o) SSRLCV_HIP_TRY(hipStreamWaitEvent(st, as->dogDone[o], 0));
  }
  return SSRLCV_OK;
}

}
```

ssrlcv_amd/csrc/sift_plan.h:

```cpp
#pragma once
#include <stdint.h>
#include <stddef.h>
#include <hip/hip_runtime.h>
#include "ssrlcv_hip.h"

namespace svp {

constexpr int kOctaves = 4;
constexpr int kGauss = 6;
constexpr int kDog = 5;
constexpr int kMaxTaps = 129;
constexpr int kMaxOrient = 4;
constexpr float kNoiseThreshold = 0.01f;
constexpr float kEdgeThreshold = 12.1f;
constexpr int kNoiseFlagShift = 4;

struct OctaveState {
  int idx[kDog];
  int n;
  int hasExtrema;
  int overflow;
  int stale[kDog];
  int pad[3];
};

__host__ __device__ inline size_t polar_level_stride(uint32_t w, uint32_t h) { return (size_t)w * h + w + 2; }

struct OctavePlan {
  uint32_t w, h;
  float pixelWidth;
  float sigma[kGauss];
  int taps[kGauss];
  float weights[kGauss][kMaxTaps];
  uint32_t cap;
  size_t off_flags;
  size_t off_polar;
  size_t off_kpA, off_kpB;
  size_t off_theta;
  size_t off_thetaCnt;
  size_t off_part;
  size_t off_featBase;
  size_t off_descConst;
};

constexpr unsigned kDogMaxBlocks = 16384;
constexpr unsigned kDogMaxWaves = kDogMaxBlocks * 4;

constexpr int kSampleGroups = 4;

struct PlanAsync {
  hipStream_t chain, table, chain2;
  hipStream_t polar;
  hipEvent_t fork;
  hipEvent_t groupFork, groupExpanded[kSampleGroups], groupReady[kSampleGroups];
  hipEvent_t join[kOctaves + 1], convDone[kOctaves], dogDone[kOctaves], polarDone[kOctaves];
  hipEvent_t binDone[kOctaves];
  hipEvent_t expandFork, expandJoin[2];
  hipEvent_t levelDone[kOctaves][kGauss];
};

}

struct ssrlcv_sift_plan {
  uint32_t W, H;
  int padMode;
  uint32_t padX, padY;
  size_t off_pad;
  ssrlcv_sift_params params;
  svp::OctavePlan oct[svp::kOctaves];
  size_t off_in0, off_in1, off_in2;
  size_t off_gauss[svp::kOctaves][svp::kGauss];
  size_t off_minmax;
  size_t off_state;
  size_t off_extremaCounts;
  size_t off_dogPartial;
  size_t off_groups;
  size_t total;
  uint32_t maxFeatures;
  int stopStage;
  mutable uint8_t listInB[svp::kOctaves];
  mutable int fusedCall;
  mutable int polarInFlight;
  mutable int chain0InFlight;
  mutable hipEvent_t stageEvent;
  mutable svp::PlanAsync* async;
  mutable int asyncState;
};

namespace svp {
PlanAsync* plan_async(const ssrlcv_sift_plan* plan);
int stream_priority_mode();
void launch_polar_octave(const ssrlcv_sift_plan* plan, char* ws, int octave, hipStream_t st);
int launch_chain_octave(const ssrlcv_sift_plan* plan, char* ws, int octave, hipStream_t st);
}
```

Baseline: 3622 Mpix/s.

## Fuse orientation prologue memsets and expand launches into single multi-octave kernels

Replaces the per-octave hipMemsetAsync calls and the build_ranges kernel with one k_orient_prepare kernel that zeroes the scan scratch and group controls and builds the theta range table. Merges the per-octave expand launches into one multi-octave k_expand_orient grid whose last block, chosen by a ticket counter, does the feature booking and builds the descriptor range table, so the separate book kernel is no longer launched. The goal is fewer launches and stream/event hops on the critical path. In exchange, expansion of all octaves now runs serialised on one stream unless opted out, and the ticket-based last-block logic adds grid-wide atomics. The diff also adds instrumented-only gap stamps for measuring kernel timing.

```diff
diff --git a/ssrlcv_amd/csrc/dev_switch.h b/ssrlcv_amd/csrc/dev_switch.h
--- a/ssrlcv_amd/csrc/dev_switch.h
+++ b/ssrlcv_amd/csrc/dev_switch.h
@@ -1,8 +1,8 @@
 #pragma once
 #include <stdlib.h>
 
-#if (defined(SSRLCV_STAMPS) || defined(SSRLCV_MATCH_STATS) || defined(SSRLCV_TIMING_VARIANT)) && !defined(SSRLCV_INSTRUMENTED_BUILD)
-#error "SSRLCV_STAMPS / SSRLCV_MATCH_STATS only build through `make instrumented` or the tools/ lab programs (-DSSRLCV_INSTRUMENTED_BUILD)"
+#if (defined(SSRLCV_STAMPS) || defined(SSRLCV_MATCH_STATS) || defined(SSRLCV_TIMING_VARIANT) || defined(SSRLCV_GAP_STAMPS)) && !defined(SSRLCV_INSTRUMENTED_BUILD)
+#error "SSRLCV_STAMPS / SSRLCV_MATCH_STATS / SSRLCV_GAP_STAMPS only build through `make instrumented` or the tools/ lab programs (-DSSRLCV_INSTRUMENTED_BUILD)"
 #endif
 #if defined(SSRLCV_LAB) || defined(SSRLCV_MATCH_LAB) || defined(SSRLCV_LAB_LOCAL_GATHER) || defined(SSRLCV_LAB_UPS_LOADS)
 #error "the timing-lab variants (results invalid) were removed in round 6; see git history before 2026-10-05"
diff --git a/ssrlcv_amd/csrc/keypoints.hip b/ssrlcv_amd/csrc/keypoints.hip
--- a/ssrlcv_amd/csrc/keypoints.hip
+++ b/ssrlcv_amd/csrc/keypoints.hip
@@ -280,6 +280,9 @@
   float2* out[svp::kOctaves];
   uint32_t start[svp::kOctaves + 1];
   uint32_t tilesX[svp::kOctaves];
+#ifdef SSRLCV_GAP_STAMPS
+  unsigned long long* gapStamps;
+#endif
 };
 #ifndef SSRLCV_NT_STORES
 #define SSRLCV_NT_STORES 1
@@ -293,6 +296,7 @@
 #endif
 }
 __global__ __launch_bounds__(256) void k_polar(PolarJobs jobs) {
+  SSRLCV_GAP_STAMP(jobs.gapStamps, svp::kGapPolar);
   __shared__ float s_n[kPolRows][256 + 2];
   int o = 0;
 #pragma unroll
@@ -428,7 +432,8 @@
   tab->total = pos;
 }
 __global__ void k_build_ranges(const OctaveState* st, RangeTable* tab, int unitShift, uint32_t sel) { build_ranges(st, tab, unitShift, sel); }
-__global__ void k_book_and_desc_ranges(OctaveState* st, uint32_t* featBase, uint32_t* numFeatures, uint32_t maxFeatures, RangeTable* tab) {
+__device__ __forceinline__ void book_and_desc_ranges(const OctaveState* st, uint32_t* featBase, uint32_t* numFeatures, uint32_t maxFeatures,
+                                                     RangeTable* tab) {
   uint32_t tot = 0;
   for (int o = 0; o < svp::kOctaves; ++o) {
     featBase[o] = tot;
@@ -437,6 +442,9 @@
   if (tot > maxFeatures) tot = maxFeatures;
   *numFeatures = tot;
   build_ranges(st, tab, 0, 0xFFFFFu);
+}
+__global__ void k_book_and_desc_ranges(const OctaveState* st, uint32_t* featBase, uint32_t* numFeatures, uint32_t maxFeatures, RangeTable* tab) {
+  book_and_desc_ranges(st, featBase, numFeatures, maxFeatures, tab);
 }
 
 constexpr int kOct0Groups = svp::kSampleGroups - 1;
@@ -447,7 +455,8 @@
   uint32_t done[svp::kSampleGroups];
   uint32_t regular;
   uint32_t cut[2];
-  uint32_t pad[32 - svp::kDog - 3 * svp::kSampleGroups - 4];
+  uint32_t ticket;
+  uint32_t pad[32 - svp::kDog - 3 * svp::kSampleGroups - 5];
 };
 static_assert(sizeof(GroupCtl) == 128, "four of them + eight range tables fit the plan's 4 KB group block");
 __device__ __forceinline__ bool blur_indices_regular(const OctaveState* st) {
@@ -514,6 +523,9 @@
   float* thetas[svp::kOctaves];
   uint32_t* thetaCnt[svp::kOctaves];
   const void* consts[svp::kOctaves];
+#ifdef SSRLCV_GAP_STAMPS
+  unsigned long long* gapStamps;
+#endif
 };
 
 template <int MAXO, int LPKS>
@@ -521,6 +533,7 @@
                                                float orientationThreshold) {
   constexpr int LANES = 1 << LPKS, PER_BLOCK = 64 >> LPKS, CW = kThetaChunk * LANES;
   __shared__ float s_hist[36][PER_BLOCK];
+  SSRLCV_GAP_STAMP(set.gapStamps, svp::kGapThetas);
   if (blockIdx.x >= tab->total) return;
   const int range = __builtin_amdgcn_readfirstlane(range_of(tab, blockIdx.x));
   const int octave = range & 3, useg = kSegOrder[range >> 2];
@@ -760,6 +773,7 @@
 static_assert(sizeof(DescConst) == 32, "one s_load_dwordx8");
 __global__ __launch_bounds__(256) void k_desc_consts(const RangeTable* tab, OctaveSet set, float lambda, const OctaveState* states,
                                                      const GroupCtl* regularCtl) {
+  SSRLCV_GAP_STAMP(set.gapStamps, svp::kGapDescConsts);
   const uint32_t total = tab->total;
   const bool fromTable = regularCtl != nullptr && regularCtl->regular != 0u;
   for (uint32_t u = blockIdx.x * 256 + threadIdx.x; u < total; u += gridDim.x * 256) {
@@ -803,6 +817,7 @@
                                                      ssrlcv_sift_feature* __restrict__ features, uint32_t maxFeatures) {
   __shared__ unsigned s_bins[4][(1 + 128 + 2) * kDescCopies];
   __shared__ __attribute__((aligned(8))) uint8_t s_bytes[4][128];
+  SSRLCV_GAP_STAMP(set.gapStamps, svp::kGapDescriptors);
   const int lane = threadIdx.x & 63, wave = __builtin_amdgcn_readfirstlane(threadIdx.x >> 6);
   unsigned* bins = s_bins[wave] + kDescCopies;
   const int copy = lane & (kDescCopies - 1);
@@ -1011,6 +1026,9 @@
     if (o >= oFirst && o <= oLast) pos += jobs.tilesX[o] * ((oc.h + kPolRows - 1) / kPolRows);
   }
   jobs.start[svp::kOctaves] = pos;
+#ifdef SSRLCV_GAP_STAMPS
+  jobs.gapStamps = svp::gap_stamps(plan, ws);
+#endif
   hipLaunchKernelGGL(k_polar, dim3(pos), dim3(256), 0, st, jobs);
 }
 
@@ -1027,6 +1045,9 @@
     jobs.start[o] = o <= octave ? 0u : tiles;
   }
   jobs.start[svp::kOctaves] = tiles;
+#ifdef SSRLCV_GAP_STAMPS
+  jobs.gapStamps = svp::gap_stamps(plan, ws);
+#endif
   hipLaunchKernelGGL(k_polar, dim3(tiles), dim3(256), 0, st, jobs);
 }
 }
@@ -1198,14 +1219,16 @@
     set.thetaCnt[o] = (uint32_t*)(ws + oc.off_thetaCnt);
     set.consts[o] = ws + oc.off_descConst;
   }
+#ifdef SSRLCV_GAP_STAMPS
+  set.gapStamps = svp::gap_stamps(plan, ws);
+#endif
   return set;
 }
 
 constexpr int kExpandItems = 16;
-__global__ __launch_bounds__(svs::kThreads) void k_expand_orient(OctaveState* st, const ssrlcv_sskeypoint* __restrict__ src,
-                                                                 ssrlcv_sskeypoint* __restrict__ dst, const float* __restrict__ thetas,
-                                                                 const uint32_t* __restrict__ thetaCnt, uint32_t maxO, uint32_t cap,
-                                                                 svs::TileScan<1> ts, GroupCtl* ctl, int g, int pieces) {
+__device__ __forceinline__ void expand_octave(OctaveState* st, const ssrlcv_sskeypoint* __restrict__ src, ssrlcv_sskeypoint* __restrict__ dst,
+                                              const float* __restrict__ thetas, const uint32_t* __restrict__ thetaCnt, uint32_t maxO,
+                                              uint32_t cap, const svs::TileScan<1>& ts, GroupCtl* ctl, int g, int pieces, uint32_t numBlocks) {
   constexpr int ITEMS = kExpandItems;
   constexpr uint32_t kTile = svs::kThreads * ITEMS;
   const uint32_t n = st->hasExtrema && st->n > 0 ? (uint32_t)st->n : 0u;
@@ -1259,7 +1282,7 @@
   __syncthreads();
   if (threadIdx.x == 0) {
     __threadfence();
-    s_last = atomicAdd(&ctl->done[g], 1u) == gridDim.x - 1;
+    s_last = atomicAdd(&ctl->done[g], 1u) == numBlocks - 1;
   }
   __syncthreads();
   if (s_last && threadIdx.x == 0) {
@@ -1279,13 +1302,67 @@
     }
   }
 }
+struct ExpandJobs {
+  OctaveState* states;
+  GroupCtl* ctl;
+  const ssrlcv_sskeypoint* src[svp::kOctaves];
+  ssrlcv_sskeypoint* dst[svp::kOctaves];
+  const float* thetas[svp::kOctaves];
+  const uint32_t* thetaCnt[svp::kOctaves];
+  uint32_t cap[svp::kOctaves];
+  svs::TileScan<1> ts[svp::kOctaves];
+  uint32_t start[svp::kOctaves + 1];
+  uint32_t maxO;
+  int g, pieces;
+  uint32_t* featBase;
+  uint32_t* numFeatures;
+  uint32_t maxFeatures;
+  RangeTable* descTab;
+#ifdef SSRLCV_GAP_STAMPS
+  unsigned long long* gapStamps;
+#endif
+};
+__global__ __launch_bounds__(svs::kThreads) void k_expand_orient(ExpandJobs jobs) {
+  SSRLCV_GAP_STAMP(jobs.gapStamps, svp::kGapExpand);
+  int o = 0;
+#pragma unroll
+  for (int k = 1; k < svp::kOctaves; ++k)
+    if (blockIdx.x >= jobs.start[k]) o = k;
+  expand_octave(jobs.states + o, jobs.src[o], jobs.dst[o], jobs.thetas[o], jobs.thetaCnt[o], jobs.maxO, jobs.cap[o], jobs.ts[o], jobs.ctl + o,
+                jobs.g, jobs.pieces, jobs.start[o + 1] - jobs.start[o]);
+  if (jobs.descTab == nullptr || threadIdx.x != 0) return;
+  __threadfence();
+  if (atomicAdd(&jobs.ctl[0].ticket, 1u) != gridDim.x - 1) return;
+  __threadfence();
+  book_and_desc_ranges(jobs.states, jobs.featBase, jobs.numFeatures, jobs.maxFeatures, jobs.descTab);
+}
+struct OrientPrepare {
+  uint4* part[svp::kOctaves];
+  uint32_t part16[svp::kOctaves];
+  GroupCtl* ctl;
+  const OctaveState* states;
+  RangeTable* thetaTab;
+  int unitShift;
+  uint32_t sel;
+};
+__global__ __launch_bounds__(256) void k_orient_prepare(OrientPrepare p) {
+  const uint32_t tid = blockIdx.x * 256 + threadIdx.x, step = gridDim.x * 256;
+  const uint4 zero = make_uint4(0u, 0u, 0u, 0u);
+#pragma unroll
+  for (int o = 0; o < svp::kOctaves; ++o)
+    for (uint32_t i = tid; i < p.part16[o]; i += step) p.part[o][i] = zero;
+  if (tid < svp::kOctaves * sizeof(GroupCtl) / 16) reinterpret_cast<uint4*>(p.ctl)[tid] = zero;
+  if (tid == 0) build_ranges(p.states, p.thetaTab, p.unitShift, p.sel);
+}
 
 struct GroupBlock {
   RangeTable thetaTab[svp::kSampleGroups];
   RangeTable descTab[svp::kSampleGroups];
   GroupCtl ctl[svp::kOctaves];
 };
-static_assert(sizeof(RangeTable) <= 256 && 8 * 256 + svp::kOctaves * sizeof(GroupCtl) <= 4096, "fits the plan's group block");
+static_assert(sizeof(RangeTable) <= 256 && 8 * 256 + svp::kOctaves * sizeof(GroupCtl) <= svp::kGapStampOffset &&
+                  svp::kGapStampOffset + svp::kGapStampWords * svp::kGapKernels * sizeof(unsigned long long) <= 4096,
+              "fits the plan's group block (the instrumented build's kernel stamps sit behind it, sift_plan.h)");
 inline RangeTable* theta_tab(const ssrlcv_sift_plan* plan, char* ws, int g) { return (RangeTable*)(ws + plan->off_groups + 256 * g); }
 inline RangeTable* desc_tab(const ssrlcv_sift_plan* plan, char* ws, int g) { return (RangeTable*)(ws + plan->off_groups + 256 * (svp::kSampleGroups + g)); }
 inline GroupCtl* group_ctl(const ssrlcv_sift_plan* plan, char* ws, int o) { return (GroupCtl*)(ws + plan->off_groups + 2048) + o; }
@@ -1326,32 +1403,66 @@
   }
 }
 
-int expand_prepare(const ssrlcv_sift_plan* plan, char* ws, int o, int g, hipStream_t st) {
+inline uint32_t expand_cap_tiles(const ssrlcv_sift_plan* plan, int o) {
+  return (plan->oct[o].cap * plan->params.maxOrientations + svs::kThreads * kExpandItems - 1) / (svs::kThreads * kExpandItems);
+}
+inline char* expand_scratch(const ssrlcv_sift_plan* plan, char* ws, int o, int g) {
+  return ws + plan->oct[o].off_part + (size_t)g * svs::workspace_bytes<1>(expand_cap_tiles(plan, o));
+}
+unsigned expand_job(ExpandJobs& jobs, const ssrlcv_sift_plan* plan, char* ws, int o, int g) {
   const svp::OctavePlan& oc = plan->oct[o];
-  const uint32_t capTiles = (oc.cap * plan->params.maxOrientations + svs::kThreads * kExpandItems - 1) / (svs::kThreads * kExpandItems);
-  const size_t scanBytes = svs::workspace_bytes<1>(capTiles);
-  SSRLCV_HIP_TRY(hipMemsetAsync(ws + oc.off_part + (size_t)g * scanBytes, 0, scanBytes, st));
+  jobs.src[o] = (const ssrlcv_sskeypoint*)(ws + (plan->listInB[o] ? oc.off_kpB : oc.off_kpA));
+  jobs.dst[o] = (ssrlcv_sskeypoint*)(ws + (plan->listInB[o] ? oc.off_kpA : oc.off_kpB));
+  jobs.thetas[o] = (const float*)(ws + oc.off_theta);
+  jobs.thetaCnt[o] = (const uint32_t*)(ws + oc.off_thetaCnt);
+  jobs.cap[o] = oc.cap;
+  const uint32_t capTiles = expand_cap_tiles(plan, o);
+  jobs.ts[o] = svs::make_tile_scan<1>(expand_scratch(plan, ws, o, g), capTiles);
+  const unsigned blocks = capTiles / 8 + 1;
+  return blocks > 1024u ? 1024u : blocks;
+}
+void expand_job_common(ExpandJobs& jobs, const ssrlcv_sift_plan* plan, char* ws) {
+  jobs = ExpandJobs{};
+  jobs.states = (OctaveState*)(ws + plan->off_state);
+  jobs.ctl = group_ctl(plan, ws, 0);
+  jobs.maxO = plan->params.maxOrientations;
+  jobs.g = 0;
+  jobs.pieces = 1;
+  jobs.maxFeatures = plan->maxFeatures;
+#ifdef SSRLCV_GAP_STAMPS
+  jobs.gapStamps = svp::gap_stamps(plan, ws);
+#endif
+}
+int launch_expand(const ssrlcv_sift_plan* plan, char* ws, int o, int g, int pieces, hipStream_t es, bool scratchZeroed = false) {
+  ExpandJobs jobs;
+  expand_job_common(jobs, plan, ws);
+  const unsigned blocks = expand_job(jobs, plan, ws, o, g);
+  for (int k = 0; k <= svp::kOctaves; ++k) jobs.start[k] = k <= o ? 0u : blocks;
+  jobs.g = g;
+  jobs.pieces = pieces;
+  if (!scratchZeroed) SSRLCV_HIP_TRY(hipMemsetAsync(expand_scratch(plan, ws, o, g), 0, svs::workspace_bytes<1>(expand_cap_tiles(plan, o)), es));
+  hipLaunchKernelGGL(k_expand_orient, dim3(blocks), dim3(svs::kThreads), 0, es, jobs);
   return SSRLCV_OK;
 }
-int launch_expand(const ssrlcv_sift_plan* plan, char* ws, int o, int g, int pieces, hipStream_t es, bool scratchZeroed = false) {
-  const svp::OctavePlan& oc = plan->oct[o];
-  const uint32_t maxO = plan->params.maxOrientations, cap = oc.cap;
-  OctaveState* states = (OctaveState*)(ws + plan->off_state);
-  const ssrlcv_sskeypoint* src = (const ssrlcv_sskeypoint*)(ws + (plan->listInB[o] ? oc.off_kpB : oc.off_kpA));
-  ssrlcv_sskeypoint* dst = (ssrlcv_sskeypoint*)(ws + (plan->listInB[o] ? oc.off_kpA : oc.off_kpB));
-  const uint32_t capTiles = (cap * maxO + svs::kThreads * kExpandItems - 1) / (svs::kThreads * kExpandItems);
-  const size_t scanBytes = svs::workspace_bytes<1>(capTiles);
-  char* part = ws + oc.off_part + (size_t)g * scanBytes;
-  if (!scratchZeroed) SSRLCV_HIP_TRY(hipMemsetAsync(part, 0, scanBytes, es));
-  unsigned blocks = capTiles / 8 + 1;
-  blocks = blocks > 1024u ? 1024u : blocks;
-  hipLaunchKernelGGL(k_expand_orient, dim3(blocks), dim3(svs::kThreads), 0, es, states + o, src, dst, (const float*)(ws + oc.off_theta),
-                     (const uint32_t*)(ws + oc.off_thetaCnt), maxO, cap, svs::make_tile_scan<1>(part, capTiles), group_ctl(plan, ws, o), g, pieces);
-  return SSRLCV_OK;
+void launch_expand_all(const ssrlcv_sift_plan* plan, char* ws, hipStream_t st, uint32_t* numFeatures) {
+  ExpandJobs jobs;
+  expand_job_common(jobs, plan, ws);
+  uint32_t pos = 0;
+  for (int o = 0; o < svp::kOctaves; ++o) {
+    jobs.start[o] = pos;
+    pos += expand_job(jobs, plan, ws, o, 0);
+  }
+  jobs.start[svp::kOctaves] = pos;
+  if (numFeatures) {
+    jobs.featBase = (uint32_t*)(ws + plan->oct[0].off_featBase);
+    jobs.numFeatures = numFeatures;
+    jobs.descTab = desc_tab(plan, ws, 0);
+  }
+  hipLaunchKernelGGL(k_expand_orient, dim3(pos), dim3(svs::kThreads), 0, st, jobs);
 }
 bool expand_scratch_fits(const ssrlcv_sift_plan* plan, int o, int pieces) {
   const svp::OctavePlan& oc = plan->oct[o];
-  const uint32_t capTiles = (oc.cap * plan->params.maxOrientations + svs::kThreads * kExpandItems - 1) / (svs::kThreads * kExpandItems);
+  const uint32_t capTiles = expand_cap_tiles(plan, o);
   const size_t P = (size_t)oc.w * oc.h;
   const size_t words = (size_t)3 * 4 * ((P + 8191) / 8192) + 16 + (size_t)svp::kDog * 4 * (((size_t)oc.cap * svp::kMaxOrient + 2047) / 2048) + 16;
   return (size_t)pieces * svs::workspace_bytes<1>(capTiles) <= words * 4;
@@ -1382,27 +1493,34 @@
 inline hipStream_t expand_stream(svp::PlanAsync* as, hipStream_t caller, int o) {
   return !as || o == 0 ? caller : (o == 1 ? as->chain : (o == 2 ? as->table : as->chain2));
 }
-int orientations_prologue(const ssrlcv_sift_plan* plan, char* ws, hipStream_t caller, svp::PlanAsync* as) {
-  OctaveState* states = (OctaveState*)(ws + plan->off_state);
+inline bool expand_on_streams() {
+  static const bool wanted = svdev::env("SSRLCV_EXPAND_STREAMS") != nullptr;
+  return wanted;
+}
+int orientations_prologue(const ssrlcv_sift_plan* plan, char* ws, hipStream_t st) {
+  OrientPrepare p;
   uint32_t thetaSel = 0xFFFFFu;
 #ifdef SSRLCV_INSTRUMENTED_BUILD
   if (const char* e = svdev::env("SSRLCV_TIMING_THETAS_SEL")) thetaSel = (uint32_t)strtoul(e, nullptr, 16);
 #endif
-  SSRLCV_HIP_TRY(hipMemsetAsync(group_ctl(plan, ws, 0), 0, sizeof(GroupCtl) * svp::kOctaves, caller));
-  hipLaunchKernelGGL(k_build_ranges, dim3(1), dim3(1), 0, caller, states, theta_tab(plan, ws, 0), 6 - thetas_lanes_shift(), thetaSel);
-  if (as) {
-    SSRLCV_HIP_TRY(hipEventRecord(as->expandFork, caller));
-    for (int o = 1; o < svp::kOctaves; ++o) SSRLCV_HIP_TRY(hipStreamWaitEvent(expand_stream(as, caller, o), as->expandFork, 0));
-  }
+  uint32_t words = svp::kOctaves * sizeof(GroupCtl) / 16;
   for (int o = 0; o < svp::kOctaves; ++o) {
-    const int rc = expand_prepare(plan, ws, o, 0, expand_stream(as, caller, o));
-    if (rc) return rc;
-  }
+    p.part[o] = (uint4*)expand_scratch(plan, ws, o, 0);
+    p.part16[o] = (uint32_t)(svs::workspace_bytes<1>(expand_cap_tiles(plan, o)) / 16);
+    words += p.part16[o];
+  }
+  p.ctl = group_ctl(plan, ws, 0);
+  p.states = (const OctaveState*)(ws + plan->off_state);
+  p.thetaTab = theta_tab(plan, ws, 0);
+  p.unitShift = 6 - thetas_lanes_shift();
+  p.sel = thetaSel;
+  const unsigned blocks = (words + 255) / 256;
+  hipLaunchKernelGGL(k_orient_prepare, dim3(blocks > 64u ? 64u : blocks), dim3(256), 0, st, p);
   return SSRLCV_OK;
 }
 
 int stage_orientations(const ssrlcv_sift_plan* plan, char* ws, hipStream_t caller, svp::PlanAsync* as, bool polarDone, bool restInFlight = false,
-                       bool prologueDone = false) {
+                       bool prologueDone = false, uint32_t* bookInto = nullptr, bool* booked = nullptr) {
   OctaveState* states = (OctaveState*)(ws + plan->off_state);
   const uint32_t maxO = plan->params.maxOrientations;
   OctaveSet set = make_set(plan, ws);
@@ -1423,9 +1541,15 @@
     SSRLCV_HIP_TRY(hipStreamWaitEvent(caller, as->expandJoin[1], 0));
     return SSRLCV_OK;
   }
-  if (!prologueDone) orientations_prologue(plan, ws, caller, as);
+  if (!prologueDone) orientations_prologue(plan, ws, caller);
   if (!polarDone) launch_polar(plan, ws, caller);
   launch_thetas(maxO, lanesShift, thetas_grid(plan, 0, svp::kOctaves - 1, lanesShift), caller, (const OctaveState*)states, (const RangeTable*)thetaRanges, set, lambdaO, othr);
+  if (!expand_on_streams()) {
+    launch_expand_all(plan, ws, caller, bookInto);
+    for (int o = 0; o < svp::kOctaves; ++o) plan->listInB[o] ^= 1;
+    if (booked) *booked = bookInto != nullptr;
+    return SSRLCV_OK;
+  }
   if (as) {
     SSRLCV_HIP_TRY(hipEventRecord(as->groupFork, caller));
     for (int o = 1; o < svp::kOctaves; ++o) SSRLCV_HIP_TRY(hipStreamWaitEvent(expand_stream(as, caller, o), as->groupFork, 0));
@@ -1607,6 +1731,8 @@
       }
     }
   }
+  const bool earlyPrologue = as && stop >= 6 && !splitRest && !(stop >= 7 && pipelinedSampling && expand_scratch_fits(plan, 0, kOct0Groups));
+  const bool prologueOnChain2 = earlyPrologue && (plan->chain0InFlight & 1);
   for (int o = 0; o < svp::kOctaves; ++o) {
     const hipStream_t cs = !as || o == 0 ? caller : (o == 1 ? as->chain : as->chain2);
     if (!((plan->chain0InFlight >> o) & 1)) {
@@ -1614,6 +1740,11 @@
       if (rc) return rc;
     }
     if (as && (o == 1 || o == svp::kOctaves - 1)) {
+      if (prologueOnChain2 && o == svp::kOctaves - 1) {
+        SSRLCV_HIP_TRY(hipStreamWaitEvent(cs, as->join[1], 0));
+        const int rc = orientations_prologue(plan, ws, cs);
+        if (rc) return rc;
+      }
       SSRLCV_HIP_TRY(hipEventRecord(as->join[o], cs));
       SSRLCV_HIP_TRY(hipStreamWaitEvent(caller, as->join[o], 0));
     }
@@ -1625,9 +1756,8 @@
     const int rc = queue_rest_orientations(plan, ws, as->chain2, as);
     if (rc) return rc;
   }
-  const bool earlyPrologue = as && stop >= 6 && !splitRest && !(stop >= 7 && pipelinedSampling && expand_scratch_fits(plan, 0, kOct0Groups));
-  if (earlyPrologue) {
-    const int rc = orientations_prologue(plan, ws, caller, as);
+  if (earlyPrologue && !prologueOnChain2) {
+    const int rc = orientations_prologue(plan, ws, caller);
     if (rc) return rc;
   }
   if (as) {
@@ -1644,11 +1774,12 @@
     SSRLCV_LAUNCH_CHECK();
     return SSRLCV_OK;
   }
+  bool booked = false;
   if (stop >= 6) {
-    int rc = stage_orientations(plan, ws, caller, as, as != nullptr, splitRest, earlyPrologue);
+    int rc = stage_orientations(plan, ws, caller, as, as != nullptr, splitRest, earlyPrologue, stop >= 7 ? numFeatures : nullptr, &booked);
     if (rc) return rc;
   }
-  book_features(plan, ws, numFeatures, caller, stop >= 7);
+  if (!booked) book_features(plan, ws, numFeatures, caller, stop >= 7);
   if (stop >= 7) {
     int rc = stage_descriptors(plan, ws, features, caller, true);
     if (rc) return rc;
diff --git a/ssrlcv_amd/csrc/pyramid.hip b/ssrlcv_amd/csrc/pyramid.hip
--- a/ssrlcv_amd/csrc/pyramid.hip
+++ b/ssrlcv_amd/csrc/pyramid.hip
@@ -1052,7 +1052,8 @@
 
 constexpr int kFinalizeThreads = 1024;
 __global__ __launch_bounds__(kFinalizeThreads) void k_dog_finalize(const float* __restrict__ partial, unsigned waves, int first,
-                                                                   float* __restrict__ dogMinMax) {
+                                                                   float* __restrict__ dogMinMax, unsigned long long* gapStamps) {
+  SSRLCV_GAP_STAMP(gapStamps, svp::kGapDogFinalize);
   const int b = first + (int)blockIdx.x;
   const float* pmn = partial + (size_t)(2 * b) * svp::kDogMaxWaves;
   const float* pmx = partial + (size_t)(2 * b + 1) * svp::kDogMaxWaves;
@@ -1086,6 +1087,9 @@
   int strips;
   int rowsPerWave;
   float minAbs;
+#ifdef SSRLCV_GAP_STAMPS
+  unsigned long long* gapStamps;
+#endif
 };
 
 __device__ __forceinline__ float dpp_from_lane_below(float v) {
@@ -1114,6 +1118,7 @@
 #define SSRLCV_PAIR_F32_MINPX (~(size_t)0)
 #endif
 __global__ __launch_bounds__(256, SSRLCV_DOGX_MINWAVES) void k_dogx(DogxArgs a) {
+  SSRLCV_GAP_STAMP(a.gapStamps, svp::kGapDogx);
   typedef float vec __attribute__((ext_vector_type(NPX)));
   const int lane = threadIdx.x & 63;
   const int gwave = blockIdx.x * 4 + (threadIdx.x >> 6);
@@ -1335,7 +1340,7 @@
 
 int launch_dogx(const float* const levels[svp::kGauss], const float* levelMinMax, uint32_t w, uint32_t h, uint8_t* flags,
                 float* dogMinMax, float* partial, int first, int last, int mmFirst, bool orFlags, float minAbs,
-                unsigned targetWaves, hipStream_t st) {
+                unsigned targetWaves, hipStream_t st, unsigned long long* gapStamps = nullptr) {
   if (first < 0 || last > svp::kDog || last - first < 1 || mmFirst < first || mmFirst >= last) return SSRLCV_ERR_INVALID_ARG;
   DogxArgs a;
   for (int b = 0; b < svp::kGauss; ++b) a.lvl[b] = levels[b];
@@ -1345,6 +1350,9 @@
   a.w = (int)w;
   a.h = (int)h;
   a.minAbs = minAbs;
+#ifdef SSRLCV_GAP_STAMPS
+  a.gapStamps = gapStamps;
+#endif
   static const int forceNpx = svdev::env("SSRLCV_DOGX_NPX") ? atoi(svdev::env("SSRLCV_DOGX_NPX")) : 0;
   bool aligned16 = (w & 3) == 0, aligned8 = (w & 1) == 0;
   for (int b = first; b <= last; ++b) {
@@ -1379,7 +1387,7 @@
   else if (first == 1 && last == 5 && mmFirst == 3 && orFlags) SSRLCV_LAUNCH_DOGX(1, 5, 3, true);
   else return SSRLCV_ERR_INVALID_ARG;
 #undef SSRLCV_LAUNCH_DOGX
-  hipLaunchKernelGGL(k_dog_finalize, dim3((unsigned)(last - mmFirst)), dim3(kFinalizeThreads), 0, st, partial, waves, mmFirst, dogMinMax);
+  hipLaunchKernelGGL(k_dog_finalize, dim3((unsigned)(last - mmFirst)), dim3(kFinalizeThreads), 0, st, partial, waves, mmFirst, dogMinMax, gapStamps);
   SSRLCV_LAUNCH_CHECK();
   return SSRLCV_OK;
 }
@@ -1769,7 +1777,7 @@
     if (blocks > maxBlocks) blocks = maxBlocks;
     hipLaunchKernelGGL(k_dog<true>, dim3((unsigned)blocks), dim3(256), 0, (hipStream_t)stream, a, firstDog, lastDog);
     hipLaunchKernelGGL(k_dog_finalize, dim3((unsigned)(lastDog - firstDog)), dim3(kFinalizeThreads), 0, (hipStream_t)stream, partial,
-                       (unsigned)blocks * 4, firstDog, dogMinMax);
+                       (unsigned)blocks * 4, firstDog, dogMinMax, (unsigned long long*)nullptr);
   } else {
     if (blocks > 1024) blocks = 1024;
     hipLaunchKernelGGL(k_dog<false>, dim3((unsigned)blocks), dim3(256), 0, (hipStream_t)stream, a, firstDog, lastDog);
@@ -2046,7 +2054,7 @@
       }
       float* dogPartial = (float*)(ws + plan->off_dogPartial) + (size_t)o * 2 * svp::kDog * svp::kDogMaxWaves;
       rc = launch_dogx(lv, mm, oc.w, oc.h, (uint8_t*)(ws + oc.off_flags), mm + 2 * svp::kGauss, dogPartial, 0, svp::kDog, 0, false, firstNoise,
-                       sched.waves, sb);
+                       sched.waves, sb, svp::gap_stamps(plan, ws));
       if (rc) return rc;
       SSRLCV_HIP_TRY(hipEventRecord(as->dogDone[o], sb));
       if (earlyPolar) {
@@ -2110,7 +2118,7 @@
           for (int q = 0; q < svp::kGauss; ++q) lv0[q] = (const float*)(ws + plan->off_gauss[0][q]);
           SSRLCV_HIP_TRY(hipStreamWaitEvent(sd, as->binDone[o], 0));
           rc = launch_dogx(lv0, mmAll, o0.w, o0.h, (uint8_t*)(ws + o0.off_flags), mmAll + 2 * svp::kGauss, (float*)(ws + plan->off_dogPartial), 0,
-                           svp::kDog, 0, false, firstNoise, sched.waves, sd);
+                           svp::kDog, 0, false, firstNoise, sched.waves, sd, svp::gap_stamps(plan, ws));
           if (rc) return rc;
           SSRLCV_HIP_TRY(hipEventRecord(as->dogDone[0], sd));
         }
@@ -2118,7 +2126,7 @@
       if (split && b == 3) {
         SSRLCV_HIP_TRY(hipEventRecord(as->levelDone[o][b], so));
         SSRLCV_HIP_TRY(hipStreamWaitEvent(sdo, as->levelDone[o][b], 0));
-        rc = launch_dogx(lv, mm, oc.w, oc.h, flags, mm + 2 * svp::kGauss, dogPartial, 0, 3, 0, false, firstNoise, sched.waves, sdo);
+        rc = launch_dogx(lv, mm, oc.w, oc.h, flags, mm + 2 * svp::kGauss, dogPartial, 0, 3, 0, false, firstNoise, sched.waves, sdo, svp::gap_stamps(plan, ws));
         if (rc) return rc;
       }
     }
@@ -2127,8 +2135,8 @@
       SSRLCV_HIP_TRY(hipStreamWaitEvent(sdo, as->convDone[o], 0));
     }
     if (deferDog0 && as && o == 0) continue;
-    if (split) rc = launch_dogx(lv, mm, oc.w, oc.h, flags, mm + 2 * svp::kGauss, dogPartial, 1, svp::kDog, 3, true, firstNoise, sched.waves, sdo);
-    else rc = launch_dogx(lv, mm, oc.w, oc.h, flags, mm + 2 * svp::kGauss, dogPartial, 0, svp::kDog, 0, false, firstNoise, sched.waves, sdo);
+    if (split) rc = launch_dogx(lv, mm, oc.w, oc.h, flags, mm + 2 * svp::kGauss, dogPartial, 1, svp::kDog, 3, true, firstNoise, sched.waves, sdo, svp::gap_stamps(plan, ws));
+    else rc = launch_dogx(lv, mm, oc.w, oc.h, flags, mm + 2 * svp::kGauss, dogPartial, 0, svp::kDog, 0, false, firstNoise, sched.waves, sdo, svp::gap_stamps(plan, ws));
     if (rc) return rc;
     if (as) SSRLCV_HIP_TRY(hipEventRecord(as->dogDone[o], sdo));
 #if SSRLCV_EARLY_CHAIN0
diff --git a/ssrlcv_amd/csrc/sift_plan.h b/ssrlcv_amd/csrc/sift_plan.h
--- a/ssrlcv_amd/csrc/sift_plan.h
+++ b/ssrlcv_amd/csrc/sift_plan.h
@@ -88,6 +88,30 @@
 };
 
 namespace svp {
+enum GapKernel { kGapDogx = 0, kGapDogFinalize, kGapPolar, kGapThetas, kGapExpand, kGapDescConsts, kGapDescriptors, kGapKernels };
+constexpr size_t kGapStampOffset = 3072;
+constexpr int kGapStampWords = 16;
+inline unsigned long long* gap_stamps(const ssrlcv_sift_plan* plan, char* ws) { return (unsigned long long*)(ws + plan->off_groups + kGapStampOffset); }
+#ifdef SSRLCV_GAP_STAMPS
+struct GapStamp {
+  unsigned long long* pair;
+  __device__ __forceinline__ GapStamp(unsigned long long* stamps, int kernel) : pair(stamps ? stamps + kGapStampWords * kernel : nullptr) {
+    if (pair && threadIdx.x == 0) {
+      const unsigned long long t = wall_clock64();
+      if (t < __hip_atomic_load(pair, __ATOMIC_RELAXED, __HIP_MEMORY_SCOPE_AGENT)) atomicMin(pair, t);
+    }
+  }
+  __device__ __forceinline__ ~GapStamp() {
+    if (pair && threadIdx.x == 0) atomicMax(pair + 1 + blockIdx.x % (kGapStampWords - 1), (unsigned long long)wall_clock64());
+  }
+};
+#define SSRLCV_GAP_STAMP(stamps, kernel) const svp::GapStamp gapStamp_((stamps), (kernel))
+#else
+#define SSRLCV_GAP_STAMP(stamps, kernel)
+#endif
+}
+
+namespace svp {
 PlanAsync* plan_async(const ssrlcv_sift_plan* plan);
 int stream_priority_mode();
 void launch_polar_octave(const ssrlcv_sift_plan* plan, char* ws, int octave, hipStream_t st);
```

After: 3658 Mpix/s (median of 6 runs). 1.01x the previous value.
